# skyepurchase/MeatModeler

Measured on AMD Instinct MI355X. Metric: descriptor-match pairs/sec + BA residuals/sec, 500×1080p frames, 1/2/4/8 GPU, higher is better.
Workload: dtype u8/int32 (match), f64 (BA); 1 GPU; 500 frames 1920x1080, 4000 ORB kpts/frame, BF Hamming 2-NN + ratio, track linking, 2-view DLT, full BA (TRF, Schur, f64 MFMA Cholesky); frames=500, height=1080, width=1920, nfeatures=4000, parallelism=pairs/points x1

## Files before the change

include/meatmodeler.h:

```cpp
#ifndef MEATMODELER_H
#define MEATMODELER_H

#include <stddef.h>
#include <stdint.h>

#ifdef __cplusplus
extern "C" {
#endif

#define MM_OK 0
#define MM_ERR_ARG (-1)
#define MM_ERR_HIP (-2)
#define MM_ERR_WORKSPACE (-3)
#define MM_ERR_NUMERIC (-4)

typedef struct mm_ctx mm_ctx;

int mm_abi_version(void);
int mm_ctx_create(int device, void *hip_stream, mm_ctx **out);
void mm_ctx_destroy(mm_ctx *ctx);
const char *mm_last_error(mm_ctx *ctx);
int mm_ctx_sync(mm_ctx *ctx);
#define MM_CTL_CHOL_FORCE_ABANDON 1
#define MM_CTL_CHOL_LAST_PATH 2
#define MM_CTL_CHOL_RESERVED 3
#define MM_CTL_CU_COUNT 4
#define MM_CTL_CHOL_AVOID_FUSED 5
#define MM_CTL_LINK_LAST_VARIANT 6
#define MM_CTL_BATCH_LAST 7
long long mm_ctx_control(mm_ctx *ctx, int what, long long value);
int mm_timer_create(mm_ctx *ctx, void **timer_out);
int mm_timer_start(mm_ctx *ctx, void *timer);
int mm_timer_stop(mm_ctx *ctx, void *timer);
int mm_timer_elapsed_ms(mm_ctx *ctx, void *timer, float *ms_out);
void mm_timer_destroy(mm_ctx *ctx, void *timer);
int mm_profile_enable(mm_ctx *ctx, int on);
int mm_profile_select(mm_ctx *ctx, const char *name);
int mm_profile_report(mm_ctx *ctx, char *buf, size_t buf_len);

size_t mm_bf_workspace_bytes(int n_pairs, int nq_cap, int nt_cap);
int mm_bf_knn2_batched(mm_ctx *ctx, const uint8_t *q , const int32_t *nq , int nq_cap,
                       size_t q_set_stride, const uint8_t *t , const int32_t *nt , int nt_cap,
                       size_t t_set_stride, int n_pairs, int32_t *idx , int32_t *dist ,
                       void *ws , size_t ws_bytes);
int mm_bf_knn2_hamming(mm_ctx *ctx, const uint8_t *q , int nq, const uint8_t *t , int nt,
                       int32_t *idx , int32_t *dist , void *ws, size_t ws_bytes);
int mm_ratio_filter_batched(mm_ctx *ctx, const int32_t *idx , const int32_t *dist ,
                            const int32_t *nq , int nq_cap, int n_pairs, double threshold,
                            int32_t *pairs , int32_t *m_out );
size_t mm_bf_match_ratio_workspace_bytes(int n_pairs, int nq_cap, int nt_cap);
int mm_bf_match_ratio_batched(mm_ctx *ctx, const uint8_t *q , const int32_t *nq , int nq_cap,
                              size_t q_set_stride, const uint8_t *t , const int32_t *nt , int nt_cap,
                              size_t t_set_stride, int n_pairs, double threshold,
                              int32_t *pairs , int32_t *m_out ,
                              void *ws , size_t ws_bytes);

typedef struct mm_orb_params {
    int32_t nfeatures;
    int32_t nlevels;
    int32_t edge_threshold;
    int32_t fast_threshold;
    float scale_factor;
    int32_t reserved;
} mm_orb_params;
size_t mm_orb_workspace_bytes(int batch, int height, int width, const mm_orb_params *prm);
int mm_orb_detect_compute(mm_ctx *ctx, const uint8_t *imgs , int batch, int height, int width, int stride,
                          const mm_orb_params *prm, const int8_t *pattern , void *ws , size_t ws_bytes,
                          float *kp_xy, int32_t *kp_meta, float *kp_resp, int32_t *kp_mom, uint8_t *desc,
                          int32_t *n_out);
int mm_orb_level_sizes(int height, int width, const mm_orb_params *prm, int32_t *lvl_w ,
                       int32_t *lvl_h , int32_t *lvl_n ,
                       float *lvl_scale );

int64_t mm_link_tracks_clip(int n_frames, int cap, const int32_t *kp_count, const float *kp_xy, int mcap,
                            const int32_t *match_count, const int32_t *matches, int64_t max_tracks,
                            int64_t max_obs, int64_t *track_ptr , int32_t *obs_frame,
                            int32_t *obs_kp, int64_t *n_obs_out);
size_t mm_link_workspace_bytes(int n_frames, int cap);
int mm_link_tracks_device(mm_ctx *ctx, int n_frames, int cap, const int32_t *kp_count, const float *kp_xy,
                          const int32_t *match_count, const int32_t *matches, void *ws, size_t ws_bytes,
                          int32_t *track_ptr, int32_t *obs_frame, int32_t *obs_kp, int64_t *counts );
int mm_flatten_offsets(mm_ctx *ctx, const int32_t *track_ptr, const int32_t *sel, int64_t n_sel, int64_t *out_ptr);
int mm_flatten_tracks(mm_ctx *ctx, const int32_t *track_ptr, const int32_t *obs_frame, const int32_t *obs_kp, const float *kp_xy,
                      int cap, const int32_t *sel , int t_lo, int64_t n_sel, const int64_t *out_ptr , int64_t n_obs,
                      int frame_offset, double *coords, int32_t *frame_indices, int32_t *point_indices);
int64_t mm_ba_build_pairs(int F, int P, int64_t O, const int32_t *fi, const int32_t *pi, const int32_t *pt_ptr,
                          const int32_t *pt_obs, const int32_t *cam_ptr, const int32_t *cam_obs, int span,
                          int64_t *seg_ptr, int32_t *pair_o, int32_t *pair_o2, int64_t max_pairs);
int mm_ba_build_index(int F, int P, int64_t O, const int32_t *fi, const int32_t *pi, int32_t *pt_ptr ,
                      int32_t *pt_obs , int32_t *cam_ptr , int32_t *cam_obs );

#define MM_VERIFY_TOO_FEW 1
#define MM_VERIFY_NO_MODEL 2
#define MM_VERIFY_WEAK 4
#define MM_VERIFY_MALFORMED 8
typedef struct mm_verify_params {
    int32_t n_hyp, min_matches, min_inliers, refit_iters;
    uint32_t seed, pair_base;
    int32_t on_fail, reserved;
    double threshold_px;
} mm_verify_params;
size_t mm_verify_workspace_bytes(int n_pairs, int n_hyp);
int mm_verify_matches(mm_ctx *ctx, const float *kp_xy , const int32_t *pairs ,
                      const int32_t *m , int n_pairs, int cap, const mm_verify_params *prm,
                      int32_t *pairs_out , int32_t *m_out , double *Fm ,
                      double *cost , int32_t *info , void *ws, size_t ws_bytes);

#define MM_POSE_TOO_FEW 1
#define MM_POSE_NO_MODEL 2
#define MM_POSE_AMBIGUOUS 4
#define MM_POSE_MALFORMED 8
typedef struct mm_pose_params {
    int32_t min_matches, reserved;
    double min_front_frac, ambiguous_frac;
} mm_pose_params;
int mm_recover_poses(mm_ctx *ctx, const double *K , const float *kp_xy ,
                     const int32_t *pairs , const int32_t *m , const double *Fm ,
                     int n_pairs, int cap, const mm_pose_params *prm, double *R , double *t ,
                     double *sigma , double *depth , int32_t *info );
#define MM_CHAIN_FEW_COMMON 1
#define MM_CHAIN_BROKEN 2
int mm_chain_poses(mm_ctx *ctx, const int32_t *pairs , const int32_t *m ,
                   const double *depth , const double *R , const double *t ,
                   const int32_t *info , int n_pairs, int cap, const double *E0 , int min_common,
                   double *extrinsics , double *scale , double *rho ,
                   int32_t *chain_info );

#define MM_RESECT_TOO_FEW 1
#define MM_RESECT_NO_MODEL 2
#define MM_RESECT_WEAK 4
#define MM_RESECT_MALFORMED 8
typedef struct mm_resect_params {
    int32_t n_hyp, min_rows, min_inliers, refit_iters, polish_iters, reserved;
    uint32_t seed, cam_base;
    double threshold_px;
} mm_resect_params;
size_t mm_resect_workspace_bytes(int n_cams, int n_hyp, int64_t n_rows);
int mm_resect_cameras(mm_ctx *ctx, const double *K , const double *X , int64_t P, const double *obs ,
                      const int32_t *pi , int64_t O, const int32_t *cam_ptr ,
                      const int32_t *cam_obs , int64_t n_rows, int n_cams, const uint8_t *pt_ok ,
                      const double *prior , const mm_resect_params *prm, double *extrinsics ,
                      double *cost , uint8_t *inlier , int32_t *info , void *ws, size_t ws_bytes);

#define MM_RESECT_PLANAR 16
typedef struct mm_resect_planar_params {
    int32_t n_hyp, min_rows, min_inliers, refit_iters, polish_iters, reserved;
    uint32_t seed, cam_base;
    double threshold_px;
    double planar_tol, collinear_tol;
} mm_resect_planar_params;
size_t mm_resect_planar_workspace_bytes(int n_cams, int n_hyp, int64_t n_rows);
int mm_resect_planar(mm_ctx *ctx, const double *K , const double *X , int64_t P, const double *obs ,
                     const int32_t *pi , int64_t O, const int32_t *cam_ptr ,
                     const int32_t *cam_obs , int64_t n_rows, int n_cams, const uint8_t *pt_ok ,
                     const double *prior , const mm_resect_planar_params *prm,
                     double *extrinsics , double *cost , uint8_t *inlier ,
                     int32_t *info , double *plane , void *ws, size_t ws_bytes);

int mm_triangulate_dlt(mm_ctx *ctx, const double *proj , const int32_t *f0 , const int32_t *f1 ,
                       const double *x0 , const double *x1 , int64_t n,
                       double *X );
#define MM_TRI_BEHIND 1
#define MM_TRI_REPROJ 2
#define MM_TRI_PARALLAX 4
#define MM_TRI_DEGENERATE 8
typedef struct mm_tri_params {
    int32_t refine_iters, reserved;
    double max_reproj_px, max_cos_parallax, min_depth;
} mm_tri_params;
size_t mm_triangulate_tracks_workspace_bytes(int F);
int mm_triangulate_tracks(mm_ctx *ctx, const double *proj , int F, const int32_t *track_ptr , int64_t T,
                          const int32_t *obs_frame , const double *obs_xy , const mm_tri_params *prm,
                          double *X , double *quality , int32_t *flags , void *ws, size_t ws_bytes);

typedef struct mm_ba_problem {
    int32_t F, P;
    int64_t O;
    const double *K;
    const int32_t *fi, *pi;
    const double *obs;
    const int32_t *pt_ptr, *pt_obs;
    const int32_t *cam_ptr, *cam_obs;
    int32_t cam_span;
    int32_t reserved;
    int64_t n_seg;
    const int32_t *seg_ids;
    const int32_t *seg_chunk_ptr;
    int64_t n_chunks;
    const int32_t *chunk_seg;
    const int32_t *chunk_begin, *chunk_end;
    const int32_t *pair_o, *pair_o2;
    const int32_t *pair_p;
} mm_ba_problem;

int mm_ba_residual(mm_ctx *ctx, const mm_ba_problem *pb, const double *cams ,
                   const double *pts , double *res , double *cost2 ,
                   void *ws, size_t ws_bytes);
int mm_ba_jacobian(mm_ctx *ctx, const mm_ba_problem *pb, const double *cams, const double *pts, double *Jc,
                   double *Jp);
int mm_ba_normal_eq(mm_ctx *ctx, const mm_ba_problem *pb, const double *cams, const double *pts, double *B,
                    double *gc, double *C, double *gp);
int mm_ba_jvp(mm_ctx *ctx, const mm_ba_problem *pb, const double *cams, const double *pts, const double *wc,
              const double *wp, double *out);
size_t mm_ba_jvp_dots_workspace_bytes(const mm_ba_problem *pb);
int mm_ba_jvp_dots(mm_ctx *ctx, const mm_ba_problem *pb, const double *cams, const double *pts, const double *wc,
                   const double *wp, double *out, const double *other , double *rows ,
                   void *ws, size_t ws_bytes);
int mm_ba_schur(mm_ctx *ctx, const mm_ba_problem *pb, const double *cams, const double *pts, const double *Bd,
                const double *Cd, const double *gc, const double *gp, double *S, double *v, double *Cinv, void *ws,
                size_t ws_bytes);
size_t mm_ba_schur_workspace_bytes(const mm_ba_problem *pb);
int mm_ba_pairs_count(mm_ctx *ctx, const mm_ba_problem *pb, int32_t *cnt , int32_t *span_out );
int mm_ba_pairs_emit(mm_ctx *ctx, const mm_ba_problem *pb, const int64_t *offsets , int span,
                     int32_t *key , int32_t *pair_o , int32_t *pair_o2 );
typedef struct mm_ba_index {
    int32_t F, P;
    int64_t O;
    const int32_t *fi, *pi;
    int32_t *pt_ptr, *pt_obs, *cam_ptr, *cam_obs;
    int64_t *head;
    int32_t cam_span, chunk;
    int64_t n_pairs;
    int32_t *pair_o, *pair_o2, *pair_p;
    int32_t *seg_ids, *seg_chunk_ptr;
    int32_t *chunk_seg, *chunk_begin, *chunk_end;
} mm_ba_index;
int mm_ba_index_bounds(int F, int cam_span, int64_t n_pairs, int chunk, int64_t *seg_cap, int64_t *chunk_cap);
size_t mm_ba_index_workspace_bytes(mm_ctx *ctx, const mm_ba_index *ix, int stage);
int mm_ba_index_build(mm_ctx *ctx, const mm_ba_index *ix, int stage, void *ws0 , size_t ws0_bytes,
                      void *ws1 , size_t ws1_bytes);
size_t mm_multi_dot_workspace_bytes(void);
int mm_multi_dot(mm_ctx *ctx, int k, const double *const *a, const double *const *b, int64_t n, int64_t split,
                 double *out, void *ws, size_t ws_bytes);
int mm_trf_fused(mm_ctx *ctx, int op, const double *const *in, double *const *outv, const double *const *scalars,
                 double h0, double h1, int64_t n, int64_t split, double *out, void *ws, size_t ws_bytes);
int mm_trf_damping(mm_ctx *ctx, const double *gh2, const double *d11, double Delta, double min_damping, double *out);
size_t mm_ba_backsub_workspace_bytes(const mm_ba_problem *pb);
int mm_ba_backsub(mm_ctx *ctx, const mm_ba_problem *pb, const double *cams, const double *pts, const double *Cinv,
                  const double *gp, const double *dc , double *dp, void *ws , size_t ws_bytes);
int mm_ba_schur_solve(mm_ctx *ctx, const mm_ba_problem *pb, const double *cams, const double *pts, const double *Bd,
                      const double *Cd, const double *gc, const double *gp, double *S, double *v, double *Cinv,
                      int half_bandwidth, int32_t *info, void *ws_schur, size_t ws_schur_bytes, void *ws_chol,
                      size_t ws_chol_bytes, int n_slabs, int cams_per_slab, const int64_t *slab_seg_ptr,
                      const int64_t *slab_chunk_ptr);
int mm_ba_scale_update(mm_ctx *ctx, int F, int P, const double *B, const double *C, double *scale_inv , int first);
int mm_ba_damp(mm_ctx *ctx, int F, int P, const double *B, const double *C, const double *scale_inv, const double *reg ,
               double *Bd, double *Cd);
int mm_trf_step2d(mm_ctx *ctx, const double *r0, const double *d11, const double *r1, const double *r2, const double *r3,
                  const double *bs, const double *reg, const int32_t *info, double Delta, double *board );
typedef struct mm_trf_params {
    double ftol, xtol, gtol;
    double min_damping;
    int64_t max_nfev;
} mm_trf_params;
typedef struct mm_trf_row {
    int32_t iteration, nfev;
    double cost, reduction, step_norm, optimality;
} mm_trf_row;
typedef struct mm_trf_report {
    double cost0, cost, optimality, min_damping ;
    int32_t nfev, njev, status, iterations, log_rows;
    int32_t chol_fallbacks;
    int32_t collectives;
    int32_t reserved;
} mm_trf_report;
size_t mm_ba_trf_workspace_bytes(const mm_ba_problem *pb);
int mm_ba_trf(mm_ctx *ctx, const mm_ba_problem *pb, double *cams , double *pts ,
              const mm_trf_params *prm, mm_trf_report *report , mm_trf_row *log , int log_cap,
              void *ws , size_t ws_bytes);
typedef int (*mm_allreduce_fn)(void *user, double *buf , int64_t count);
typedef struct mm_dist {
    int32_t rank, world;
    int32_t half_bandwidth, band_exchange;
    mm_allreduce_fn allreduce;
    void *user;
} mm_dist;
size_t mm_ba_trf_dist_workspace_bytes(const mm_ba_problem *pb, int half_bandwidth);
int mm_ba_trf_dist(mm_ctx *ctx, const mm_ba_problem *pb, double *cams, double *pts, const mm_trf_params *prm,
                   mm_trf_report *report, mm_trf_row *log, int log_cap, void *ws, size_t ws_bytes, const mm_dist *dist);
size_t mm_ba_trf_batched_workspace_bytes(const mm_ba_problem *pb);
int mm_ba_trf_batched(mm_ctx *ctx, int n_prob, const mm_ba_problem *const *pbs, double *const *cams ,
                      double *const *pts , const mm_trf_params *prm, mm_trf_report *reports ,
                      void *const *ws , const size_t *ws_bytes, int32_t *solved_alone );
typedef struct mm_ba_fixed {
    int32_t F_fixed;
    int32_t reserved;
    const double *cams;
} mm_ba_fixed;
int mm_ba_residual_fixed(mm_ctx *ctx, const mm_ba_problem *pb, const mm_ba_fixed *fx, const double *cams ,
                         const double *pts , double *res , double *cost2 , void *ws,
                         size_t ws_bytes);
int mm_ba_normal_eq_fixed(mm_ctx *ctx, const mm_ba_problem *pb, const mm_ba_fixed *fx, const double *cams, const double *pts,
                          double *B, double *gc, double *C, double *gp);
size_t mm_ba_trf_fixed_workspace_bytes(const mm_ba_problem *pb, const mm_ba_fixed *fx);
int mm_ba_trf_fixed(mm_ctx *ctx, const mm_ba_problem *pb, const mm_ba_fixed *fx, double *cams ,
                    double *pts , const mm_trf_params *prm, mm_trf_report *report ,
                    mm_trf_row *log , int log_cap, void *ws , size_t ws_bytes);
size_t mm_chol_workspace_bytes(int n);
int mm_chol_solve_sym(mm_ctx *ctx, double *A , int n, double *b , int half_bandwidth, int both_triangles,
                      int32_t *info , void *ws, size_t ws_bytes);
int mm_chol_solve(mm_ctx *ctx, double *A , int n, double *b , int nrhs, int half_bandwidth,
                  int32_t *info , void *ws, size_t ws_bytes);

int mm_pyr_down(mm_ctx *ctx, const uint8_t *src , int w, int h, int src_pitch, uint8_t *dst , int dst_pitch);
int mm_lk_track(mm_ctx *ctx, const uint8_t *const *prev_levels, const uint8_t *const *next_levels, const int *w, const int *h,
                const int *pitch, int levels, const float *pts, int n, int win_w, int win_h, int max_count,
                double epsilon_sq, float *next_pts, uint8_t *status, float *err);
int mm_min_eig(mm_ctx *ctx, const uint8_t *img , int w, int h, int pitch, int block_size, double *eig );
int mm_corner_candidates(mm_ctx *ctx, const double *eig, int w, int h, double quality, unsigned long long *max_bits ,
                         long long *val_bits , int32_t *pos , int cap, int32_t *count );
int mm_gftt_select(const int32_t *pos , int64_t n, int w, int h, int max_corners, double min_distance,
                   float *out , int cap);
size_t mm_contrast_workspace_bytes(int batch, int w, int h, int tiles_x, int tiles_y);
int mm_increase_contrast(mm_ctx *ctx, const uint8_t *bgr, int batch, int w, int h, const uint16_t *gamma,
                         const uint16_t *cbrt_tab, const uint8_t *gamma_inv, double clip_limit, int tiles_x, int tiles_y,
                         uint8_t *out, uint8_t *grey , void *ws, size_t ws_bytes);
int mm_bgr_to_grey(mm_ctx *ctx, const uint8_t *bgr , size_t n_pixels, uint8_t *grey );
int mm_write_ply(const char *path, const double *xyz , int64_t n);

#ifdef __cplusplus
}
#endif
#endif
```

meatmodeler_amd/_lib.py:

```python
import ctypes as C
import os

_HERE = os.path.dirname(os.path.abspath(__file__))
LIB_PATH = os.path.join(_HERE, "libmeatmodeler_hip.so")

c_i32p = C.POINTER(C.c_int32)
c_i64p = C.POINTER(C.c_int64)
c_f32p = C.POINTER(C.c_float)
c_f64p = C.POINTER(C.c_double)
c_u8p = C.POINTER(C.c_uint8)
c_i8p = C.POINTER(C.c_int8)
vp = C.c_void_p


class MMError(RuntimeError):
    pass


class OrbParams(C.Structure):
    _fields_ = [("nfeatures", C.c_int32), ("nlevels", C.c_int32), ("edge_threshold", C.c_int32),
                ("fast_threshold", C.c_int32), ("scale_factor", C.c_float), ("reserved", C.c_int32)]


class BAProblem(C.Structure):
    _fields_ = [("F", C.c_int32), ("P", C.c_int32), ("O", C.c_int64), ("K", vp), ("fi", vp), ("pi", vp),
                ("obs", vp), ("pt_ptr", vp), ("pt_obs", vp), ("cam_ptr", vp), ("cam_obs", vp),
                ("cam_span", C.c_int32), ("reserved", C.c_int32), ("n_seg", C.c_int64), ("seg_ids", vp),
                ("seg_chunk_ptr", vp), ("n_chunks", C.c_int64), ("chunk_seg", vp), ("chunk_begin", vp),
                ("chunk_end", vp), ("pair_o", vp), ("pair_o2", vp), ("pair_p", vp)]


class BAIndex(C.Structure):
    _fields_ = [("F", C.c_int32), ("P", C.c_int32), ("O", C.c_int64), ("fi", vp), ("pi", vp),
                ("pt_ptr", vp), ("pt_obs", vp), ("cam_ptr", vp), ("cam_obs", vp), ("head", vp),
                ("cam_span", C.c_int32), ("chunk", C.c_int32), ("n_pairs", C.c_int64),
                ("pair_o", vp), ("pair_o2", vp), ("pair_p", vp), ("seg_ids", vp), ("seg_chunk_ptr", vp),
                ("chunk_seg", vp), ("chunk_begin", vp), ("chunk_end", vp)]


class BAFixed(C.Structure):
    _fields_ = [("F_fixed", C.c_int32), ("reserved", C.c_int32), ("cams", vp)]


class TrfParams(C.Structure):
    _fields_ = [("ftol", C.c_double), ("xtol", C.c_double), ("gtol", C.c_double), ("min_damping", C.c_double),
                ("max_nfev", C.c_int64)]


class TrfRow(C.Structure):
    _fields_ = [("iteration", C.c_int32), ("nfev", C.c_int32), ("cost", C.c_double), ("reduction", C.c_double),
                ("step_norm", C.c_double), ("optimality", C.c_double)]


class TriParams(C.Structure):
    _fields_ = [("refine_iters", C.c_int32), ("reserved", C.c_int32), ("max_reproj_px", C.c_double),
                ("max_cos_parallax", C.c_double), ("min_depth", C.c_double)]


class VerifyParams(C.Structure):
    _fields_ = [("n_hyp", C.c_int32), ("min_matches", C.c_int32), ("min_inliers", C.c_int32), ("refit_iters", C.c_int32),
                ("seed", C.c_uint32), ("pair_base", C.c_uint32), ("on_fail", C.c_int32), ("reserved", C.c_int32),
                ("threshold_px", C.c_double)]


class PoseParams(C.Structure):
    _fields_ = [("min_matches", C.c_int32), ("reserved", C.c_int32), ("min_front_frac", C.c_double),
                ("ambiguous_frac", C.c_double)]


class ResectParams(C.Structure):
    _fields_ = [("n_hyp", C.c_int32), ("min_rows", C.c_int32), ("min_inliers", C.c_int32), ("refit_iters", C.c_int32),
                ("polish_iters", C.c_int32), ("reserved", C.c_int32), ("seed", C.c_uint32), ("cam_base", C.c_uint32),
                ("threshold_px", C.c_double)]


class ResectPlanarParams(C.Structure):
    _fields_ = ResectParams._fields_ + [("planar_tol", C.c_double), ("collinear_tol", C.c_double)]


ALLREDUCE_FN =C.CFUNCTYPE(C.c_int, vp, vp, C.c_int64)


class Dist(C.Structure):
    _fields_ = [("rank", C.c_int32), ("world", C.c_int32), ("half_bandwidth", C.c_int32), ("band_exchange", C.c_int32),
                ("allreduce", ALLREDUCE_FN), ("user", vp)]


class TrfReport(C.Structure):
    _fields_ = [("cost0", C.c_double), ("cost", C.c_double), ("optimality", C.c_double), ("min_damping", C.c_double),
                ("nfev", C.c_int32), ("njev", C.c_int32), ("status", C.c_int32), ("iterations", C.c_int32),
                ("log_rows", C.c_int32), ("chol_fallbacks", C.c_int32), ("collectives", C.c_int32), ("reserved", C.c_int32)]


SIGNATURES = {
    "mm_abi_version": (C.c_int, []),
    "mm_ctx_create": (C.c_int, [C.c_int, vp, C.POINTER(vp)]),
    "mm_ctx_destroy": (None, [vp]),
    "mm_ctx_control": (C.c_longlong, [vp, C.c_int, C.c_longlong]),
    "mm_last_error": (C.c_char_p, [vp]),
    "mm_ctx_sync": (C.c_int, [vp]),
    "mm_timer_create": (C.c_int, [vp, C.POINTER(vp)]),
    "mm_timer_start": (C.c_int, [vp, vp]),
    "mm_timer_stop": (C.c_int, [vp, vp]),
    "mm_timer_elapsed_ms": (C.c_int, [vp, vp, C.POINTER(C.c_float)]),
    "mm_timer_destroy": (None, [vp, vp]),
    "mm_profile_enable": (C.c_int, [vp, C.c_int]),
    "mm_profile_report": (C.c_int, [vp, C.c_char_p, C.c_size_t]),
    "mm_profile_select": (C.c_int, [vp, C.c_char_p]),
    "mm_bf_workspace_bytes": (C.c_size_t, [C.c_int, C.c_int, C.c_int]),
    "mm_bf_knn2_batched": (C.c_int, [vp, vp, vp, C.c_int, C.c_size_t, vp, vp, C.c_int, C.c_size_t, C.c_int, vp, vp,
                                     vp, C.c_size_t]),
    "mm_bf_knn2_hamming": (C.c_int, [vp, vp, C.c_int, vp, C.c_int, vp, vp, vp, C.c_size_t]),
    "mm_ratio_filter_batched": (C.c_int, [vp, vp, vp, vp, C.c_int, C.c_int, C.c_double, vp, vp]),
    "mm_bf_match_ratio_workspace_bytes": (C.c_size_t, [C.c_int, C.c_int, C.c_int]),
    "mm_bf_match_ratio_batched": (C.c_int, [vp, vp, vp, C.c_int, C.c_size_t, vp, vp, C.c_int, C.c_size_t, C.c_int,
                                            C.c_double, vp, vp, vp, C.c_size_t]),
    "mm_orb_workspace_bytes": (C.c_size_t, [C.c_int, C.c_int, C.c_int, C.POINTER(OrbParams)]),
    "mm_orb_detect_compute": (C.c_int, [vp, vp, C.c_int, C.c_int, C.c_int, C.c_int, C.POINTER(OrbParams), vp, vp,
                                        C.c_size_t, vp, vp, vp, vp, vp, vp]),
    "mm_orb_level_sizes": (C.c_int, [C.c_int, C.c_int, C.POINTER(OrbParams), c_i32p, c_i32p, c_i32p, c_f32p]),
    "mm_link_tracks_clip": (C.c_int64, [C.c_int, C.c_int, c_i32p, c_f32p, C.c_int, c_i32p, c_i32p, C.c_int64,
                                        C.c_int64, c_i64p, c_i32p, c_i32p, c_i64p]),
    "mm_link_workspace_bytes": (C.c_size_t, [C.c_int, C.c_int]),
    "mm_link_tracks_device": (C.c_int, [vp, C.c_int, C.c_int, vp, vp, vp, vp, vp, C.c_size_t, vp, vp, vp, vp]),
    "mm_flatten_offsets": (C.c_int, [vp, vp, vp, C.c_int64, vp]),
    "mm_flatten_tracks": (C.c_int, [vp, vp, vp, vp, vp, C.c_int, vp, C.c_int, C.c_int64, vp, C.c_int64, C.c_int, vp, vp, vp]),
    "mm_ba_build_pairs": (C.c_int64, [C.c_int, C.c_int, C.c_int64, c_i32p, c_i32p, c_i32p, c_i32p, c_i32p, c_i32p, C.c_int,
                                      c_i64p, c_i32p, c_i32p, C.c_int64]),
    "mm_ba_build_index": (C.c_int, [C.c_int, C.c_int, C.c_int64, c_i32p, c_i32p, c_i32p, c_i32p, c_i32p, c_i32p]),
    "mm_verify_workspace_bytes": (C.c_size_t, [C.c_int, C.c_int]),
    "mm_verify_matches": (C.c_int, [vp, vp, vp, vp, C.c_int, C.c_int, C.POINTER(VerifyParams), vp, vp, vp, vp, vp, vp, C.c_size_t]),
    "mm_recover_poses": (C.c_int, [vp, c_f64p, vp, vp, vp, vp, C.c_int, C.c_int, C.POINTER(PoseParams), vp, vp, vp, vp, vp]),
    "mm_chain_poses": (C.c_int, [vp, vp, vp, vp, vp, vp, vp, C.c_int, C.c_int, c_f64p, C.c_int, vp, vp, vp, vp]),
    "mm_resect_workspace_bytes": (C.c_size_t, [C.c_int, C.c_int, C.c_int64]),
    "mm_resect_cameras": (C.c_int, [vp, c_f64p, vp, C.c_int64, vp, vp, C.c_int64, vp, vp, C.c_int64, C.c_int, vp, vp,
                                    C.POINTER(ResectParams), vp, vp, vp, vp, vp, C.c_size_t]),
    "mm_resect_planar_workspace_bytes": (C.c_size_t, [C.c_int, C.c_int, C.c_int64]),
    "mm_resect_planar": (C.c_int, [vp, c_f64p, vp, C.c_int64, vp, vp, C.c_int64, vp, vp, C.c_int64, C.c_int, vp, vp,
                                   C.POINTER(ResectPlanarParams), vp, vp, vp, vp, vp, vp, C.c_size_t]),
    "mm_triangulate_dlt": (C.c_int, [vp, vp, vp, vp, vp, vp, C.c_int64, vp]),
    "mm_triangulate_tracks_workspace_bytes": (C.c_size_t, [C.c_int]),
    "mm_triangulate_tracks": (C.c_int, [vp, vp, C.c_int, vp, C.c_int64, vp, vp, C.POINTER(TriParams), vp, vp, vp, vp, C.c_size_t]),
    "mm_ba_residual": (C.c_int, [vp, C.POINTER(BAProblem), vp, vp, vp, vp, vp, C.c_size_t]),
    "mm_ba_jacobian": (C.c_int, [vp, C.POINTER(BAProblem), vp, vp, vp, vp]),
    "mm_ba_normal_eq": (C.c_int, [vp, C.POINTER(BAProblem), vp, vp, vp, vp, vp, vp]),
    "mm_ba_jvp": (C.c_int, [vp, C.POINTER(BAProblem), vp, vp, vp, vp, vp]),
    "mm_ba_schur": (C.c_int, [vp, C.POINTER(BAProblem), vp, vp, vp, vp, vp, vp, vp, vp, vp, vp, C.c_size_t]),
    "mm_ba_schur_workspace_bytes": (C.c_size_t, [C.POINTER(BAProblem)]),
    "mm_ba_pairs_count": (C.c_int, [vp, C.POINTER(BAProblem), vp, vp]),
    "mm_ba_pairs_emit": (C.c_int, [vp, C.POINTER(BAProblem), vp, C.c_int, vp, vp, vp]),
    "mm_ba_index_bounds": (C.c_int, [C.c_int, C.c_int, C.c_int64, C.c_int, c_i64p, c_i64p]),
    "mm_ba_index_workspace_bytes": (C.c_size_t, [vp, C.POINTER(BAIndex), C.c_int]),
    "mm_ba_index_build": (C.c_int, [vp, C.POINTER(BAIndex), C.c_int, vp, C.c_size_t, vp, C.c_size_t]),
    "mm_ba_schur_solve": (C.c_int, [vp, C.POINTER(BAProblem), vp, vp, vp, vp, vp, vp, vp, vp, vp, C.c_int, vp, vp,
                                    C.c_size_t, vp, C.c_size_t, C.c_int, C.c_int, c_i64p, c_i64p]),
    "mm_multi_dot_workspace_bytes": (C.c_size_t, []),
    "mm_multi_dot": (C.c_int, [vp, C.c_int, C.POINTER(vp), C.POINTER(vp), C.c_int64, C.c_int64, vp, vp, C.c_size_t]),
    "mm_trf_fused": (C.c_int, [vp, C.c_int, C.POINTER(vp), C.POINTER(vp), C.POINTER(vp), C.c_double, C.c_double, C.c_int64,
                               C.c_int64, vp, vp, C.c_size_t]),
    "mm_trf_damping": (C.c_int, [vp, vp, vp, C.c_double, C.c_double, vp]),
    "mm_ba_backsub": (C.c_int, [vp, C.POINTER(BAProblem), vp, vp, vp, vp, vp, vp, vp, C.c_size_t]),
    "mm_ba_backsub_workspace_bytes": (C.c_size_t, [C.POINTER(BAProblem)]),
    "mm_chol_workspace_bytes": (C.c_size_t, [C.c_int]),
    "mm_chol_solve": (C.c_int, [vp, vp, C.c_int, vp, C.c_int, C.c_int, vp, vp, C.c_size_t]),
    "mm_ba_jvp_dots_workspace_bytes": (C.c_size_t, [C.POINTER(BAProblem)]),
    "mm_ba_jvp_dots": (C.c_int, [vp, C.POINTER(BAProblem), vp, vp, vp, vp, vp, vp, vp, vp, C.c_size_t]),
    "mm_ba_scale_update": (C.c_int, [vp, C.c_int, C.c_int, vp, vp, vp, C.c_int]),
    "mm_ba_damp": (C.c_int, [vp, C.c_int, C.c_int, vp, vp, vp, vp, vp, vp]),
    "mm_trf_step2d": (C.c_int, [vp, vp, vp, vp, vp, vp, vp, vp, vp, C.c_double, vp]),
    "mm_pyr_down": (C.c_int, [vp, vp, C.c_int, C.c_int, C.c_int, vp, C.c_int]),
    "mm_lk_track": (C.c_int, [vp, vp, vp, vp, vp, vp, C.c_int, vp, C.c_int, C.c_int, C.c_int, C.c_int, C.c_double, vp, vp, vp]),
    "mm_min_eig": (C.c_int, [vp, vp, C.c_int, C.c_int, C.c_int, C.c_int, vp]),
    "mm_corner_candidates": (C.c_int, [vp, vp, C.c_int, C.c_int, C.c_double, vp, vp, vp, C.c_int, vp]),
    "mm_gftt_select": (C.c_int, [vp, C.c_int64, C.c_int, C.c_int, C.c_int, C.c_double, vp, C.c_int]),
    "mm_contrast_workspace_bytes": (C.c_size_t, [C.c_int, C.c_int, C.c_int, C.c_int, C.c_int]),
    "mm_increase_contrast": (C.c_int, [vp, vp, C.c_int, C.c_int, C.c_int, vp, vp, vp, C.c_double, C.c_int, C.c_int, vp, vp, vp,
                                       C.c_size_t]),
    "mm_bgr_to_grey": (C.c_int, [vp, vp, C.c_size_t, vp]),
    "mm_write_ply": (C.c_int, [C.c_char_p, vp, C.c_int64]),
    "mm_chol_solve_sym": (C.c_int, [vp, vp, C.c_int, vp, C.c_int, C.c_int, vp, vp, C.c_size_t]),
    "mm_ba_trf_workspace_bytes": (C.c_size_t, [C.POINTER(BAProblem)]),
    "mm_ba_trf": (C.c_int, [vp, C.POINTER(BAProblem), vp, vp, C.POINTER(TrfParams), C.POINTER(TrfReport),
                            C.POINTER(TrfRow), C.c_int, vp, C.c_size_t]),
    "mm_ba_trf_batched_workspace_bytes": (C.c_size_t, [C.POINTER(BAProblem)]),
    "mm_ba_trf_batched": (C.c_int, [vp, C.c_int, C.POINTER(C.POINTER(BAProblem)), C.POINTER(vp), C.POINTER(vp),
                                    C.POINTER(TrfParams), C.POINTER(TrfReport), C.POINTER(vp), C.POINTER(C.c_size_t), c_i32p]),
    "mm_ba_residual_fixed": (C.c_int, [vp, C.POINTER(BAProblem), C.POINTER(BAFixed), vp, vp, vp, vp, vp, C.c_size_t]),
    "mm_ba_normal_eq_fixed": (C.c_int, [vp, C.POINTER(BAProblem), C.POINTER(BAFixed), vp, vp, vp, vp, vp, vp]),
    "mm_ba_trf_fixed_workspace_bytes": (C.c_size_t, [C.POINTER(BAProblem), C.POINTER(BAFixed)]),
    "mm_ba_trf_fixed": (C.c_int, [vp, C.POINTER(BAProblem), C.POINTER(BAFixed), vp, vp, C.POINTER(TrfParams),
                                  C.POINTER(TrfReport), C.POINTER(TrfRow), C.c_int, vp, C.c_size_t]),
    "mm_ba_trf_dist_workspace_bytes": (C.c_size_t, [C.POINTER(BAProblem), C.c_int]),
    "mm_ba_trf_dist": (C.c_int, [vp, C.POINTER(BAProblem), vp, vp, C.POINTER(TrfParams), C.POINTER(TrfReport),
                                 C.POINTER(TrfRow), C.c_int, vp, C.c_size_t, C.POINTER(Dist)]),
}


def _load():
    if not os.path.exists(LIB_PATH):
        raise ImportError(
            f"{LIB_PATH} is missing: the HIP extension has not been built "
            "(make -C meatmodeler_amd/csrc).  meatmodeler_amd has no CPU fallback.")
    lib = C.CDLL(LIB_PATH)
    for name, (res, args) in SIGNATURES.items():
        fn = getattr(lib, name)
        fn.restype = res
        fn.argtypes = args
    return lib


lib = _load()


def ptr(t):
    if t is None:
        return None
    if hasattr(t, "data_ptr"):
        return t.data_ptr()
    return t.ctypes.data


class Context:

    def __init__(self, device=None, stream=None):
        import torch
        if not torch.cuda.is_available():
            raise MMError("meatmodeler_amd needs an AMD GPU (torch.cuda.is_available() is False); "
                          "there is no CPU path")
        if device is None:
            device = torch.cuda.current_device()
        self.device = torch.device("cuda", device if isinstance(device, int) else device.index or 0)
        self.stream = stream if stream is not None else torch.cuda.current_stream(self.device)
        h = vp()
        rc = lib.mm_ctx_create(self.device.index, vp(self.stream.cuda_stream), C.byref(h))
        if rc != 0:
            raise MMError(f"mm_ctx_create failed ({rc})")
        self.h = h

    def check(self, rc, what=""):
        if rc != 0:
            msg = lib.mm_last_error(self.h)
            raise MMError(f"{what} failed ({rc}): {msg.decode() if msg else ''}")

    def sync(self):
        self.check(lib.mm_ctx_sync(self.h), "mm_ctx_sync")

    CTL_CHOL_FORCE_ABANDON, CTL_CHOL_LAST_PATH, CTL_CHOL_RESERVED, CTL_CU_COUNT, CTL_CHOL_AVOID_FUSED = 1, 2, 3, 4, 5
    CTL_LINK_LAST_VARIANT = 6
    CTL_BATCH_LAST = 7

    def control(self, what, value=0):
        r = int(lib.mm_ctx_control(self.h, int(what), int(value)))
        if r < -1 or (r == -1 and what not in (self.CTL_CHOL_LAST_PATH, self.CTL_LINK_LAST_VARIANT, self.CTL_BATCH_LAST)):
            self.check(r, "mm_ctx_control")
        return r

    def profile(self, level, only=None):
        if only is not None:
            self.check(lib.mm_profile_select(self.h, only.encode()), "mm_profile_select")
        self.check(lib.mm_profile_enable(self.h, int(level)), "mm_profile_enable")

    def profile_report(self):
        buf = C.create_string_buffer(1 << 16)
        n = lib.mm_profile_report(self.h, buf, len(buf))
        if n < 0:
            self.check(n, "mm_profile_report")
        out = {}
        for line in buf.value.decode().splitlines():
            name, cnt, ms = line.split()
            out[name] = (int(cnt), float(ms))
        return out

    def __del__(self):
        try:
            if getattr(self, "h", None):
                lib.mm_ctx_destroy(self.h)
                self.h = None
        except Exception:
            pass


class Timer:

    def __init__(self, ctx):
        self.ctx = ctx
        self.t = vp()
        ctx.check(lib.mm_timer_create(ctx.h, C.byref(self.t)), "mm_timer_create")

    def start(self):
        self.ctx.check(lib.mm_timer_start(self.ctx.h, self.t), "mm_timer_start")

    def stop(self):
        self.ctx.check(lib.mm_timer_stop(self.ctx.h, self.t), "mm_timer_stop")

    def elapsed_ms(self):
        ms = C.c_float()
        self.ctx.check(lib.mm_timer_elapsed_ms(self.ctx.h, self.t, C.byref(ms)), "mm_timer_elapsed_ms")
        return ms.value

    def __del__(self):
        try:
            lib.mm_timer_destroy(self.ctx.h, self.t)
        except Exception:
            pass


_default_ctx = {}


def default_context():
    import torch
    key = (torch.cuda.current_device(), torch.cuda.current_stream().cuda_stream)
    c = _default_ctx.get(key)
    if c is None:
        c = _default_ctx[key] = Context()
    return c
```

meatmodeler_amd/csrc/ba.hip:

```cpp
#include "ba_eval.h"


namespace {

template <bool FIXED>
__device__ __forceinline__ const double *cam_at(const double *__restrict__ cams, const double *__restrict__ fxc, int F, int f) {
    if constexpr (FIXED)
        return f < F ? cams + (size_t)f * 6 : fxc + (size_t)(f - F) * 6;
    else
        return cams + (size_t)f * 6;
}

template <bool FIXED>
__device__ __forceinline__ void ba_residual_body(mm_ba_problem pb, const double *__restrict__ cams, const double *__restrict__ fxc,
                                                          const double *__restrict__ pts, const CamCoef *__restrict__ ctab, double *__restrict__ res,
                                                          double *__restrict__ partial, const unsigned bx, const unsigned gx) {
    __shared__ double sm[4];
    __shared__ double Ks[9];
    if (threadIdx.x < 9) Ks[threadIdx.x] = pb.K[threadIdx.x];
    __syncthreads();
    double acc = 0;
    for (int64_t o = (int64_t)bx * 256 + threadIdx.x; o < pb.O; o += (int64_t)gx * 256) {
        Proj pr;
        const int f = pb.fi[o];
        ba_eval_cc<false, false>(cam_at<FIXED>(cams, fxc, pb.F, f), ctab[f],
                                 pts + (size_t)pb.pi[o] * 3, Ks, pb.obs[2 * o], pb.obs[2 * o + 1], pr);
        if (res) {
            res[2 * o] = pr.r0;
            res[2 * o + 1] = pr.r1;
        }
        acc += pr.r0 * pr.r0 + pr.r1 * pr.r1;
    }
    double t = block_sum<256>(acc, sm);
    if (threadIdx.x == 0) partial[bx] = t;
}
__global__ __launch_bounds__(256) void ba_residual_kernel(mm_ba_problem pb, const double *__restrict__ cams,
                                                          const double *__restrict__ pts, const CamCoef *__restrict__ ctab, double *__restrict__ res,
                                                          double *__restrict__ partial) { ba_residual_body<false>(pb, cams, nullptr, pts, ctab, res, partial, blockIdx.x, gridDim.x); }
__global__ __launch_bounds__(256) void ba_residual_fixed_kernel(mm_ba_problem pb, const double *__restrict__ cams, const double *__restrict__ fxc,
                                                                const double *__restrict__ pts, const CamCoef *__restrict__ ctab, double *__restrict__ res,
                                                                double *__restrict__ partial) { ba_residual_body<true>(pb, cams, fxc, pts, ctab, res, partial, blockIdx.x, gridDim.x); }

__global__ __launch_bounds__(256) void sum_partials_kernel(const double *__restrict__ partial, int n,
                                                           double *__restrict__ out) {
    __shared__ double sm[4];
    double acc = 0;
    for (int i = threadIdx.x; i < n; i += 256) acc += partial[i];
    double t = block_sum<256>(acc, sm);
    if (threadIdx.x == 0) out[0] = t;
}

struct MMHostBoard {
    double v[16];
    unsigned long long seq;
};
__device__ __forceinline__ void sum_partials_publish_body(const double *__restrict__ partial, int n,
                                                                   double *__restrict__ board, int cost_slot, int count,
                                                                   MMHostBoard *hb, unsigned long long seq, const unsigned bx, const unsigned gx) {
    __shared__ double sm[4];
    double acc = 0;
    for (int i = threadIdx.x; i < n; i += 256) acc += partial[i];
    const double t = block_sum<256>(acc, sm);
    if (threadIdx.x == 0) board[cost_slot] = t;
    if (threadIdx.x < 64) {
        const double t0 = __shfl(t, 0, 64);
        if ((int)threadIdx.x < count) hb->v[threadIdx.x] = (int)threadIdx.x == cost_slot ? t0 : board[threadIdx.x];
        __threadfence_system();
        __builtin_amdgcn_wave_barrier();
        if (threadIdx.x == 0) __hip_atomic_store(&hb->seq, seq, __ATOMIC_RELEASE, __HIP_MEMORY_SCOPE_SYSTEM);
    }
}
__global__ __launch_bounds__(256) void sum_partials_publish_kernel(const double *__restrict__ partial, int n,
                                                                   double *__restrict__ board, int cost_slot, int count,
                                                                   MMHostBoard *hb, unsigned long long seq) { sum_partials_publish_body(partial, n, board, cost_slot, count, hb, seq, blockIdx.x, gridDim.x); }

__global__ __launch_bounds__(256) void ba_jacobian_kernel(mm_ba_problem pb, const double *__restrict__ cams,
                                                          const double *__restrict__ pts, const CamCoef *__restrict__ ctab, double *__restrict__ Jc,
                                                          double *__restrict__ Jp) {
    __shared__ double Ks[9];
    if (threadIdx.x < 9) Ks[threadIdx.x] = pb.K[threadIdx.x];
    __syncthreads();
    int64_t o = (int64_t)blockIdx.x * 256 + threadIdx.x;
    if (o >= pb.O) return;
    Proj pr;
    const int f = pb.fi[o];
    ba_eval_cc<true, true>(cams + (size_t)f * 6, ctab[f],
                           pts + (size_t)pb.pi[o] * 3, Ks, pb.obs[2 * o], pb.obs[2 * o + 1], pr);
#pragma unroll
    for (int k = 0; k < 6; ++k) {
        Jc[o * 12 + k] = pr.Jc[0][k];
        Jc[o * 12 + 6 + k] = pr.Jc[1][k];
    }
#pragma unroll
    for (int k = 0; k < 3; ++k) {
        Jp[o * 6 + k] = pr.Jp[0][k];
        Jp[o * 6 + 3 + k] = pr.Jp[1][k];
    }
}

#ifndef MM_PB_LANES
#define MM_PB_LANES 4
#endif
constexpr int PB_LANES = MM_PB_LANES;
template <bool FIXED>
__device__ __forceinline__ void ba_point_blocks_body(mm_ba_problem pb, const double *__restrict__ cams, const double *__restrict__ fxc,
                                                              const double *__restrict__ pts, const CamCoef *__restrict__ ctab, double *__restrict__ C,
                                                              double *__restrict__ gp, const unsigned bx, const unsigned gx) {
    __shared__ double Ks[9];
    if (threadIdx.x < 9) Ks[threadIdx.x] = pb.K[threadIdx.x];
    __syncthreads();
    const int sub = threadIdx.x & (PB_LANES - 1);
    const int p = bx * (256 / PB_LANES) + (threadIdx.x / PB_LANES);
    const bool live = p < pb.P;
    double c[9] = {0, 0, 0, 0, 0, 0, 0, 0, 0};
    if (live) {
        const double *Xp = pts + (size_t)p * 3;
        const int e_end = pb.pt_ptr[p + 1];
        for (int e = pb.pt_ptr[p] + sub; e < e_end; e += PB_LANES) {
            const int o = pb.pt_obs[e];
            Proj pr;
            const int f = pb.fi[o];
            ba_eval_cc<false, true>(cam_at<FIXED>(cams, fxc, pb.F, f), ctab[f], Xp, Ks, pb.obs[2 * (size_t)o], pb.obs[2 * (size_t)o + 1], pr);
#pragma unroll
            for (int m = 0; m < 2; ++m) {
                const double j0 = pr.Jp[m][0], j1 = pr.Jp[m][1], j2 = pr.Jp[m][2];
                const double r = m == 0 ? pr.r0 : pr.r1;
                c[0] += j0 * j0; c[1] += j0 * j1; c[2] += j0 * j2;
                c[3] += j1 * j1; c[4] += j1 * j2; c[5] += j2 * j2;
                c[6] += j0 * r; c[7] += j1 * r; c[8] += j2 * r;
            }
        }
    }
#pragma unroll
    for (int off = 1; off < PB_LANES; off <<= 1) {
        double t[9];
#pragma unroll
        for (int q = 0; q < 9; ++q) t[q] = __shfl_xor(c[q], off, 64);
#pragma unroll
        for (int q = 0; q < 9; ++q) c[q] += t[q];
    }
    if (live && sub == 0) {
        double *Cp = C + (size_t)p * 6;
#pragma unroll
        for (int q = 0; q < 6; ++q) Cp[q] = c[q];
        gp[(size_t)p * 3] = c[6]; gp[(size_t)p * 3 + 1] = c[7]; gp[(size_t)p * 3 + 2] = c[8];
    }
}
__global__ __launch_bounds__(256) void ba_point_blocks_kernel(mm_ba_problem pb, const double *__restrict__ cams,
                                                              const double *__restrict__ pts, const CamCoef *__restrict__ ctab, double *__restrict__ C,
                                                              double *__restrict__ gp) { ba_point_blocks_body<false>(pb, cams, nullptr, pts, ctab, C, gp, blockIdx.x, gridDim.x); }
__global__ __launch_bounds__(256) void ba_point_blocks_fixed_kernel(mm_ba_problem pb, const double *__restrict__ cams, const double *__restrict__ fxc,
                                                                    const double *__restrict__ pts, const CamCoef *__restrict__ ctab, double *__restrict__ C,
                                                                    double *__restrict__ gp) { ba_point_blocks_body<true>(pb, cams, fxc, pts, ctab, C, gp, blockIdx.x, gridDim.x); }

__device__ __forceinline__ void ba_camera_blocks_body(mm_ba_problem pb, const double *__restrict__ cams,
                                                               const double *__restrict__ pts, double *__restrict__ B,
                                                               double *__restrict__ gc, const unsigned bx, const unsigned gx) {
    __shared__ double smn[4 * 27];
    __shared__ double Ks[9];
    __shared__ double cs[6];
    const int f = bx;
    if (threadIdx.x < 9) Ks[threadIdx.x] = pb.K[threadIdx.x];
    if (threadIdx.x < 6) cs[threadIdx.x] = cams[(size_t)f * 6 + threadIdx.x];
    __syncthreads();
    const CamCoef ccf = cam_coef_of(cs);
    double acc[27];
#pragma unroll
    for (int i = 0; i < 27; ++i) acc[i] = 0;
    for (int e = pb.cam_ptr[f] + threadIdx.x; e < pb.cam_ptr[f + 1]; e += 256) {
        int o = pb.cam_obs[e];
        Proj pr;
        ba_eval_cc<true, false>(cs, ccf, pts + (size_t)pb.pi[o] * 3, Ks, pb.obs[2 * (size_t)o], pb.obs[2 * (size_t)o + 1],
                                pr);
        int t = 0;
#pragma unroll
        for (int i = 0; i < 6; ++i) {
#pragma unroll
            for (int j = i; j < 6; ++j) {
                acc[t] += pr.Jc[0][i] * pr.Jc[0][j] + pr.Jc[1][i] * pr.Jc[1][j];
                ++t;
            }
            acc[21 + i] += pr.Jc[0][i] * pr.r0 + pr.Jc[1][i] * pr.r1;
        }
    }
    block_sum_n<27, 256>(acc, smn);
    if (threadIdx.x == 0) {
        int t = 0;
#pragma unroll
        for (int i = 0; i < 6; ++i) {
#pragma unroll
            for (int j = i; j < 6; ++j) {
                B[(size_t)f * 36 + i * 6 + j] = acc[t];
                B[(size_t)f * 36 + j * 6 + i] = acc[t];
                ++t;
            }
            gc[(size_t)f * 6 + i] = acc[21 + i];
        }
    }
}
__global__ __launch_bounds__(256) void ba_camera_blocks_kernel(mm_ba_problem pb, const double *__restrict__ cams,
                                                               const double *__restrict__ pts, double *__restrict__ B,
                                                               double *__restrict__ gc) { ba_camera_blocks_body(pb, cams, pts, B, gc, blockIdx.x, gridDim.x); }

__global__ __launch_bounds__(256) void ba_normal_eq_kernel(mm_ba_problem pb, const double *__restrict__ cams, const double *__restrict__ pts,
                                                           const CamCoef *__restrict__ ctab, double *__restrict__ B, double *__restrict__ gc,
                                                           double *__restrict__ C, double *__restrict__ gp) {
    if ((int)blockIdx.x < pb.F) ba_camera_blocks_body(pb, cams, pts, B, gc, blockIdx.x, (unsigned)pb.F);
    else ba_point_blocks_body<false>(pb, cams, nullptr, pts, ctab, C, gp, blockIdx.x - (unsigned)pb.F, gridDim.x - (unsigned)pb.F);
}
__global__ __launch_bounds__(256) void ba_normal_eq_fixed_kernel(mm_ba_problem pb, const double *__restrict__ cams, const double *__restrict__ fxc,
                                                                 const double *__restrict__ pts, const CamCoef *__restrict__ ctab, double *__restrict__ B,
                                                                 double *__restrict__ gc, double *__restrict__ C, double *__restrict__ gp) {
    if ((int)blockIdx.x < pb.F) ba_camera_blocks_body(pb, cams, pts, B, gc, blockIdx.x, (unsigned)pb.F);
    else ba_point_blocks_body<true>(pb, cams, fxc, pts, ctab, C, gp, blockIdx.x - (unsigned)pb.F, gridDim.x - (unsigned)pb.F);
}

__global__ __launch_bounds__(256) void ba_jvp_kernel(mm_ba_problem pb, const double *__restrict__ cams,
                                                     const double *__restrict__ pts, const CamCoef *__restrict__ ctab, const double *__restrict__ wc,
                                                     const double *__restrict__ wp, double *__restrict__ out) {
    __shared__ double Ks[9];
    if (threadIdx.x < 9) Ks[threadIdx.x] = pb.K[threadIdx.x];
    __syncthreads();
    int64_t o = (int64_t)blockIdx.x * 256 + threadIdx.x;
    if (o >= pb.O) return;
    const int f = pb.fi[o], p = pb.pi[o];
    Proj pr;
    ba_eval_cc<true, true>(cams + (size_t)f * 6, ctab[f],
                           pts + (size_t)p * 3, Ks, pb.obs[2 * o], pb.obs[2 * o + 1], pr);
    double y0 = 0, y1 = 0;
    if (wc) {
#pragma unroll
        for (int k = 0; k < 6; ++k) {
            double w = wc[(size_t)f * 6 + k];
            y0 += pr.Jc[0][k] * w;
            y1 += pr.Jc[1][k] * w;
        }
    }
    if (wp) {
#pragma unroll
        for (int k = 0; k < 3; ++k) {
            double w = wp[(size_t)p * 3 + k];
            y0 += pr.Jp[0][k] * w;
            y1 += pr.Jp[1][k] * w;
        }
    }
    out[2 * o] = y0;
    out[2 * o + 1] = y1;
}

template <bool FIXED>
__device__ __forceinline__ void ba_jvp_dots_body(mm_ba_problem pb, const double *__restrict__ cams, const double *__restrict__ fxc,
                                                          const double *__restrict__ pts, const CamCoef *__restrict__ ctab, const double *__restrict__ wc,
                                                          const double *__restrict__ wp, double *__restrict__ out,
                                                          const double *__restrict__ other, double *__restrict__ partial, const unsigned bx, const unsigned gx) {
    __shared__ double Ks[9];
    __shared__ double sm[(256 / 64) * 2];
    if (threadIdx.x < 9) Ks[threadIdx.x] = pb.K[threadIdx.x];
    __syncthreads();
    double acc[2] = {0.0, 0.0};
    for (int64_t o = (int64_t)bx * 256 + threadIdx.x; o < pb.O; o += (int64_t)gx * 256) {
        const int f = pb.fi[o], p = pb.pi[o];
        Proj pr;
        ba_eval_cc<true, true>(cam_at<FIXED>(cams, fxc, pb.F, f), ctab[f],
                               pts + (size_t)p * 3, Ks, pb.obs[2 * o], pb.obs[2 * o + 1], pr);
        double y0 = 0, y1 = 0;
        if (wc && (!FIXED || f < pb.F)) {
#pragma unroll
            for (int k = 0; k < 6; ++k) {
                const double w = wc[(size_t)f * 6 + k];
                y0 += pr.Jc[0][k] * w;
                y1 += pr.Jc[1][k] * w;
            }
        }
        if (wp) {
#pragma unroll
            for (int k = 0; k < 3; ++k) {
                const double w = wp[(size_t)p * 3 + k];
                y0 += pr.Jp[0][k] * w;
                y1 += pr.Jp[1][k] * w;
            }
        }
        out[2 * o] = y0;
        out[2 * o + 1] = y1;
        const double sq = y0 * y0 + y1 * y1;
        acc[1] += sq;
        acc[0] += other ? y0 * other[2 * o] + y1 * other[2 * o + 1] : sq;
    }
    block_sum_n<2, 256>(acc, sm);
    if (threadIdx.x == 0) {
        partial[2 * (size_t)bx] = acc[0];
        partial[2 * (size_t)bx + 1] = acc[1];
    }
}
__global__ __launch_bounds__(256) void ba_jvp_dots_kernel(mm_ba_problem pb, const double *__restrict__ cams,
                                                          const double *__restrict__ pts, const CamCoef *__restrict__ ctab, const double *__restrict__ wc,
                                                          const double *__restrict__ wp, double *__restrict__ out,
                                                          const double *__restrict__ other, double *__restrict__ partial) { ba_jvp_dots_body<false>(pb, cams, nullptr, pts, ctab, wc, wp, out, other, partial, blockIdx.x, gridDim.x); }
__global__ __launch_bounds__(256) void ba_jvp_dots_fixed_kernel(mm_ba_problem pb, const double *__restrict__ cams, const double *__restrict__ fxc,
                                                                const double *__restrict__ pts, const CamCoef *__restrict__ ctab, const double *__restrict__ wc,
                                                                const double *__restrict__ wp, double *__restrict__ out,
                                                                const double *__restrict__ other, double *__restrict__ partial) { ba_jvp_dots_body<true>(pb, cams, fxc, pts, ctab, wc, wp, out, other, partial, blockIdx.x, gridDim.x); }

__global__ __launch_bounds__(256) void jvp_rows_kernel(const double *__restrict__ partial, unsigned n_wg, double *__restrict__ rows) { (void)jvp_rows_body(partial, n_wg, rows, blockIdx.x, gridDim.x); }

__global__ __launch_bounds__(256) void ba_backsub_kernel(mm_ba_problem pb, const double *__restrict__ cams,
                                                         const double *__restrict__ pts, const CamCoef *__restrict__ ctab,
                                                         const double *__restrict__ Cinv, const double *__restrict__ gp,
                                                         const double *__restrict__ dc, double *__restrict__ dp) {
    __shared__ double Ks[9];
    if (threadIdx.x < 9) Ks[threadIdx.x] = pb.K[threadIdx.x];
    __syncthreads();
    int p = blockIdx.x * 256 + threadIdx.x;
    if (p >= pb.P) return;
    const double *Xp = pts + (size_t)p * 3;
    double t0 = gp[(size_t)p * 3], t1 = gp[(size_t)p * 3 + 1], t2 = gp[(size_t)p * 3 + 2];
    for (int e = pb.pt_ptr[p]; e < pb.pt_ptr[p + 1]; ++e) {
        int o = pb.pt_obs[e];
        int f = pb.fi[o];
        Proj pr;
        ba_eval_cc<true, true>(cams + (size_t)f * 6, ctab[f], Xp, Ks,
                               pb.obs[2 * (size_t)o], pb.obs[2 * (size_t)o + 1], pr);
        double s0 = 0, s1 = 0;
#pragma unroll
        for (int k = 0; k < 6; ++k) {
            double d = dc[(size_t)f * 6 + k];
            s0 += pr.Jc[0][k] * d;
            s1 += pr.Jc[1][k] * d;
        }
        t0 -= pr.Jp[0][0] * s0 + pr.Jp[1][0] * s1;
        t1 -= pr.Jp[0][1] * s0 + pr.Jp[1][1] * s1;
        t2 -= pr.Jp[0][2] * s0 + pr.Jp[1][2] * s1;
    }
    const double *c = Cinv + (size_t)p * 6;
    dp[(size_t)p * 3] = c[0] * t0 + c[1] * t1 + c[2] * t2;
    dp[(size_t)p * 3 + 1] = c[1] * t0 + c[3] * t1 + c[4] * t2;
    dp[(size_t)p * 3 + 2] = c[2] * t0 + c[4] * t1 + c[5] * t2;
}

template <bool FIXED>
__device__ __forceinline__ void ba_backsub_obs_body(mm_ba_problem pb, const double *__restrict__ cams, const double *__restrict__ fxc,
                                                             const double *__restrict__ pts, const CamCoef *__restrict__ ctab,
                                                             const double *__restrict__ dc, double *__restrict__ T, const unsigned bx, const unsigned gx) {
    __shared__ double Ks[9];
    if (threadIdx.x < 9) Ks[threadIdx.x] = pb.K[threadIdx.x];
    __syncthreads();
    const int64_t e = (int64_t)bx * 256 + threadIdx.x;
    if (e >= pb.O) return;
    const int o = pb.pt_obs[e];
    const int f = pb.fi[o], p = pb.pi[o];
    Proj pr;
    ba_eval_cc<true, true>(cam_at<FIXED>(cams, fxc, pb.F, f), ctab[f], pts + (size_t)p * 3, Ks, pb.obs[2 * (size_t)o],
                           pb.obs[2 * (size_t)o + 1], pr);
    double s0 = 0, s1 = 0;
    if (!FIXED || f < pb.F) {
#pragma unroll
        for (int k = 0; k < 6; ++k) {
            const double d = dc[(size_t)f * 6 + k];
            s0 += pr.Jc[0][k] * d;
            s1 += pr.Jc[1][k] * d;
        }
    }
    T[3 * e] = pr.Jp[0][0] * s0 + pr.Jp[1][0] * s1;
    T[3 * e + 1] = pr.Jp[0][1] * s0 + pr.Jp[1][1] * s1;
    T[3 * e + 2] = pr.Jp[0][2] * s0 + pr.Jp[1][2] * s1;
}
__global__ __launch_bounds__(256) void ba_backsub_obs_kernel(mm_ba_problem pb, const double *__restrict__ cams,
                                                             const double *__restrict__ pts, const CamCoef *__restrict__ ctab,
                                                             const double *__restrict__ dc, double *__restrict__ T) { ba_backsub_obs_body<false>(pb, cams, nullptr, pts, ctab, dc, T, blockIdx.x, gridDim.x); }
__global__ __launch_bounds__(256) void ba_backsub_obs_fixed_kernel(mm_ba_problem pb, const double *__restrict__ cams, const double *__restrict__ fxc,
                                                                   const double *__restrict__ pts, const CamCoef *__restrict__ ctab,
                                                                   const double *__restrict__ dc, double *__restrict__ T) { ba_backsub_obs_body<true>(pb, cams, fxc, pts, ctab, dc, T, blockIdx.x, gridDim.x); }

__device__ __forceinline__ void ba_backsub_points_body(mm_ba_problem pb, const double *__restrict__ T,
                                                                const double *__restrict__ Cinv, const double *__restrict__ gp,
                                                                double *__restrict__ dp, const unsigned bx, const unsigned gx) {
    const int sub = threadIdx.x & (PB_LANES - 1);
    const int p = bx * (256 / PB_LANES) + (threadIdx.x / PB_LANES);
    const bool live = p < pb.P;
    double t[3] = {0.0, 0.0, 0.0};
    if (live) {
        const int e_end = pb.pt_ptr[p + 1];
        for (int e = pb.pt_ptr[p] + sub; e < e_end; e += PB_LANES) {
            t[0] += T[3 * (size_t)e];
            t[1] += T[3 * (size_t)e + 1];
            t[2] += T[3 * (size_t)e + 2];
        }
    }
#pragma unroll
    for (int off = 1; off < PB_LANES; off <<= 1) {
        double u[3];
#pragma unroll
        for (int q = 0; q < 3; ++q) u[q] = __shfl_xor(t[q], off, 64);
#pragma unroll
        for (int q = 0; q < 3; ++q) t[q] += u[q];
    }
    if (live && sub == 0) {
        const double t0 = gp[(size_t)p * 3] - t[0], t1 = gp[(size_t)p * 3 + 1] - t[1], t2 = gp[(size_t)p * 3 + 2] - t[2];
        const double *c = Cinv + (size_t)p * 6;
        dp[(size_t)p * 3] = c[0] * t0 + c[1] * t1 + c[2] * t2;
        dp[(size_t)p * 3 + 1] = c[1] * t0 + c[3] * t1 + c[4] * t2;
        dp[(size_t)p * 3 + 2] = c[2] * t0 + c[4] * t1 + c[5] * t2;
    }
}
__global__ __launch_bounds__(256) void ba_backsub_points_kernel(mm_ba_problem pb, const double *__restrict__ T,
                                                                const double *__restrict__ Cinv, const double *__restrict__ gp,
                                                                double *__restrict__ dp) { ba_backsub_points_body(pb, T, Cinv, gp, dp, blockIdx.x, gridDim.x); }

__device__ __forceinline__ void cam_coef_body(const double *__restrict__ cams, int F, CamCoef *__restrict__ tab, const unsigned bx, const unsigned gx) {
    const int f = bx * 256 + threadIdx.x;
    if (f < F) tab[f] = cam_coef_of(cams + (size_t)f * 6);
}
__global__ __launch_bounds__(256) void cam_coef_kernel(const double *__restrict__ cams, int F, CamCoef *__restrict__ tab) { cam_coef_body(cams, F, tab, blockIdx.x, gridDim.x); }

int check_pb(mm_ctx *ctx, const mm_ba_problem *pb, const char *who) {
    if (!ctx) return MM_ERR_ARG;
    if (!pb || pb->F < 0 || pb->P < 0 || pb->O < 0 || !pb->K) return mm_fail(ctx, MM_ERR_ARG, "%s: bad problem", who);
    if (pb->O > 0 && (!pb->fi || !pb->pi || !pb->obs)) return mm_fail(ctx, MM_ERR_ARG, "%s: null observation arrays", who);
    return MM_OK;
}

constexpr int RES_BLOCKS = 2048;
constexpr int JVP_MAX_WG = 2048;
inline int res_wg_cap() {
    static const int cap = [] {
        const char *e = getenv("MM_RES_WG");
        const int v = e ? atoi(e) : RES_BLOCKS;
        return v < 1 ? 1 : (v > RES_BLOCKS ? RES_BLOCKS : v);
    }();
    return cap;
}
inline int jvp_wg_cap() {
    static const int cap = [] {
        const char *e = getenv("MM_JVP_WG");
        const int v = e ? atoi(e) : 1024;
        return v < 1 ? 1 : (v > JVP_MAX_WG ? JVP_MAX_WG : v);
    }();
    return cap;
}

__device__ __forceinline__ void trf_damping_body(const double *__restrict__ gh2, const double *__restrict__ d11, double Delta,
                                                 double min_damping, double *__restrict__ out) {
    if (threadIdx.x != 0) return;
    const double reg = trf_damping_value(gh2[0], d11[0], Delta);
    out[0] = reg;
    out[1] = fmax(reg, min_damping);
}
__global__ void trf_damping_kernel(const double *__restrict__ gh2, const double *__restrict__ d11, double Delta,
                                   double min_damping, double *__restrict__ out) {
    if (blockIdx.x != 0) return;
    trf_damping_body(gh2, d11, Delta, min_damping, out);
}

#define MM_BATCH_PROB(gfield)                                   \
    const int pid = list[blockIdx.y];                           \
    const mm_batch_prob &bp = tab[pid];                         \
    if (blockIdx.x >= bp.gfield) return
__global__ __launch_bounds__(256) void cam_coef_batch_kernel(const mm_batch_prob *__restrict__ tab, const int32_t *__restrict__ list, int which) {
    MM_BATCH_PROB(g_coef);
    cam_coef_body(which ? bp.x_new : bp.x, bp.pb.F, (CamCoef *)(which ? bp.ctab_new : bp.ctab_x), blockIdx.x, bp.g_coef);
}
__global__ __launch_bounds__(256) void ba_residual_batch_kernel(const mm_batch_prob *__restrict__ tab, const int32_t *__restrict__ list) {
    MM_BATCH_PROB(g_res);
    ba_residual_body<false>(bp.pb, bp.x_new, nullptr, bp.x_new + bp.nc, (const CamCoef *)bp.ctab_new, nullptr, bp.res_partial, blockIdx.x, bp.g_res);
}
__global__ __launch_bounds__(256) void sum_partials_publish_batch_kernel(const mm_batch_prob *__restrict__ tab, const int32_t *__restrict__ list,
                                                                         const mm_batch_dyn *__restrict__ dyn) {
    const int pid = list[blockIdx.x];
    const mm_batch_prob &bp = tab[pid];
    sum_partials_publish_body(bp.res_partial, (int)bp.g_res, bp.board, 14, 16, (MMHostBoard *)bp.mailbox, dyn[pid].seq, 0, 1);
}
__global__ __launch_bounds__(64) void publish_r0_batch_kernel(const mm_batch_prob *__restrict__ tab, const int32_t *__restrict__ list,
                                                              const mm_batch_dyn *__restrict__ dyn) {
    const int pid = list[blockIdx.x];
    const mm_batch_prob &bp = tab[pid];
    MMHostBoard *hb = (MMHostBoard *)bp.mailbox;
    if (threadIdx.x < 6) hb->v[threadIdx.x] = bp.r0[threadIdx.x];
    __threadfence_system();
    __builtin_amdgcn_wave_barrier();
    if (threadIdx.x == 0) __hip_atomic_store(&hb->seq, dyn[pid].seq, __ATOMIC_RELEASE, __HIP_MEMORY_SCOPE_SYSTEM);
}
__global__ __launch_bounds__(256) void ba_jvp_dots_batch_kernel(const mm_batch_prob *__restrict__ tab, const int32_t *__restrict__ list, int second) {
    MM_BATCH_PROB(g_jvp);
    const double *w = second ? bp.s2 : bp.ghs;
    ba_jvp_dots_body<false>(bp.pb, bp.x, nullptr, bp.x + bp.nc, (const CamCoef *)bp.ctab_x, w, w + bp.nc, second ? bp.Jq2 : bp.u1,
                     second ? bp.u1 : nullptr, bp.jvp_partial, blockIdx.x, bp.g_jvp);
}
__global__ __launch_bounds__(256) void jvp_rows_batch_kernel(const mm_batch_prob *__restrict__ tab, const int32_t *__restrict__ list, int second) {
    const mm_batch_prob &bp = tab[list[blockIdx.x]];
    jvp_rows_body(bp.jvp_partial, bp.g_jvp, second ? bp.bs : bp.d11, 0, 1);
}
__global__ void trf_damping_batch_kernel(const mm_batch_prob *__restrict__ tab, const int32_t *__restrict__ list,
                                         const mm_batch_dyn *__restrict__ dyn) {
    const int pid = list[blockIdx.x];
    const mm_batch_prob &bp = tab[pid];
    trf_damping_body(bp.r0 + 2, bp.d11 + 2, dyn[pid].Delta, dyn[pid].min_damping, bp.damp);
}
__global__ void set_reg_batch_kernel(const mm_batch_prob *__restrict__ tab, const int32_t *__restrict__ list,
                                     const mm_batch_dyn *__restrict__ dyn) {
    const int pid = list[blockIdx.x];
    if (threadIdx.x == 0) tab[pid].damp[1] = dyn[pid].reg;
}
__global__ __launch_bounds__(256) void ba_backsub_obs_batch_kernel(const mm_batch_prob *__restrict__ tab, const int32_t *__restrict__ list) {
    MM_BATCH_PROB(g_obs);
    ba_backsub_obs_body<false>(bp.pb, bp.x, nullptr, bp.x + bp.nc, (const CamCoef *)bp.ctab_x, bp.v, bp.backsub_T, blockIdx.x, bp.g_obs);
}
__global__ __launch_bounds__(256) void ba_backsub_points_batch_kernel(const mm_batch_prob *__restrict__ tab, const int32_t *__restrict__ list) {
    MM_BATCH_PROB(g_pts);
    ba_backsub_points_body(bp.pb, bp.backsub_T, bp.Cinv, bp.g + bp.nc, bp.dp, blockIdx.x, bp.g_pts);
}
__global__ __launch_bounds__(256) void ba_normal_eq_batch_kernel(const mm_batch_prob *__restrict__ tab, const int32_t *__restrict__ list) {
    const mm_batch_prob &bp = tab[list[blockIdx.y]];
    const unsigned F = (unsigned)bp.pb.F;
    if (blockIdx.x < F) ba_camera_blocks_body(bp.pb, bp.x, bp.x + bp.nc, bp.B, bp.g, blockIdx.x, F);
    else if (blockIdx.x - F < bp.g_pblk)
        ba_point_blocks_body<false>(bp.pb, bp.x, nullptr, bp.x + bp.nc, (const CamCoef *)bp.ctab_x, bp.C, bp.g + bp.nc, blockIdx.x - F, bp.g_pblk);
}

}

int mm_cam_coef_table(mm_ctx *ctx, const double *cams, int F, const void **tab_out) {
    const int rows = F + ctx->fx_F;
    if (rows > ctx->cam_tab_cap) {
        if (ctx->cam_tab) (void)hipFree(ctx->cam_tab);
        ctx->cam_tab = nullptr;
        ctx->cam_tab_cap = 0;
        const int cap = rows < 1024 ? 1024 : rows + rows / 2;
        MM_HIP(ctx, hipMalloc(&ctx->cam_tab, (size_t)cap * sizeof(CamCoef)));
        ctx->cam_tab_cap = cap;
        ctx->cam_tab_for = nullptr;
        ctx->fx_tab_ok = false;
    }
    if (!(ctx->cam_tab_hold && ctx->cam_tab_for == cams && ctx->cam_tab_F == F)) {
        if (F > 0)
            MM_LAUNCH(ctx, "cam_coef_kernel", cam_coef_kernel, dim3((F + 255) / 256), dim3(256), 0, cams, F, (CamCoef *)ctx->cam_tab);
        ctx->cam_tab_for = cams;
        ctx->cam_tab_F = F;
    }
    if (ctx->fx_F > 0 && !ctx->fx_tab_ok) {
        MM_LAUNCH(ctx, "cam_coef_kernel", cam_coef_kernel, dim3((ctx->fx_F + 255) / 256), dim3(256), 0, ctx->fx_cams, ctx->fx_F,
                  (CamCoef *)ctx->cam_tab + F);
        ctx->fx_tab_ok = true;
    }
    *tab_out = ctx->cam_tab;
    return MM_OK;
}
int mm_cam_table_adopt(mm_ctx *ctx, const double *cams, int F, void **tab_out) {
    const int rows = F + ctx->fx_F;
    if (rows > ctx->cam_tab_cap) {
        if (ctx->cam_tab) (void)hipFree(ctx->cam_tab);
        ctx->cam_tab = nullptr;
        ctx->cam_tab_cap = 0;
        const int cap = rows < 1024 ? 1024 : rows + rows / 2;
        MM_HIP(ctx, hipMalloc(&ctx->cam_tab, (size_t)cap * sizeof(CamCoef)));
        ctx->cam_tab_cap = cap;
        ctx->fx_tab_ok = false;
    }
    ctx->cam_tab_for = cams;
    ctx->cam_tab_F = F;
    *tab_out = ctx->cam_tab;
    return MM_OK;
}
void mm_cam_table_hold(mm_ctx *ctx, bool on) {
    ctx->cam_tab_hold = on;
    ctx->cam_tab_for = nullptr;
}
void mm_cam_table_invalidate(mm_ctx *ctx) { ctx->cam_tab_for = nullptr; }

int mm_ba_residual_publish(mm_ctx *ctx, const mm_ba_problem *pb, const double *cams, const double *pts, void *ws,
                           size_t ws_bytes, double *board, int cost_slot, int count, void *host_board, unsigned long long seq);

#define MM_CAM_TABLE(ctx, pb, cams)                                               \
    const CamCoef *ctab = nullptr;                                                \
    do {                                                                          \
        const void *t_ = nullptr;                                                 \
        int rc_ = mm_cam_coef_table(ctx, cams, (pb)->F, &t_);                     \
        if (rc_) return rc_;                                                      \
        ctab = (const CamCoef *)t_;                                               \
    } while (0)

extern "C" {

int mm_ba_residual(mm_ctx *ctx, const mm_ba_problem *pb, const double *cams, const double *pts, double *res,
                   double *cost2, void *ws, size_t ws_bytes) {
    int rc = check_pb(ctx, pb, "mm_ba_residual");
    if (rc) return rc;
    if (!cams || !pts || !cost2) return mm_fail(ctx, MM_ERR_ARG, "mm_ba_residual: null pointer");
    if (!ws || ws_bytes < RES_BLOCKS * sizeof(double)) return mm_fail(ctx, MM_ERR_WORKSPACE, "mm_ba_residual: workspace < 16 KiB");
    int64_t nb = (pb->O + 255) / 256;
    int blocks = (int)(nb < 1 ? 1 : (nb > res_wg_cap() ? res_wg_cap() : nb));
    MM_CAM_TABLE(ctx, pb, cams);
    if (ctx->fx_F > 0)
        MM_LAUNCH(ctx, "ba_residual_fixed_kernel", ba_residual_fixed_kernel, dim3(blocks), dim3(256), 0, *pb, cams, ctx->fx_cams, pts, ctab, res,
                  (double *)ws);
    else
        MM_LAUNCH(ctx, "ba_residual_kernel", ba_residual_kernel, dim3(blocks), dim3(256), 0, *pb, cams, pts, ctab, res, (double *)ws);
    MM_LAUNCH(ctx, "sum_partials_kernel", sum_partials_kernel, dim3(1), dim3(256), 0, (const double *)ws, blocks, cost2);
    return MM_OK;
}

int mm_ba_jacobian(mm_ctx *ctx, const mm_ba_problem *pb, const double *cams, const double *pts, double *Jc, double *Jp) {
    int rc = check_pb(ctx, pb, "mm_ba_jacobian");
    if (rc) return rc;
    if (!cams || !pts || !Jc || !Jp) return mm_fail(ctx, MM_ERR_ARG, "mm_ba_jacobian: null pointer");
    if (ctx->fx_F > 0) return mm_fail(ctx, MM_ERR_ARG, "mm_ba_jacobian: no fixed-camera form");
    if (pb->O == 0) return MM_OK;
    MM_CAM_TABLE(ctx, pb, cams);
    MM_LAUNCH(ctx, "ba_jacobian_kernel", ba_jacobian_kernel, dim3((unsigned)((pb->O + 255) / 256)), dim3(256), 0, *pb, cams, pts, ctab, Jc, Jp);
    return MM_OK;
}

int mm_ba_normal_eq(mm_ctx *ctx, const mm_ba_problem *pb, const double *cams, const double *pts, double *B, double *gc,
                    double *C, double *gp) {
    int rc = check_pb(ctx, pb, "mm_ba_normal_eq");
    if (rc) return rc;
    if (!cams || !pts) return mm_fail(ctx, MM_ERR_ARG, "mm_ba_normal_eq: null pointer");
    if ((B == nullptr) != (gc == nullptr) || (C == nullptr) != (gp == nullptr))
        return mm_fail(ctx, MM_ERR_ARG, "mm_ba_normal_eq: B/gc and C/gp come in pairs");
    if (B && C && pb->P > 0 && pb->F > 0) {
        if (!pb->pt_ptr || !pb->pt_obs || !pb->cam_ptr || !pb->cam_obs) return mm_fail(ctx, MM_ERR_ARG, "mm_ba_normal_eq: CSR missing");
        MM_CAM_TABLE(ctx, pb, cams);
        const unsigned g_pblk = (unsigned)((pb->P + 256 / PB_LANES - 1) / (256 / PB_LANES));
        if (ctx->fx_F > 0)
            MM_LAUNCH(ctx, "ba_normal_eq_fixed_kernel", ba_normal_eq_fixed_kernel, dim3((unsigned)pb->F + g_pblk), dim3(256), 0, *pb, cams,
                      ctx->fx_cams, pts, ctab, B, gc, C, gp);
        else
            MM_LAUNCH(ctx, "ba_normal_eq_kernel", ba_normal_eq_kernel, dim3((unsigned)pb->F + g_pblk), dim3(256), 0, *pb, cams, pts, ctab, B, gc, C, gp);
        return MM_OK;
    }
    if (C) {
        if (!pb->pt_ptr || !pb->pt_obs) return mm_fail(ctx, MM_ERR_ARG, "mm_ba_normal_eq: point CSR missing");
        if (pb->P > 0) {
            MM_CAM_TABLE(ctx, pb, cams);
            if (ctx->fx_F > 0)
                MM_LAUNCH(ctx, "ba_point_blocks_fixed_kernel", ba_point_blocks_fixed_kernel, dim3((pb->P + 256 / PB_LANES - 1) / (256 / PB_LANES)),
                          dim3(256), 0, *pb, cams, ctx->fx_cams, pts, ctab, C, gp);
            else
                MM_LAUNCH(ctx, "ba_point_blocks_kernel", ba_point_blocks_kernel, dim3((pb->P + 256 / PB_LANES - 1) / (256 / PB_LANES)), dim3(256), 0,
                          *pb, cams, pts, ctab, C, gp);
        }
    }
    if (B) {
        if (!pb->cam_ptr || !pb->cam_obs) return mm_fail(ctx, MM_ERR_ARG, "mm_ba_normal_eq: camera CSR missing");
        if (pb->F > 0) {
            MM_LAUNCH(ctx, "ba_camera_blocks_kernel", ba_camera_blocks_kernel, dim3(pb->F), dim3(256), 0, *pb, cams, pts, B, gc);
        }
    }
    return MM_OK;
}

int mm_ba_jvp(mm_ctx *ctx, const mm_ba_problem *pb, const double *cams, const double *pts, const double *wc,
              const double *wp, double *out) {
    int rc = check_pb(ctx, pb, "mm_ba_jvp");
    if (rc) return rc;
    if (!cams || !pts || !out) return mm_fail(ctx, MM_ERR_ARG, "mm_ba_jvp: null pointer");
    if (ctx->fx_F > 0) return mm_fail(ctx, MM_ERR_ARG, "mm_ba_jvp: no fixed-camera form");
    if (pb->O == 0) return MM_OK;
    MM_CAM_TABLE(ctx, pb, cams);
    MM_LAUNCH(ctx, "ba_jvp_kernel", ba_jvp_kernel, dim3((unsigned)((pb->O + 255) / 256)), dim3(256), 0, *pb, cams, pts, ctab, wc, wp, out);
    return MM_OK;
}

size_t mm_ba_jvp_dots_workspace_bytes(const mm_ba_problem *pb) {
    if (!pb || pb->O <= 0) return 256;
    return 256 + mm_align_up((size_t)((pb->O + 255) / 256) * 2 * sizeof(double), 256);
}

int mm_ba_jvp_dots(mm_ctx *ctx, const mm_ba_problem *pb, const double *cams, const double *pts, const double *wc,
                   const double *wp, double *out, const double *other, double *rows, void *ws, size_t ws_bytes) {
    int rc = check_pb(ctx, pb, "mm_ba_jvp_dots");
    if (rc) return rc;
    if (!cams || !pts || !out || !rows) return mm_fail(ctx, MM_ERR_ARG, "mm_ba_jvp_dots: null pointer");
    if (!ws || ws_bytes < mm_ba_jvp_dots_workspace_bytes(pb) || ((uintptr_t)ws & 255))
        return mm_fail(ctx, MM_ERR_WORKSPACE, "mm_ba_jvp_dots: workspace too small or misaligned");
    if (pb->O == 0) {
        MM_HIP(ctx, hipMemsetAsync(rows, 0, 6 * sizeof(double), ctx->stream));
        return MM_OK;
    }
    const int64_t n_all = (pb->O + 255) / 256;
    const unsigned n_wg = (unsigned)(n_all < jvp_wg_cap() ? n_all : jvp_wg_cap());
    MM_CAM_TABLE(ctx, pb, cams);
    if (ctx->fx_F > 0)
        MM_LAUNCH(ctx, "ba_jvp_fixed_kernel", ba_jvp_dots_fixed_kernel, dim3(n_wg), dim3(256), 0, *pb, cams, ctx->fx_cams, pts, ctab, wc, wp,
                  out, other, (double *)((char *)ws + 256));
    else
        MM_LAUNCH(ctx, "ba_jvp_kernel", ba_jvp_dots_kernel, dim3(n_wg), dim3(256), 0, *pb, cams, pts, ctab, wc, wp, out, other,
                  (double *)((char *)ws + 256));
    if (ctx->jvp_rows_deferred) {
        ctx->jvp_partial = (const double *)((char *)ws + 256);
        ctx->jvp_n_wg = n_wg;
        return MM_OK;
    }
    MM_LAUNCH(ctx, "jvp_rows_kernel", jvp_rows_kernel, dim3(1), dim3(256), 0, (const double *)((char *)ws + 256), n_wg, rows);
    return MM_OK;
}

size_t mm_ba_backsub_workspace_bytes(const mm_ba_problem *pb) {
    if (!pb || pb->O <= 0) return 256;
    return mm_align_up((size_t)pb->O * 3 * sizeof(double), 256);
}

int mm_ba_backsub(mm_ctx *ctx, const mm_ba_problem *pb, const double *cams, const double *pts, const double *Cinv,
                  const double *gp, const double *dc, double *dp, void *ws, size_t ws_bytes) {
    int rc = check_pb(ctx, pb, "mm_ba_backsub");
    if (rc) return rc;
    if (!cams || !pts || !Cinv || !gp || !dc || !dp || !pb->pt_ptr || !pb->pt_obs)
        return mm_fail(ctx, MM_ERR_ARG, "mm_ba_backsub: null pointer");
    if (ws && ws_bytes < mm_ba_backsub_workspace_bytes(pb)) return mm_fail(ctx, MM_ERR_WORKSPACE, "mm_ba_backsub: workspace too small");
    if (pb->P == 0) return MM_OK;
    if (ctx->fx_F > 0 && !ws) return mm_fail(ctx, MM_ERR_WORKSPACE, "mm_ba_backsub: fixed cameras need the workspace");
    MM_CAM_TABLE(ctx, pb, cams);
    if (ws && pb->O > 0) {
        if (ctx->fx_F > 0)
            MM_LAUNCH(ctx, "ba_backsub_fixed_kernel", ba_backsub_obs_fixed_kernel, dim3((unsigned)((pb->O + 255) / 256)), dim3(256), 0, *pb,
                      cams, ctx->fx_cams, pts, ctab, dc, (double *)ws);
        else
            MM_LAUNCH(ctx, "ba_backsub_kernel", ba_backsub_obs_kernel, dim3((unsigned)((pb->O + 255) / 256)), dim3(256), 0, *pb, cams, pts,
                      ctab, dc, (double *)ws);
        MM_LAUNCH(ctx, "ba_backsub_points_kernel", ba_backsub_points_kernel, dim3((pb->P + 256 / PB_LANES - 1) / (256 / PB_LANES)), dim3(256), 0,
                  *pb, (const double *)ws, Cinv, gp, dp);
        return MM_OK;
    }
    MM_LAUNCH(ctx, "ba_backsub_kernel", ba_backsub_kernel, dim3((pb->P + 255) / 256), dim3(256), 0, *pb, cams, pts, ctab, Cinv, gp, dc, dp);
    return MM_OK;
}

static int mm_ba_fixed_check(mm_ctx *ctx, const mm_ba_fixed *fx, const char *who) {
    if (fx->F_fixed < 0 || (fx->F_fixed > 0 && !fx->cams)) return mm_fail(ctx, MM_ERR_ARG, "%s: bad fixed-camera descriptor", who);
    return MM_OK;
}

int mm_ba_residual_fixed(mm_ctx *ctx, const mm_ba_problem *pb, const mm_ba_fixed *fx, const double *cams, const double *pts,
                         double *res, double *cost2, void *ws, size_t ws_bytes) {
    if (!ctx) return MM_ERR_ARG;
    if (!fx || fx->F_fixed == 0) return mm_ba_residual(ctx, pb, cams, pts, res, cost2, ws, ws_bytes);
    int rc = mm_ba_fixed_check(ctx, fx, "mm_ba_residual_fixed");
    if (rc) return rc;
    mm_fixed_scope scope(ctx, fx);
    return mm_ba_residual(ctx, pb, cams, pts, res, cost2, ws, ws_bytes);
}

int mm_ba_normal_eq_fixed(mm_ctx *ctx, const mm_ba_problem *pb, const mm_ba_fixed *fx, const double *cams, const double *pts,
                          double *B, double *gc, double *C, double *gp) {
    if (!ctx) return MM_ERR_ARG;
    if (!fx || fx->F_fixed == 0) return mm_ba_normal_eq(ctx, pb, cams, pts, B, gc, C, gp);
    int rc = mm_ba_fixed_check(ctx, fx, "mm_ba_normal_eq_fixed");
    if (rc) return rc;
    mm_fixed_scope scope(ctx, fx);
    return mm_ba_normal_eq(ctx, pb, cams, pts, B, gc, C, gp);
}

int mm_trf_damping(mm_ctx *ctx, const double *gh2, const double *d11, double Delta, double min_damping, double *out) {
    if (!ctx) return MM_ERR_ARG;
    if (!gh2 || !d11 || !out || !(Delta > 0.0)) return mm_fail(ctx, MM_ERR_ARG, "mm_trf_damping: bad argument");
    MM_LAUNCH(ctx, "trf_damping_kernel", trf_damping_kernel, dim3(1), dim3(64), 0, gh2, d11, Delta, min_damping, out);
    return MM_OK;
}

}

int mm_ba_residual_publish(mm_ctx *ctx, const mm_ba_problem *pb, const double *cams, const double *pts, void *ws,
                           size_t ws_bytes, double *board, int cost_slot, int count, void *host_board, unsigned long long seq) {
    int rc = check_pb(ctx, pb, "mm_ba_residual");
    if (rc) return rc;
    if (!cams || !pts || !board || !host_board || count > 16 || cost_slot >= count) return mm_fail(ctx, MM_ERR_ARG, "mm_ba_residual_publish: bad argument");
    if (!ws || ws_bytes < RES_BLOCKS * sizeof(double)) return mm_fail(ctx, MM_ERR_WORKSPACE, "mm_ba_residual: workspace < 16 KiB");
    int64_t nb = (pb->O + 255) / 256;
    int blocks = (int)(nb < 1 ? 1 : (nb > res_wg_cap() ? res_wg_cap() : nb));
    MM_CAM_TABLE(ctx, pb, cams);
    if (ctx->fx_F > 0)
        MM_LAUNCH(ctx, "ba_residual_fixed_kernel", ba_residual_fixed_kernel, dim3(blocks), dim3(256), 0, *pb, cams, ctx->fx_cams, pts, ctab,
                  (double *)nullptr, (double *)ws);
    else
        MM_LAUNCH(ctx, "ba_residual_kernel", ba_residual_kernel, dim3(blocks), dim3(256), 0, *pb, cams, pts, ctab, (double *)nullptr, (double *)ws);
    MM_LAUNCH(ctx, "sum_partials_kernel", sum_partials_publish_kernel, dim3(1), dim3(256), 0, (const double *)ws, blocks, board,
              cost_slot, count, (MMHostBoard *)host_board, seq);
    return MM_OK;
}


void mm_batch_ba_setup(mm_batch_prob *bp) {
    const mm_ba_problem &pb = bp->pb;
    const int64_t nb = (pb.O + 255) / 256;
    bp->g_res = (uint32_t)(nb < 1 ? 1 : (nb > res_wg_cap() ? res_wg_cap() : nb));
    bp->g_jvp = (uint32_t)(nb < jvp_wg_cap() ? (nb < 1 ? 1 : nb) : jvp_wg_cap());
    bp->g_pblk = (uint32_t)((pb.P + 256 / PB_LANES - 1) / (256 / PB_LANES));
    bp->g_obs = (uint32_t)(nb < 1 ? 1 : nb);
    bp->g_pts = (uint32_t)((pb.P + 256 / PB_LANES - 1) / (256 / PB_LANES));
    bp->g_coef = (uint32_t)((pb.F + 255) / 256);
}
int mm_batch_cam_coef(mm_ctx *ctx, const mm_batch_prob *tab, const int32_t *list, int n_list, unsigned max_g, int which) {
    if (n_list <= 0) return MM_OK;
    MM_LAUNCH(ctx, "cam_coef_kernel", cam_coef_batch_kernel, dim3(max_g, (unsigned)n_list), dim3(256), 0, tab, list, which);
    return MM_OK;
}
int mm_batch_jvp_dots(mm_ctx *ctx, const mm_batch_prob *tab, const int32_t *list, int n_list, unsigned max_g, int second) {
    if (n_list <= 0) return MM_OK;
    MM_LAUNCH(ctx, "ba_jvp_kernel", ba_jvp_dots_batch_kernel, dim3(max_g, (unsigned)n_list), dim3(256), 0, tab, list, second);
    MM_LAUNCH(ctx, "jvp_rows_kernel", jvp_rows_batch_kernel, dim3((unsigned)n_list), dim3(256), 0, tab, list, second);
    return MM_OK;
}
int mm_batch_damping(mm_ctx *ctx, const mm_batch_prob *tab, const int32_t *list, int n_list, const mm_batch_dyn *dyn) {
    if (n_list <= 0) return MM_OK;
    MM_LAUNCH(ctx, "trf_damping_kernel", trf_damping_batch_kernel, dim3((unsigned)n_list), dim3(64), 0, tab, list, dyn);
    return MM_OK;
}
int mm_batch_set_reg(mm_ctx *ctx, const mm_batch_prob *tab, const int32_t *list, int n_list, const mm_batch_dyn *dyn) {
    if (n_list <= 0) return MM_OK;
    MM_LAUNCH(ctx, "set_reg_kernel", set_reg_batch_kernel, dim3((unsigned)n_list), dim3(64), 0, tab, list, dyn);
    return MM_OK;
}
int mm_batch_backsub(mm_ctx *ctx, const mm_batch_prob *tab, const int32_t *list, int n_list, unsigned max_g_obs, unsigned max_g_pts) {
    if (n_list <= 0) return MM_OK;
    MM_LAUNCH(ctx, "ba_backsub_kernel", ba_backsub_obs_batch_kernel, dim3(max_g_obs, (unsigned)n_list), dim3(256), 0, tab, list);
    MM_LAUNCH(ctx, "ba_backsub_points_kernel", ba_backsub_points_batch_kernel, dim3(max_g_pts, (unsigned)n_list), dim3(256), 0, tab, list);
    return MM_OK;
}
int mm_batch_residual_publish(mm_ctx *ctx, const mm_batch_prob *tab, const int32_t *list, int n_list, unsigned max_g,
                              const mm_batch_dyn *dyn) {
    if (n_list <= 0) return MM_OK;
    MM_LAUNCH(ctx, "ba_residual_kernel", ba_residual_batch_kernel, dim3(max_g, (unsigned)n_list), dim3(256), 0, tab, list);
    MM_LAUNCH(ctx, "sum_partials_kernel", sum_partials_publish_batch_kernel, dim3((unsigned)n_list), dim3(256), 0, tab, list, dyn);
    return MM_OK;
}
int mm_batch_normal_eq(mm_ctx *ctx, const mm_batch_prob *tab, const int32_t *list, int n_list, unsigned max_g_pblk, unsigned max_F) {
    if (n_list <= 0) return MM_OK;
    MM_LAUNCH(ctx, "ba_normal_eq_kernel", ba_normal_eq_batch_kernel, dim3(max_F + max_g_pblk, (unsigned)n_list), dim3(256), 0, tab, list);
    return MM_OK;
}
int mm_batch_publish_rows(mm_ctx *ctx, const mm_batch_prob *tab, const int32_t *list, int n_list, const mm_batch_dyn *dyn) {
    if (n_list <= 0) return MM_OK;
    MM_LAUNCH(ctx, "board_publish_kernel", publish_r0_batch_kernel, dim3((unsigned)n_list), dim3(64), 0, tab, list, dyn);
    return MM_OK;
}
```

meatmodeler_amd/csrc/ba_index.hip:

```cpp
#include <cstring>
#include "mm_common.h"
#include <rocprim/rocprim.hpp>

namespace {

constexpr int HEAD_SPAN = 0, HEAD_PAIRS = 1, HEAD_BAD_RANGE = 2, HEAD_NOT_POINT_MAJOR = 3, HEAD_SEG = 4, HEAD_CHUNKS = 5;

__device__ __forceinline__ bool idx_ok(const int64_t *head) { return head[HEAD_BAD_RANGE] == 0 && head[HEAD_NOT_POINT_MAJOR] == 0; }

__global__ __launch_bounds__(256) void idx_validate_kernel(const int32_t *__restrict__ fi, const int32_t *__restrict__ pi,
                                                           int64_t O, int F, int P, int64_t *__restrict__ head) {
    const int64_t o = (int64_t)blockIdx.x * 256 + threadIdx.x;
    bool bad = false, unsorted = false;
    if (o < O) {
        const int f = fi[o], p = pi[o];
        bad = f < 0 || f >= F || p < 0 || p >= P;
        unsorted = o > 0 && pi[o - 1] > p;
    }
    if (__ballot(bad) != 0 && (threadIdx.x & 63) == 0) head[HEAD_BAD_RANGE] = 1;
    if (__ballot(unsorted) != 0 && (threadIdx.x & 63) == 0) head[HEAD_NOT_POINT_MAJOR] = 1;
}

__global__ __launch_bounds__(256) void idx_ptr_kernel(const int32_t *__restrict__ keys, int64_t n, int nbins,
                                                      int32_t *__restrict__ ptr, int32_t *__restrict__ identity,
                                                      const int64_t *__restrict__ head) {
    if (!idx_ok(head)) return;
    const int64_t i = (int64_t)blockIdx.x * 256 + threadIdx.x;
    if (i >= n) return;
    const int k = keys[i];
    const int lo = i == 0 ? 0 : keys[i - 1] + 1;
    for (int b = lo; b <= k; ++b) ptr[b] = (int32_t)i;
    if (i == n - 1)
        for (int b = k + 1; b <= nbins; ++b) ptr[b] = (int32_t)n;
    if (identity) identity[i] = (int32_t)i;
}

__global__ __launch_bounds__(256) void idx_count_kernel(const int32_t *__restrict__ fi, const int32_t *__restrict__ pi,
                                                        const int32_t *__restrict__ pt_ptr, int64_t O,
                                                        int32_t *__restrict__ cnt, int32_t *__restrict__ span_out,
                                                        const int64_t *__restrict__ head) {
    if (!idx_ok(head)) return;
    const int64_t o = (int64_t)blockIdx.x * 256 + threadIdx.x;
    int dmax = 0;
    if (o < O) {
        const int f = fi[o], p = pi[o];
        int c = 0;
        for (int e = pt_ptr[p]; e < pt_ptr[p + 1]; ++e) {
            const int d = f - fi[e];
            c += d >= 0;
            dmax = max(dmax, d);
        }
        cnt[o] = c;
    }
    for (int off = 32; off > 0; off >>= 1) dmax = max(dmax, __shfl_down(dmax, off, 64));
    if ((threadIdx.x & 63) == 0 && dmax > __hip_atomic_load(span_out, __ATOMIC_RELAXED, __HIP_MEMORY_SCOPE_AGENT)) atomicMax(span_out, dmax);
}

__global__ void idx_head0_kernel(const int32_t *__restrict__ cnt, const int64_t *__restrict__ offs, int64_t O,
                                 const int32_t *__restrict__ span, int64_t *__restrict__ head) {
    if (!idx_ok(head)) return;
    head[HEAD_SPAN] = *span;
    head[HEAD_PAIRS] = offs[O - 1] + cnt[O - 1];
}

__global__ __launch_bounds__(256) void idx_emit_kernel(const int32_t *__restrict__ fi, const int32_t *__restrict__ pi,
                                                       const int32_t *__restrict__ pt_ptr, int64_t O,
                                                       const int64_t *__restrict__ offs, int span, int64_t n_pairs,
                                                       int32_t *__restrict__ key, uint64_t *__restrict__ val,
                                                       const int64_t *__restrict__ head) {
    if (!idx_ok(head)) return;
    const int64_t o = (int64_t)blockIdx.x * 256 + threadIdx.x;
    if (o >= O) return;
    const int f = fi[o], p = pi[o];
    int64_t w = offs[o];
    for (int e = pt_ptr[p]; e < pt_ptr[p + 1]; ++e) {
        const int d = f - fi[e];
        if (d < 0) continue;
        if (w >= n_pairs) return;
        key[w] = f * (span + 1) + min(d, span);
        val[w] = ((uint64_t)(uint32_t)e << 32) | (uint32_t)o;
        ++w;
    }
}

__global__ __launch_bounds__(256) void idx_unpack_kernel(const uint64_t *__restrict__ val, const int32_t *__restrict__ pi,
                                                         int64_t n_pairs, int64_t O, int32_t *__restrict__ pair_o,
                                                         int32_t *__restrict__ pair_o2, int32_t *__restrict__ pair_p) {
    const int64_t i = (int64_t)blockIdx.x * 256 + threadIdx.x;
    if (i >= n_pairs) return;
    const uint64_t v = val[i];
    const uint32_t o = (uint32_t)v, o2 = (uint32_t)(v >> 32);
    pair_o[i] = (int32_t)o;
    pair_o2[i] = (int32_t)o2;
    pair_p[i] = pi[min((int64_t)o, O - 1)];
}

__global__ __launch_bounds__(256) void idx_segcount_kernel(const int32_t *__restrict__ counts, const int32_t *__restrict__ n_seg,
                                                           int64_t seg_cap, int chunk, int32_t *__restrict__ pairs_of,
                                                           int32_t *__restrict__ chunks_of) {
    const int64_t s = (int64_t)blockIdx.x * 256 + threadIdx.x;
    if (s > seg_cap) return;
    const int c = s < *n_seg ? counts[s] : 0;
    pairs_of[s] = c;
    chunks_of[s] = (c + chunk - 1) / chunk;
}

__global__ __launch_bounds__(256) void idx_chunks_kernel(const int32_t *__restrict__ n_seg_dev, const int32_t *__restrict__ seg_lo,
                                                         const int32_t *__restrict__ pairs_of,
                                                         const int32_t *__restrict__ seg_chunk_ptr, int chunk, int64_t chunk_cap,
                                                         int32_t *__restrict__ chunk_seg, int32_t *__restrict__ chunk_begin,
                                                         int32_t *__restrict__ chunk_end, int64_t *__restrict__ head) {
    const int64_t s = ((int64_t)blockIdx.x * 256 + threadIdx.x) >> 6;
    const int lane = threadIdx.x & 63;
    const int n_seg = *n_seg_dev;
    if (s == 0 && lane == 0) {
        head[HEAD_SEG] = n_seg;
        head[HEAD_CHUNKS] = seg_chunk_ptr[n_seg];
    }
    if (s >= n_seg) return;
    const int lo = seg_lo[s], hi = lo + pairs_of[s];
    const int64_t c0 = seg_chunk_ptr[s], c1 = seg_chunk_ptr[s + 1];
    for (int64_t c = c0 + lane; c < c1 && c < chunk_cap; c += 64) {
        const int b = lo + chunk * (int)(c - c0);
        chunk_seg[c] = (int32_t)s;
        chunk_begin[c] = b;
        chunk_end[c] = min(b + chunk, hi);
    }
}

int bits_for(int64_t n_values) {
    int b = 1;
    while (b < 63 && ((int64_t)1 << b) < n_values) ++b;
    return b;
}

struct Carve {
    size_t at = 0;
    size_t take(size_t bytes) {
        const size_t o = at;
        at += mm_align_up(bytes ? bytes : 1, 256);
        return o;
    }
};
struct Ws0 {
    size_t keys, cnt, offs, span, tmp, tmp_bytes, total;
};
struct Ws1 {
    size_t key, val, key_s, val_s, counts, n_seg, pairs_of, chunks_of, seg_lo, tmp, tmp_bytes, total;
};

hipError_t ws0_layout(int F, int64_t O, hipStream_t st, Ws0 &w) {
    size_t t_sort = 0, t_scan = 0;
    hipError_t e = rocprim::radix_sort_pairs(nullptr, t_sort, (const int32_t *)nullptr, (int32_t *)nullptr, (const int32_t *)nullptr,
                                             (int32_t *)nullptr, (size_t)O, 0u, (unsigned)bits_for(F), st);
    if (e != hipSuccess) return e;
    e = rocprim::exclusive_scan(nullptr, t_scan, (const int32_t *)nullptr, (int64_t *)nullptr, (int64_t)0, (size_t)O,
                                rocprim::plus<int64_t>(), st);
    if (e != hipSuccess) return e;
    Carve c;
    w.keys = c.take((size_t)O * 4);
    w.cnt = c.take((size_t)O * 4);
    w.offs = c.take((size_t)O * 8);
    w.span = c.take(4);
    w.tmp_bytes = t_sort > t_scan ? t_sort : t_scan;
    w.tmp = c.take(w.tmp_bytes);
    w.total = c.at;
    return hipSuccess;
}

hipError_t ws1_layout(int64_t n_pairs, int64_t seg_cap, int key_bits, hipStream_t st, Ws1 &w) {
    size_t t_sort = 0, t_rle = 0, t_scan = 0;
    hipError_t e = rocprim::radix_sort_pairs(nullptr, t_sort, (const int32_t *)nullptr, (int32_t *)nullptr, (const uint64_t *)nullptr,
                                             (uint64_t *)nullptr, (size_t)n_pairs, 0u, (unsigned)key_bits, st);
    if (e != hipSuccess) return e;
    e = rocprim::run_length_encode(nullptr, t_rle, (const int32_t *)nullptr, (size_t)n_pairs, (int32_t *)nullptr, (int32_t *)nullptr,
                                   (int32_t *)nullptr, st);
    if (e != hipSuccess) return e;
    e = rocprim::exclusive_scan(nullptr, t_scan, (const int32_t *)nullptr, (int32_t *)nullptr, (int32_t)0, (size_t)seg_cap + 1,
                                rocprim::plus<int32_t>(), st);
    if (e != hipSuccess) return e;
    Carve c;
    w.key = c.take((size_t)n_pairs * 4);
    w.val = c.take((size_t)n_pairs * 8);
    w.key_s = c.take((size_t)n_pairs * 4);
    w.val_s = c.take((size_t)n_pairs * 8);
    w.counts = c.take((size_t)seg_cap * 4);
    w.n_seg = c.take(4);
    w.pairs_of = c.take((size_t)(seg_cap + 1) * 4);
    w.chunks_of = c.take((size_t)(seg_cap + 1) * 4);
    w.seg_lo = c.take((size_t)(seg_cap + 1) * 4);
    w.tmp_bytes = t_sort > t_rle ? t_sort : t_rle;
    if (t_scan > w.tmp_bytes) w.tmp_bytes = t_scan;
    w.tmp = c.take(w.tmp_bytes);
    w.total = c.at;
    return hipSuccess;
}

bool index_args_ok(const mm_ba_index *ix) {
    return ix && ix->F > 0 && ix->P > 0 && ix->O > 0 && ix->O < 0x7fffffffLL && ix->fi && ix->pi && ix->head;
}
bool band_ok(const mm_ba_index *ix) {
    return ix->cam_span >= 0 && ix->cam_span < ix->F && (int64_t)ix->F * (ix->cam_span + 1) < 0x80000000LL && ix->n_pairs > 0 &&
           ix->n_pairs < 0x7fffffffLL && ix->chunk >= 64 && ix->chunk % 64 == 0;
}

}

extern "C" {

int mm_ba_index_bounds(int F, int cam_span, int64_t n_pairs, int chunk, int64_t *seg_cap, int64_t *chunk_cap) {
    if (F <= 0 || cam_span < 0 || n_pairs < 0 || chunk <= 0 || !seg_cap || !chunk_cap) return MM_ERR_ARG;
    const int64_t keys = (int64_t)F * ((int64_t)cam_span + 1);
    *seg_cap = n_pairs < keys ? n_pairs : keys;
    *chunk_cap = *seg_cap + n_pairs / chunk;
    return MM_OK;
}

size_t mm_ba_index_workspace_bytes(mm_ctx *ctx, const mm_ba_index *ix, int stage) {
    if (!ctx || !index_args_ok(ix)) return 0;
    if (stage == 0) {
        Ws0 w;
        return ws0_layout(ix->F, ix->O, ctx->stream, w) == hipSuccess ? w.total : 0;
    }
    if (stage != 1 || !band_ok(ix)) return 0;
    int64_t seg_cap, chunk_cap;
    mm_ba_index_bounds(ix->F, ix->cam_span, ix->n_pairs, ix->chunk, &seg_cap, &chunk_cap);
    Ws1 w;
    return ws1_layout(ix->n_pairs, seg_cap, bits_for((int64_t)ix->F * (ix->cam_span + 1)), ctx->stream, w) == hipSuccess ? w.total : 0;
}

int mm_ba_index_build(mm_ctx *ctx, const mm_ba_index *ix, int stage, void *ws0, size_t ws0_bytes, void *ws1, size_t ws1_bytes) {
    if (!ctx) return MM_ERR_ARG;
    if (!index_args_ok(ix) || !ix->pt_ptr || !ix->pt_obs || !ix->cam_ptr || !ix->cam_obs || !ws0 || ((uintptr_t)ws0 & 15))
        return mm_fail(ctx, MM_ERR_ARG, "mm_ba_index_build: bad argument");
    const int64_t O = ix->O;
    const unsigned gO = (unsigned)((O + 255) / 256);
    hipStream_t st = ctx->stream;
    Ws0 w0;
    MM_HIP(ctx, ws0_layout(ix->F, O, st, w0));
    if (ws0_bytes < w0.total) return mm_fail(ctx, MM_ERR_WORKSPACE, "mm_ba_index_build: stage 0 workspace too small");
    uint8_t *b0 = (uint8_t *)ws0;
    int32_t *keys = (int32_t *)(b0 + w0.keys), *cnt = (int32_t *)(b0 + w0.cnt), *span = (int32_t *)(b0 + w0.span);
    int64_t *offs = (int64_t *)(b0 + w0.offs);
    if (stage == 0) {
        MM_HIP(ctx, hipMemsetAsync(ix->head, 0, 8 * sizeof(int64_t), st));
        MM_HIP(ctx, hipMemsetAsync(span, 0, sizeof(int32_t), st));
        MM_LAUNCH(ctx, "idx_validate_kernel", idx_validate_kernel, dim3(gO), dim3(256), 0, ix->fi, ix->pi, O, ix->F, ix->P, ix->head);
        MM_LAUNCH(ctx, "idx_ptr_kernel", idx_ptr_kernel, dim3(gO), dim3(256), 0, ix->pi, O, ix->P, ix->pt_ptr, ix->pt_obs,
                  (const int64_t *)ix->head);
        size_t tb = w0.tmp_bytes;
        MM_HIP(ctx, rocprim::radix_sort_pairs((void *)(b0 + w0.tmp), tb, ix->fi, keys, (const int32_t *)ix->pt_obs, ix->cam_obs,
                                              (size_t)O, 0u, (unsigned)bits_for(ix->F), st));
        MM_LAUNCH(ctx, "idx_ptr_kernel", idx_ptr_kernel, dim3(gO), dim3(256), 0, (const int32_t *)keys, O, ix->F, ix->cam_ptr,
                  (int32_t *)nullptr, (const int64_t *)ix->head);
        MM_LAUNCH(ctx, "idx_count_kernel", idx_count_kernel, dim3(gO), dim3(256), 0, ix->fi, ix->pi, (const int32_t *)ix->pt_ptr, O,
                  cnt, span, (const int64_t *)ix->head);
        tb = w0.tmp_bytes;
        MM_HIP(ctx, rocprim::exclusive_scan((void *)(b0 + w0.tmp), tb, (const int32_t *)cnt, offs, (int64_t)0, (size_t)O,
                                            rocprim::plus<int64_t>(), st));
        MM_LAUNCH(ctx, "idx_head0_kernel", idx_head0_kernel, dim3(1), dim3(1), 0, (const int32_t *)cnt, (const int64_t *)offs, O,
                  (const int32_t *)span, ix->head);
        return MM_OK;
    }
    if (stage != 1) return mm_fail(ctx, MM_ERR_ARG, "mm_ba_index_build: stage must be 0 or 1");
    if (!band_ok(ix) || !ix->pair_o || !ix->pair_o2 || !ix->pair_p || !ix->seg_ids || !ix->seg_chunk_ptr || !ix->chunk_seg ||
        !ix->chunk_begin || !ix->chunk_end || !ws1 || ((uintptr_t)ws1 & 15))
        return mm_fail(ctx, MM_ERR_ARG, "mm_ba_index_build: bad stage 1 argument");
    int64_t seg_cap, chunk_cap;
    mm_ba_index_bounds(ix->F, ix->cam_span, ix->n_pairs, ix->chunk, &seg_cap, &chunk_cap);
    const int key_bits = bits_for((int64_t)ix->F * (ix->cam_span + 1));
    Ws1 w1;
    MM_HIP(ctx, ws1_layout(ix->n_pairs, seg_cap, key_bits, st, w1));
    if (ws1_bytes < w1.total) return mm_fail(ctx, MM_ERR_WORKSPACE, "mm_ba_index_build: stage 1 workspace too small");
    uint8_t *b1 = (uint8_t *)ws1;
    int32_t *key = (int32_t *)(b1 + w1.key), *key_s = (int32_t *)(b1 + w1.key_s), *counts = (int32_t *)(b1 + w1.counts);
    int32_t *n_seg = (int32_t *)(b1 + w1.n_seg), *pairs_of = (int32_t *)(b1 + w1.pairs_of), *chunks_of = (int32_t *)(b1 + w1.chunks_of);
    int32_t *seg_lo = (int32_t *)(b1 + w1.seg_lo);
    uint64_t *val = (uint64_t *)(b1 + w1.val), *val_s = (uint64_t *)(b1 + w1.val_s);
    const int64_t n = ix->n_pairs;
    const unsigned gN = (unsigned)((n + 255) / 256);
    MM_HIP(ctx, hipMemsetAsync(key, 0, (size_t)n * 4, st));
    MM_HIP(ctx, hipMemsetAsync(val, 0, (size_t)n * 8, st));
    MM_LAUNCH(ctx, "idx_emit_kernel", idx_emit_kernel, dim3(gO), dim3(256), 0, ix->fi, ix->pi, (const int32_t *)ix->pt_ptr, O,
              (const int64_t *)offs, ix->cam_span, n, key, val, (const int64_t *)ix->head);
    size_t tb = w1.tmp_bytes;
    MM_HIP(ctx, rocprim::radix_sort_pairs((void *)(b1 + w1.tmp), tb, (const int32_t *)key, key_s, (const uint64_t *)val, val_s, (size_t)n,
                                          0u, (unsigned)key_bits, st));
    MM_LAUNCH(ctx, "idx_unpack_kernel", idx_unpack_kernel, dim3(gN), dim3(256), 0, (const uint64_t *)val_s, ix->pi, n, O, ix->pair_o,
              ix->pair_o2, ix->pair_p);
    tb = w1.tmp_bytes;
    MM_HIP(ctx, rocprim::run_length_encode((void *)(b1 + w1.tmp), tb, (const int32_t *)key_s, (size_t)n, ix->seg_ids, counts, n_seg, st));
    MM_LAUNCH(ctx, "idx_segcount_kernel", idx_segcount_kernel, dim3((unsigned)((seg_cap + 1 + 255) / 256)), dim3(256), 0,
              (const int32_t *)counts, (const int32_t *)n_seg, seg_cap, ix->chunk, pairs_of, chunks_of);
    tb = w1.tmp_bytes;
    MM_HIP(ctx, rocprim::exclusive_scan((void *)(b1 + w1.tmp), tb, (const int32_t *)pairs_of, seg_lo, (int32_t)0, (size_t)seg_cap + 1,
                                        rocprim::plus<int32_t>(), st));
    tb = w1.tmp_bytes;
    MM_HIP(ctx, rocprim::exclusive_scan((void *)(b1 + w1.tmp), tb, (const int32_t *)chunks_of, ix->seg_chunk_ptr, (int32_t)0,
                                        (size_t)seg_cap + 1, rocprim::plus<int32_t>(), st));
    MM_LAUNCH(ctx, "idx_chunks_kernel", idx_chunks_kernel, dim3((unsigned)((seg_cap * 64 + 255) / 256)), dim3(256), 0,
              (const int32_t *)n_seg, (const int32_t *)seg_lo, (const int32_t *)pairs_of, (const int32_t *)ix->seg_chunk_ptr, ix->chunk,
              chunk_cap, ix->chunk_seg, ix->chunk_begin, ix->chunk_end, ix->head);
    return MM_OK;
}

}
```

meatmodeler_amd/csrc/mm_common.h:

```cpp
#pragma once
#include <hip/hip_runtime.h>
#include <cstdarg>
#include <cstdio>
#include <cstring>
#include <vector>
#include "../../include/meatmodeler.h"

struct mm_prof_rec {
    const char *name;
    hipEvent_t a, b;
};

struct mm_ctx {
    int device;
    hipStream_t stream;
    char err[512];
    int prof = 0;
    char prof_only[64] = {0};
    std::vector<mm_prof_rec> recs;
    std::vector<hipEvent_t> pool;
    hipStream_t aux = nullptr;
    hipEvent_t ev_fork = nullptr, ev_join = nullptr;
    bool attr_chol_fused = false, attr_chol_bwd = false, attr_chol_batch = false;
    int cu_count = 0, fused_wgs = 0, chol_last_path = -1, debug_abandon = 0;
    bool chol_avoid_fused = false;
    bool chol_strict_budget = false;
    hipEvent_t fused_ev = nullptr;
    bool fused_ev_pending = false;
    bool fused_no_event = false;
    int link_last_variant = -1;
    void *cam_tab = nullptr;
    int cam_tab_cap = 0, cam_tab_F = 0;
    const double *cam_tab_for = nullptr;
    bool cam_tab_hold = false;
    const double *fx_cams = nullptr;
    int fx_F = 0;
    bool fx_tab_ok = false;
    void *host_board = nullptr;
    unsigned long long host_board_seq = 0;
    void *batch_dev = nullptr, *batch_host = nullptr;
    size_t batch_dev_cap = 0, batch_host_cap = 0;
    bool jvp_rows_deferred = false;
    const double *jvp_partial = nullptr;
    unsigned jvp_n_wg = 0;
    const void *chol_init_done = nullptr;
    int chol_init_sides = 0;
    int batch_last = -1;
};

struct mm_stream_swap {
    mm_ctx *c;
    hipStream_t saved;
    mm_stream_swap(mm_ctx *ctx, hipStream_t s) : c(ctx), saved(ctx->stream) { ctx->stream = s; }
    ~mm_stream_swap() { c->stream = saved; }
};

struct mm_fixed_scope {
    mm_ctx *c;
    mm_fixed_scope(mm_ctx *ctx, const mm_ba_fixed *fx) : c(ctx) {
        ctx->fx_cams = fx->cams;
        ctx->fx_F = fx->F_fixed;
        ctx->fx_tab_ok = false;
    }
    ~mm_fixed_scope() {
        c->fx_cams = nullptr;
        c->fx_F = 0;
        c->fx_tab_ok = false;
    }
};

int mm_cam_coef_table(mm_ctx *ctx, const double *cams, int F, const void **tab_out);
void mm_cam_table_hold(mm_ctx *ctx, bool on);
void mm_cam_table_invalidate(mm_ctx *ctx);

int mm_ba_residual_publish(mm_ctx *ctx, const mm_ba_problem *pb, const double *cams, const double *pts, void *ws,
                           size_t ws_bytes, double *board, int cost_slot, int count, void *host_board, unsigned long long seq);

int mm_trf_fused0_scaled(mm_ctx *ctx, const double *g, double *si, const double *B, const double *C, double *gh, double *ghs, int64_t n,
                         int64_t split, double *out, void *ws, size_t ws_bytes);
int mm_trf_fused5_coef(mm_ctx *ctx, const double *x, const double *s1, const double *s2, double *x_new, const double *h01, int64_t n,
                       int64_t split, void *ctab, int F);
int mm_trf_rows_step2d(mm_ctx *ctx, const double *partial, unsigned n_wg, double *rows, const double *r0, const double *d11,
                       const double *r1, const double *r2, const double *r3, const double *reg, const int32_t *info, double Delta,
                       double *board);
int mm_cam_table_adopt(mm_ctx *ctx, const double *cams, int F, void **tab_out);
int mm_ba_damp_damping(mm_ctx *ctx, int F, int P, const double *B, const double *C, const double *scale_inv, const double *gh2,
                       const double *d11, double Delta, double min_damping, double *damp_out, double *Bd, double *Cd);
void mm_chol_release_budget(mm_ctx *ctx);
bool mm_chol_fused_eligible(int n, int half_bandwidth);
struct mm_chol_geom {
    int n, nblk, bwb;
    int a, m, b;
    int pad;
};
struct mm_chol_layout {
    double *Linv, *ytmp, *contrib, *contrib_bwd, *lpub, *spub;
    int32_t *flags;
    mm_chol_geom g;
    uint64_t nflags, nsent, nlpub;
};
struct mm_chol_plan {
    mm_chol_layout lay;
    bool fused;
    int sides;
    unsigned grid_fused, grid_bwd;
};
struct mm_chol_init_args {
    int32_t *info, *flags;
    size_t nflags;
    unsigned long long *sentinel_buf;
    size_t nsent;
    unsigned long long *lpub;
    size_t nlpub;
    unsigned long long *Linv;
    size_t nblk;
};
bool mm_chol_init_plan(mm_ctx *ctx, int n, int half_bandwidth, int32_t *info, void *ws, size_t ws_bytes, mm_chol_init_args *out, int *sides, int *bwb);
void mm_chol_init_done(mm_ctx *ctx, const void *ws, int sides);
struct mm_damp_spec {
    const double *B, *C, *si;
    const double *gh2, *d11;
    double Delta, min_damping;
    double *damp_out;
    const double *reg;
};
int mm_ba_schur_solve_damped(mm_ctx *ctx, const mm_ba_problem *pb, const double *cams, const double *pts, const mm_damp_spec *dmp,
                             double *Bd, double *Cd, const double *gc, const double *gp, double *S, double *v, double *Cinv,
                             int half_bandwidth, int32_t *info, void *ws_schur, size_t ws_schur_bytes, void *ws_chol,
                             size_t ws_chol_bytes);
int mm_chol_solve_gated(mm_ctx *ctx, double *A, int n, double *b, int nrhs, int half_bandwidth, int32_t *info, void *ws,
                        size_t ws_bytes, const int32_t *slab_ready, int cams_per_slab, int n_cams, int sym_mode);

struct mm_batch_prob {
    mm_ba_problem pb;
    int64_t n, nc;
    double *x, *x_new, *g, *si, *gh, *ghs, *gn, *q1, *w, *q2, *s1, *s2;
    double *B, *Bd, *C, *Cd, *Cinv, *u1, *Jq2, *dp, *v, *S;
    double *r0, *r1, *r2, *r3, *d11, *bs, *damp, *board;
    int32_t *info;
    void *ctab_x, *ctab_new;
    double *res_partial;
    unsigned *md_counter;
    double *md_partial;
    double *jvp_partial;
    double *backsub_T;
    double *schur_partial, *schur_camtab;
    int32_t *schur_seg_done, *schur_desc;
    mm_chol_layout chol;
    int32_t half_bw, chol_sym_mirror;
    uint32_t g_vec, g_res, g_jvp, g_pblk, g_obs, g_pts, g_scale, g_damp, g_prep, g_pairs, g_chol, g_bwd, g_coef, g_zero;
    void *mailbox;
};
struct mm_batch_dyn {
    double Delta;
    unsigned long long seq;
    double min_damping;
    double reg;
};

int mm_batch_fused(mm_ctx *ctx, int op, const mm_batch_prob *tab, const int32_t *list, int n_list, unsigned max_g);
unsigned mm_batch_fused_grid(int64_t n);
int mm_batch_scale_update(mm_ctx *ctx, const mm_batch_prob *tab, const int32_t *list, int n_list, unsigned max_g);
int mm_batch_damp(mm_ctx *ctx, const mm_batch_prob *tab, const int32_t *list, int n_list, unsigned max_g);
int mm_batch_accept(mm_ctx *ctx, const mm_batch_prob *tab, const int32_t *list, int n_list, unsigned max_g);
int mm_batch_step2d(mm_ctx *ctx, const mm_batch_prob *tab, const int32_t *list, int n_list, const mm_batch_dyn *dyn);
void mm_batch_ba_setup(mm_batch_prob *bp);
int mm_batch_cam_coef(mm_ctx *ctx, const mm_batch_prob *tab, const int32_t *list, int n_list, unsigned max_g, int which );
int mm_batch_jvp_dots(mm_ctx *ctx, const mm_batch_prob *tab, const int32_t *list, int n_list, unsigned max_g, int second);
int mm_batch_damping(mm_ctx *ctx, const mm_batch_prob *tab, const int32_t *list, int n_list, const mm_batch_dyn *dyn);
int mm_batch_set_reg(mm_ctx *ctx, const mm_batch_prob *tab, const int32_t *list, int n_list, const mm_batch_dyn *dyn);
int mm_batch_backsub(mm_ctx *ctx, const mm_batch_prob *tab, const int32_t *list, int n_list, unsigned max_g_obs, unsigned max_g_pts);
int mm_batch_residual_publish(mm_ctx *ctx, const mm_batch_prob *tab, const int32_t *list, int n_list, unsigned max_g,
                              const mm_batch_dyn *dyn);
int mm_batch_normal_eq(mm_ctx *ctx, const mm_batch_prob *tab, const int32_t *list, int n_list, unsigned max_g_pblk, unsigned max_F);
int mm_batch_publish_rows(mm_ctx *ctx, const mm_batch_prob *tab, const int32_t *list, int n_list, const mm_batch_dyn *dyn);
int mm_batch_schur_setup(mm_ctx *ctx, mm_batch_prob *bp, void *ws_schur, size_t ws_schur_bytes);
int mm_batch_schur(mm_ctx *ctx, const mm_batch_prob *tab, const int32_t *list, int n_list, unsigned max_g_zero, unsigned max_g_prep,
                   unsigned max_g_pairs);
int mm_batch_chol_setup(mm_ctx *ctx, mm_batch_prob *bp, void *ws_chol, size_t ws_chol_bytes);
int mm_batch_chol(mm_ctx *ctx, const mm_batch_prob *tab, const int32_t *list, int n_list, unsigned max_g_chol, unsigned max_g_bwd);

static inline hipEvent_t mm_prof_event(mm_ctx *c) {
    hipEvent_t e = nullptr;
    if (!c->pool.empty()) {
        e = c->pool.back();
        c->pool.pop_back();
    } else {
        (void)hipEventCreate(&e);
    }
    return e;
}

#define MM_LAUNCH(ctx, name, kernel, grid, block, shmem, ...)                                          \
    do {                                                                                               \
        hipEvent_t ea_ = nullptr, eb_ = nullptr;                                                       \
        const dim3 g_ = (grid);                                                                        \
        const bool p_ = (ctx)->prof == 1 || ((ctx)->prof == 2 && (size_t)g_.x * g_.y * g_.z >= 64) || \
                        ((ctx)->prof == 3 && strcmp(name, (ctx)->prof_only) == 0);                      \
        if (p_) {                                                                                      \
            ea_ = mm_prof_event(ctx);                                                                  \
            eb_ = mm_prof_event(ctx);                                                                  \
            (void)hipEventRecord(ea_, (ctx)->stream);                                                  \
        }                                                                                              \
        hipLaunchKernelGGL(kernel, g_, block, shmem, (ctx)->stream, __VA_ARGS__);                      \
        if (p_) {                                                                                      \
            (void)hipEventRecord(eb_, (ctx)->stream);                                                  \
            (ctx)->recs.push_back(mm_prof_rec{name, ea_, eb_});                                        \
        }                                                                                              \
        MM_LAUNCH_CHECK(ctx, name);                                                                    \
    } while (0)

static inline int mm_fail(mm_ctx *ctx, int code, const char *fmt, ...) {
    if (ctx) {
        va_list ap;
        va_start(ap, fmt);
        vsnprintf(ctx->err, sizeof(ctx->err), fmt, ap);
        va_end(ap);
    }
    return code;
}

#define MM_HIP(ctx, call)                                                                              \
    do {                                                                                               \
        hipError_t e_ = (call);                                                                        \
        if (e_ != hipSuccess)                                                                          \
            return mm_fail(ctx, MM_ERR_HIP, "%s failed: %s (%s:%d)", #call, hipGetErrorString(e_),    \
                           __FILE__, __LINE__);                                                        \
    } while (0)

#define MM_LAUNCH_CHECK(ctx, name)                                                                     \
    do {                                                                                               \
        hipError_t e_ = hipGetLastError();                                                             \
        if (e_ != hipSuccess)                                                                          \
            return mm_fail(ctx, MM_ERR_HIP, "launch of %s failed: %s", name, hipGetErrorString(e_));   \
    } while (0)

static inline size_t mm_align_up(size_t x, size_t a) { return (x + a - 1) / a * a; }
```

meatmodeler_amd/csrc/trf.hip:

```cpp
#include "mm_common.h"
#include "trf_decide.h"
#include <chrono>
#include <vector>
#include <algorithm>
#include <initializer_list>
#include <utility>
#include <cmath>
#include <cstdlib>

namespace {

__global__ __launch_bounds__(256) void vec_mul_kernel(const double *__restrict__ a, const double *__restrict__ b,
                                                      double *__restrict__ out, int64_t n) {
    const int64_t i = (int64_t)blockIdx.x * 256 + threadIdx.x;
    if (i < n) out[i] = a[i] * b[i];
}

struct HostBoard {
    double v[16];
    unsigned long long seq;
    unsigned long long pad[7];
};

__global__ __launch_bounds__(64) void board_publish_kernel(const double *__restrict__ dev, int count, HostBoard *hb,
                                                          unsigned long long seq) {
    if ((int)threadIdx.x < count) hb->v[threadIdx.x] = dev[threadIdx.x];
    __threadfence_system();
    __builtin_amdgcn_wave_barrier();
    if (threadIdx.x == 0) __hip_atomic_store(&hb->seq, seq, __ATOMIC_RELEASE, __HIP_MEMORY_SCOPE_SYSTEM);
}

constexpr int EX_MAX_ITEMS = 12, EX_SCALARS = 64, EX_MAX_WORLD = 16;
struct ExItems {
    double *p[EX_MAX_ITEMS];
    int kind[EX_MAX_ITEMS];
    int n, rank, world;
    const int32_t *info;
};
__global__ __launch_bounds__(64) void ex_pack_kernel(ExItems it, double *__restrict__ ex) {
    const int t = threadIdx.x;
    double v = 0.0;
    if (t < it.n) {
        const double *r = it.p[t];
        const int k = it.kind[t];
        if (k == 0) v = it.rank == 0 ? r[0] + r[1] : r[1];
        else if (k == 1) v = r[2];
        else if (k == 3) v = r[0];
    }
    ex[t] = v;
    __syncthreads();
    if (t == 0) {
        int slot = 16;
        for (int i = 0; i < it.n; ++i) {
            if (it.kind[i] == 2) { ex[slot + it.rank] = it.p[i][1]; slot += EX_MAX_WORLD; }
            if (it.kind[i] == 4) { ex[slot + it.rank] = it.info[0] < 0 ? 1.0 : 0.0; slot += EX_MAX_WORLD; }
        }
    }
}
__global__ __launch_bounds__(64) void ex_unpack_kernel(ExItems it, const double *__restrict__ ex) {
    const int t = threadIdx.x;
    if (t < it.n) {
        double *r = it.p[t];
        const int k = it.kind[t];
        if (k == 0 || k == 1) r[2] = ex[t];
        else if (k == 3) r[0] = ex[t];
    }
    if (t == 0) {
        int slot = 16;
        for (int i = 0; i < it.n; ++i) {
            if (it.kind[i] == 2) {
                double m = it.p[i][0];
                for (int q = 0; q < it.world; ++q) m = fmax(m, ex[slot + q]);
                it.p[i][2] = m;
                slot += EX_MAX_WORLD;
            }
            if (it.kind[i] == 4) {
                double sum = 0.0;
                for (int q = 0; q < it.world; ++q) sum += ex[slot + q];
                it.p[i][0] = sum;
                slot += EX_MAX_WORLD;
            }
        }
    }
}
__global__ __launch_bounds__(256) void band_pack_kernel(const double *__restrict__ S, int64_t n, int hb, double *__restrict__ band) {
    const int64_t i = (int64_t)blockIdx.x * 256 + threadIdx.x, total = n * (hb + 1);
    if (i >= total) return;
    const int64_t j = i / (hb + 1), k = i % (hb + 1);
    band[i] = j + k < n ? S[(j + k) * n + j] : 0.0;
}
__global__ __launch_bounds__(256) void band_unpack_kernel(double *__restrict__ S, int64_t n, int hb, const double *__restrict__ band,
                                                          const double *__restrict__ Bd, double dup) {
    const int64_t i = (int64_t)blockIdx.x * 256 + threadIdx.x, total = n * (hb + 1);
    if (i >= total) return;
    const int64_t j = i / (hb + 1), k = i % (hb + 1), row = j + k;
    if (row >= n) return;
    double v = band[i];
    if (row / 6 == j / 6) v -= dup * Bd[(j / 6) * 36 + (row % 6) * 6 + j % 6];
    S[row * n + j] = v;
}
__global__ __launch_bounds__(256) void dedup_dense_kernel(double *__restrict__ S, int64_t n, const double *__restrict__ Bd, double dup) {
    const int64_t i = (int64_t)blockIdx.x * 256 + threadIdx.x;
    if (i >= n * 6) return;
    const int64_t f = i / 36, a = (i % 36) / 6, b = i % 6;
    S[(6 * f + a) * n + 6 * f + b] -= dup * Bd[i];
}
__global__ __launch_bounds__(256) void axpy_kernel(double *__restrict__ y, const double *__restrict__ x, double a, int64_t n) {
    const int64_t i = (int64_t)blockIdx.x * 256 + threadIdx.x;
    if (i < n) y[i] += a * x[i];
}

struct Carve {
    char *p;
    size_t used = 0;
    explicit Carve(void *base) : p((char *)base) {}
    template <class T>
    T *take(size_t count) {
        T *r = p ? (T *)(p + used) : nullptr;
        used += mm_align_up(count * sizeof(T), 256);
        return r;
    }
};

struct TrfWs {
    double *x, *x_new, *g, *si, *gh, *ghs, *gn, *q1, *w, *q2, *s1, *s2;
    double *B, *Bd, *C, *Cd, *Cinv, *u1, *Jq2, *dp, *v, *S;
    double *r0, *r1, *r2, *r3, *d11, *bs, *damp, *board, *cost2, *rowsx;
    int32_t *info;
    void *ws_res, *ws_md, *ws_jvp, *ws_schur, *ws_chol, *ws_back;
    size_t ws_res_b, ws_md_b, ws_jvp_b, ws_schur_b, ws_chol_b, ws_back_b;
    double *exs, *ex;
    size_t ex_count;
    size_t total;
};

TrfWs carve_trf(const mm_ba_problem *pb, void *base, int64_t ex_half_bw = -1) {
    TrfWs t;
    Carve c(base);
    const size_t F = pb->F, P = pb->P, O = (size_t)pb->O, n = 6 * F + 3 * P, nc = 6 * F;
    double **vecs[12] = {&t.x, &t.x_new, &t.g, &t.si, &t.gh, &t.ghs, &t.gn, &t.q1, &t.w, &t.q2, &t.s1, &t.s2};
    for (auto v : vecs) *v = c.take<double>(n + 2);
    t.B = c.take<double>(F * 36);
    t.Bd = c.take<double>(F * 36);
    t.C = c.take<double>(P * 6 + 2);
    t.Cd = c.take<double>(P * 6 + 2);
    t.Cinv = c.take<double>(P * 6 + 2);
    t.u1 = c.take<double>(O * 2 + 2);
    t.Jq2 = c.take<double>(O * 2 + 2);
    t.dp = c.take<double>(P * 3 + 2);
    t.v = c.take<double>(nc + 2);
    t.S = c.take<double>(2 * nc * nc + 2);
    t.r0 = c.take<double>(6);
    t.r1 = c.take<double>(9);
    t.r2 = c.take<double>(6);
    t.r3 = c.take<double>(18);
    t.d11 = c.take<double>(6);
    t.bs = c.take<double>(6);
    t.damp = c.take<double>(2);
    t.board = c.take<double>(16);
    t.cost2 = c.take<double>(1);
    t.rowsx = c.take<double>(3);
    t.info = c.take<int32_t>(1);
    t.ws_res_b = 2048 * 8;
    t.ws_res = c.take<char>(t.ws_res_b);
    t.ws_md_b = mm_multi_dot_workspace_bytes();
    t.ws_md = c.take<char>(t.ws_md_b);
    t.ws_jvp_b = mm_ba_jvp_dots_workspace_bytes(pb);
    t.ws_jvp = c.take<char>(t.ws_jvp_b);
    t.ws_schur_b = mm_ba_schur_workspace_bytes(pb);
    if (t.ws_schur_b < 256) t.ws_schur_b = 256;
    t.ws_schur = c.take<char>(t.ws_schur_b);
    t.ws_chol_b = mm_chol_workspace_bytes((int)nc);
    t.ws_chol = c.take<char>(t.ws_chol_b);
    t.ws_back_b = mm_ba_backsub_workspace_bytes(pb);
    t.ws_back = c.take<char>(t.ws_back_b);
    t.exs = nullptr;
    t.ex = nullptr;
    t.ex_count = 0;
    if (ex_half_bw >= 0) {
        const size_t hb = (size_t)(ex_half_bw < (int64_t)nc - 1 ? ex_half_bw : (nc ? nc - 1 : 0));
        t.ex_count = nc * (hb + 1) + nc;
        if (t.ex_count < F * 42) t.ex_count = F * 42;
        t.exs = c.take<double>(EX_SCALARS);
        t.ex = c.take<double>(t.ex_count + 2);
    }
    t.total = c.used;
    return t;
}

int wait_seq(mm_ctx *ctx, const unsigned long long *word, unsigned long long seq, const char *what, int problem = -1) {
    const auto t0 = std::chrono::steady_clock::now();
    unsigned long spins = 0;
    while (__atomic_load_n(word, __ATOMIC_ACQUIRE) != seq) {
        __builtin_ia32_pause();
        if ((++spins & 0xFFFFF) == 0 && std::chrono::steady_clock::now() - t0 > std::chrono::seconds(20)) {
            MM_HIP(ctx, hipStreamSynchronize(ctx->stream));
            if (__atomic_load_n(word, __ATOMIC_ACQUIRE) == seq) break;
            if (problem < 0) return mm_fail(ctx, MM_ERR_HIP, "%s never arrived", what);
            return mm_fail(ctx, MM_ERR_HIP, "%s %d never arrived", what, problem);
        }
    }
    return MM_OK;
}

using namespace mm_trf;

}

extern "C" size_t mm_ba_trf_workspace_bytes(const mm_ba_problem *pb) {
    if (!pb || pb->F < 0 || pb->P < 0 || pb->O < 0) return 0;
    return carve_trf(pb, nullptr).total;
}

#define TRF_CALL(expr)        \
    do {                      \
        int rc_ = (expr);     \
        if (rc_) return rc_;  \
    } while (0)

extern "C" size_t mm_ba_trf_dist_workspace_bytes(const mm_ba_problem *pb, int half_bandwidth) {
    if (!pb || pb->F < 0 || pb->P < 0 || pb->O < 0 || half_bandwidth < 0) return 0;
    return carve_trf(pb, nullptr, half_bandwidth).total;
}

static int trf_run(mm_ctx *ctx, const mm_ba_problem *pb, double *cams, double *pts, const mm_trf_params *prm, mm_trf_report *rep,
                   mm_trf_row *log, int log_cap, void *ws, size_t ws_bytes, const mm_dist *dist) {
    const auto t_enter = std::chrono::steady_clock::now();
    if (!ctx) return MM_ERR_ARG;
    if (!pb || !cams || !pts || !prm || !rep || pb->F <= 0 || pb->P < 0 || pb->O < 0 || !pb->K || log_cap < 0 || (log_cap > 0 && !log))
        return mm_fail(ctx, MM_ERR_ARG, "mm_ba_trf: bad argument");
    if (dist && (dist->world < 1 || dist->world > EX_MAX_WORLD || dist->rank < 0 || dist->rank >= dist->world || !dist->allreduce ||
                 dist->half_bandwidth < 0))
        return mm_fail(ctx, MM_ERR_ARG, "mm_ba_trf_dist: bad communicator description (1 <= world <= %d)", EX_MAX_WORLD);
    const size_t need = dist ? mm_ba_trf_dist_workspace_bytes(pb, dist->half_bandwidth) : mm_ba_trf_workspace_bytes(pb);
    if (!ws || ws_bytes < need || ((uintptr_t)ws & 255))
        return mm_fail(ctx, MM_ERR_WORKSPACE, "mm_ba_trf: workspace too small or misaligned");
    const TrfWs t = carve_trf(pb, ws, dist ? dist->half_bandwidth : -1);
    struct TableHold {
        mm_ctx *c;
        explicit TableHold(mm_ctx *ctx) : c(ctx) { mm_cam_table_hold(c, true); }
        ~TableHold() { mm_cam_table_hold(c, false); }
    } table_hold(ctx);
    struct FusedGuard {
        mm_ctx *c;
        bool saved, saved_strict, saved_no_event;
        FusedGuard(mm_ctx *ctx, bool sharded)
            : c(ctx), saved(ctx->chol_avoid_fused), saved_strict(ctx->chol_strict_budget), saved_no_event(ctx->fused_no_event) {
            c->fused_no_event = true;
            if (sharded) c->chol_strict_budget = true;
        }
        ~FusedGuard() {
            c->chol_avoid_fused = saved;
            c->chol_strict_budget = saved_strict;
            c->fused_no_event = saved_no_event;
            mm_chol_release_budget(c);
        }
    } fused_guard(ctx, dist != nullptr);
    const int F = pb->F, P = pb->P;
    const int64_t nc = 6 * (int64_t)F, n = nc + 3 * (int64_t)P;
    hipStream_t st = ctx->stream;
    auto pts_of = [&](double *v) { return v + nc; };
    MM_HIP(ctx, hipMemsetAsync(t.ws_md, 0, t.ws_md_b, st));
    MM_HIP(ctx, hipMemsetAsync(t.ws_jvp, 0, t.ws_jvp_b, st));
    MM_HIP(ctx, hipMemsetAsync(t.S, 0, (size_t)(2 * nc * nc) * sizeof(double), st));
    double *x = t.x, *x_new = t.x_new;
    MM_HIP(ctx, hipMemcpyAsync(x, cams, (size_t)nc * sizeof(double), hipMemcpyDeviceToDevice, st));
    if (P) MM_HIP(ctx, hipMemcpyAsync(x + nc, pts, (size_t)3 * P * sizeof(double), hipMemcpyDeviceToDevice, st));
    double host[16];
    rep->chol_fallbacks = 0;
    rep->collectives = 0;
    auto ar = [&](double *buf, int64_t count) -> int {
        ++rep->collectives;
        const int rc = dist->allreduce(dist->user, buf, count);
        return rc ? mm_fail(ctx, MM_ERR_HIP, "mm_ba_trf_dist: the all-reduce callback failed (%d)", rc) : MM_OK;
    };
    auto exchange = [&](std::initializer_list<std::pair<double *, int>> items) -> int {
        if (!dist) return MM_OK;
        ExItems it = {};
        it.rank = dist->rank;
        it.world = dist->world;
        it.info = t.info;
        for (auto &pr : items) {
            it.p[it.n] = pr.first;
            it.kind[it.n] = pr.second;
            ++it.n;
        }
        hipLaunchKernelGGL(ex_pack_kernel, dim3(1), dim3(64), 0, st, it, t.exs);
        TRF_CALL(ar(t.exs, EX_SCALARS));
        hipLaunchKernelGGL(ex_unpack_kernel, dim3(1), dim3(64), 0, st, it, (const double *)t.exs);
        MM_LAUNCH_CHECK(ctx, "ex_unpack_kernel");
        return MM_OK;
    };
    auto normal_eq = [&](double *v) -> int {
        TRF_CALL(mm_ba_normal_eq(ctx, pb, v, pts_of(v), t.B, t.g, t.C, pts_of(t.g)));
        if (!dist) return MM_OK;
        MM_HIP(ctx, hipMemcpyAsync(t.ex, t.B, (size_t)F * 36 * sizeof(double), hipMemcpyDeviceToDevice, st));
        MM_HIP(ctx, hipMemcpyAsync(t.ex + (size_t)F * 36, t.g, (size_t)nc * sizeof(double), hipMemcpyDeviceToDevice, st));
        TRF_CALL(ar(t.ex, (int64_t)F * 42));
        MM_HIP(ctx, hipMemcpyAsync(t.B, t.ex, (size_t)F * 36 * sizeof(double), hipMemcpyDeviceToDevice, st));
        MM_HIP(ctx, hipMemcpyAsync(t.g, t.ex + (size_t)F * 36, (size_t)nc * sizeof(double), hipMemcpyDeviceToDevice, st));
        return MM_OK;
    };
    if (!ctx->host_board) {
        MM_HIP(ctx, hipHostMalloc(&ctx->host_board, sizeof(HostBoard), hipHostMallocDefault));
        memset(ctx->host_board, 0, sizeof(HostBoard));
        ctx->host_board_seq = 0;
    }
    HostBoard *hb = (HostBoard *)ctx->host_board;
    auto take_board = [&](unsigned long long seq, int count) -> int {
        TRF_CALL(wait_seq(ctx, &hb->seq, seq, "mm_ba_trf: the trial-step scalars"));
        for (int i = 0; i < count; ++i) host[i] = ((volatile double *)hb->v)[i];
        mm_chol_release_budget(ctx);
        return MM_OK;
    };
    auto read_board = [&](const double *dev, int count) -> int {
        const unsigned long long seq = ++ctx->host_board_seq;
        hipLaunchKernelGGL(board_publish_kernel, dim3(1), dim3(64), 0, st, dev, count, hb, seq);
        MM_LAUNCH_CHECK(ctx, "board_publish_kernel");
        return take_board(seq, count);
    };
    TRF_CALL(mm_ba_residual(ctx, pb, x, pts_of(x), nullptr, t.cost2, t.ws_res, t.ws_res_b));
    if (dist) {
        const double av = ctx->chol_avoid_fused ? 1.0 : 0.0;
        MM_HIP(ctx, hipMemcpyAsync(t.board + 15, &av, sizeof(double), hipMemcpyHostToDevice, st));
        MM_HIP(ctx, hipStreamSynchronize(st));
        TRF_CALL(exchange({{t.cost2, 3}, {t.board + 15, 3}}));
        TRF_CALL(read_board(t.board + 15, 1));
        if (host[0] > 0) ctx->chol_avoid_fused = true;
    }
    TRF_CALL(read_board(t.cost2, 1));
    const double cost0 = 0.5 * host[0];
    rep->cost0 = cost0;
    if (!std::isfinite(cost0)) {
        rep->status = -2;
        return mm_fail(ctx, MM_ERR_NUMERIC, "mm_ba_trf: residuals are not finite in the initial point");
    }
    const int half_bw = dist ? dist->half_bandwidth : 6 * pb->cam_span + 5;
    TRF_CALL(normal_eq(x));
    TRF_CALL(mm_ba_scale_update(ctx, F, P, t.B, t.C, t.si, 1));
    {
        hipLaunchKernelGGL(vec_mul_kernel, dim3((unsigned)((n + 255) / 256)), dim3(256), 0, st, (const double *)x, (const double *)t.si, t.w, n);
        const double *pa[1] = {t.w}, *pbv[1] = {t.w};
        TRF_CALL(mm_multi_dot(ctx, 1, pa, pbv, n, nc, t.rowsx, t.ws_md, t.ws_md_b));
        TRF_CALL(exchange({{t.rowsx, 0}}));
        TRF_CALL(read_board(t.rowsx, 3));
    }
    TrfDecide d(cost0, host[2], n, *prm, log, log_cap);
    Outcome next = d.begin();
    static const bool timing = getenv("MM_TRF_TIMING") && atoi(getenv("MM_TRF_TIMING")) > 0;
    const auto t_loop = std::chrono::steady_clock::now();
    auto t_iter = t_loop;
    if (timing) fprintf(stderr, "mm_ba_trf timing: prologue %.1f us\n", std::chrono::duration<double, std::micro>(t_loop - t_enter).count());
    for (;;) {
        if (timing && d.iteration > 0) {
            const auto now = std::chrono::steady_clock::now();
            fprintf(stderr, "mm_ba_trf timing: iteration %d %.1f us (nfev %d)\n", d.iteration - 1,
                    std::chrono::duration<double, std::micro>(now - t_iter).count(), d.nfev);
            t_iter = now;
        }
        if (!dist && d.iteration > 0) {
            TRF_CALL(mm_trf_fused0_scaled(ctx, t.g, t.si, t.B, t.C, t.gh, t.ghs, n, nc, t.r0, t.ws_md, t.ws_md_b));
        } else {
            const double *in[2] = {t.g, t.si};
            double *outv[2] = {t.gh, t.ghs};
            TRF_CALL(mm_trf_fused(ctx, 0, in, outv, nullptr, 0, 0, n, nc, t.r0, t.ws_md, t.ws_md_b));
        }
        TRF_CALL(mm_ba_jvp_dots(ctx, pb, x, pts_of(x), t.ghs, pts_of(t.ghs), t.u1, nullptr, t.d11, t.ws_jvp, t.ws_jvp_b));
        TRF_CALL(exchange({{t.r0, 0}, {t.r0 + 3, 2}, {t.d11, 1}, {t.d11 + 3, 1}}));
        if (next == FINAL) {
            TRF_CALL(read_board(t.r0, 6));
            d.on_final(host[5]);
            break;
        }
        double *reg_eff = t.damp + 1;
        bool rows_pending = false;
        auto trial = [&](double Delta_) -> int {
            if (rows_pending) {
                rows_pending = false;
                TRF_CALL(mm_trf_rows_step2d(ctx, ctx->jvp_partial, ctx->jvp_n_wg, t.bs, t.r0, t.d11, t.r1, t.r2, t.r3, reg_eff, t.info, Delta_,
                                            t.board));
            } else {
                TRF_CALL(mm_trf_step2d(ctx, t.r0, t.d11, t.r1, t.r2, t.r3, t.bs, reg_eff, t.info, Delta_, t.board));
            }
            if (F > 0 && !dist) {
                void *ctab = nullptr;
                TRF_CALL(mm_cam_table_adopt(ctx, x_new, (int)F, &ctab));
                TRF_CALL(mm_trf_fused5_coef(ctx, x, t.s1, t.s2, x_new, t.board, n, nc, ctab, (int)F));
            } else {
                const double *in[3] = {x, t.s1, t.s2};
                double *outv[1] = {x_new};
                const double *sc[1] = {t.board};
                TRF_CALL(mm_trf_fused(ctx, 5, in, outv, sc, 0, 0, n, nc, nullptr, t.ws_md, t.ws_md_b));
                mm_cam_table_invalidate(ctx);
            }
            if (!dist) {
                const unsigned long long seq = ++ctx->host_board_seq;
                TRF_CALL(mm_ba_residual_publish(ctx, pb, x_new, pts_of(x_new), t.ws_res, t.ws_res_b, t.board, 14, 16,
                                                ctx->host_board, seq));
                return take_board(seq, 16);
            }
            TRF_CALL(mm_ba_residual(ctx, pb, x_new, pts_of(x_new), nullptr, t.board + 14, t.ws_res, t.ws_res_b));
            TRF_CALL(exchange({{t.board + 14, 3}, {t.board + 15, 4}}));
            return read_board(t.board, 16);
        };
        bool damping_known = false;
        Outcome solve;
        do {
            if (!dist) {
                mm_damp_spec dmp = {t.B, t.C, t.si, nullptr, nullptr, d.Delta, d.min_damping, t.damp, reg_eff};
                if (!damping_known) {
                    dmp.gh2 = t.r0 + 2;
                    dmp.d11 = t.d11 + 2;
                    damping_known = true;
                }
                TRF_CALL(mm_ba_schur_solve_damped(ctx, pb, x, pts_of(x), &dmp, t.Bd, t.Cd, t.g, pts_of(t.g), t.S, t.v, t.Cinv,
                                                  half_bw, t.info, t.ws_schur, t.ws_schur_b, t.ws_chol, t.ws_chol_b));
            } else {
                if (!damping_known) {
                    TRF_CALL(mm_ba_damp_damping(ctx, F, P, t.B, t.C, t.si, t.r0 + 2, t.d11 + 2, d.Delta, d.min_damping, t.damp, t.Bd, t.Cd));
                    damping_known = true;
                } else {
                    TRF_CALL(mm_ba_damp(ctx, F, P, t.B, t.C, t.si, reg_eff, t.Bd, t.Cd));
                }
                TRF_CALL(mm_ba_schur(ctx, pb, x, pts_of(x), t.Bd, t.Cd, t.g, pts_of(t.g), t.S, t.v, t.Cinv, t.ws_schur,
                                     t.ws_schur_b));
                const double dup = (double)(dist->world - 1);
                if (dist->band_exchange) {
                    const int hb = (int)(half_bw < nc - 1 ? half_bw : nc - 1);
                    const int64_t cnt = nc * (hb + 1);
                    hipLaunchKernelGGL(band_pack_kernel, dim3((unsigned)((cnt + 255) / 256)), dim3(256), 0, st, (const double *)t.S, nc, hb, t.ex);
                    MM_HIP(ctx, hipMemcpyAsync(t.ex + cnt, t.v, (size_t)nc * sizeof(double), hipMemcpyDeviceToDevice, st));
                    TRF_CALL(ar(t.ex, cnt + nc));
                    hipLaunchKernelGGL(band_unpack_kernel, dim3((unsigned)((cnt + 255) / 256)), dim3(256), 0, st, t.S, nc, hb,
                                       (const double *)t.ex, (const double *)t.Bd, dup);
                    MM_HIP(ctx, hipMemcpyAsync(t.v, t.ex + cnt, (size_t)nc * sizeof(double), hipMemcpyDeviceToDevice, st));
                } else {
                    MM_HIP(ctx, hipMemcpyAsync(t.S + nc * nc, t.v, (size_t)nc * sizeof(double), hipMemcpyDeviceToDevice, st));
                    TRF_CALL(ar(t.S, nc * nc + nc));
                    MM_HIP(ctx, hipMemcpyAsync(t.v, t.S + nc * nc, (size_t)nc * sizeof(double), hipMemcpyDeviceToDevice, st));
                    hipLaunchKernelGGL(dedup_dense_kernel, dim3((unsigned)((nc * 6 + 255) / 256)), dim3(256), 0, st, t.S, nc,
                                       (const double *)t.Bd, dup);
                }
                hipLaunchKernelGGL(axpy_kernel, dim3((unsigned)((nc + 255) / 256)), dim3(256), 0, st, t.v, (const double *)t.g, -dup, nc);
                MM_LAUNCH_CHECK(ctx, "axpy_kernel");
                TRF_CALL(mm_chol_solve_sym(ctx, t.S, (int)nc, t.v, half_bw, dist->band_exchange ? 0 : 1, t.info, t.ws_chol, t.ws_chol_b));
            }
            TRF_CALL(mm_ba_backsub(ctx, pb, x, pts_of(x), t.Cinv, pts_of(t.g), t.v, t.dp, t.ws_back, t.ws_back_b));
            {
                const double *in[4] = {t.v, t.dp, t.si, t.gh};
                double *outv[2] = {t.gn, t.q1};
                const double *sc[1] = {t.r0 + 2};
                TRF_CALL(mm_trf_fused(ctx, 1, in, outv, sc, 0, 0, n, nc, t.r1, t.ws_md, t.ws_md_b));
                TRF_CALL(exchange({{t.r1, 0}, {t.r1 + 3, 0}}));
            }
            {
                const double *in[2] = {t.gn, t.q1};
                double *outv[1] = {t.w};
                const double *sc[1] = {t.r1 + 2};
                TRF_CALL(mm_trf_fused(ctx, 2, in, outv, sc, 0, 0, n, nc, t.r2, t.ws_md, t.ws_md_b));
                TRF_CALL(exchange({{t.r2, 0}}));
            }
            {
                const double *in[5] = {t.w, t.q1, t.si, t.gh, x};
                double *outv[3] = {t.q2, t.s1, t.s2};
                const double *sc[1] = {t.r2 + 2};
                TRF_CALL(mm_trf_fused(ctx, 3, in, outv, sc, 0, 0, n, nc, t.r3, t.ws_md, t.ws_md_b));
            }
            ctx->jvp_rows_deferred = !dist && P > 0 && pb->O > 0;
            {
                const int rc_ = mm_ba_jvp_dots(ctx, pb, x, pts_of(x), t.s2, pts_of(t.s2), t.Jq2, t.u1, t.bs, t.ws_jvp, t.ws_jvp_b);
                rows_pending = ctx->jvp_rows_deferred;
                ctx->jvp_rows_deferred = false;
                if (rc_) return rc_;
            }
            TRF_CALL(exchange({{t.r3, 0}, {t.r3 + 3, 0}, {t.r3 + 6, 0}, {t.r3 + 9, 0}, {t.r3 + 12, 0}, {t.bs, 1}, {t.bs + 3, 1}}));
            TRF_CALL(trial(d.Delta));
            solve = d.on_solve(dist && host[15] > 0 ? -1 : (int)host[6], host[13], host[10], host[9]);
            if (solve == ABANDONED) {
                if (ctx->chol_avoid_fused) return mm_fail(ctx, MM_ERR_HIP, "mm_ba_trf: the banded factorisation reported info = -1");
                ctx->chol_avoid_fused = true;
                ++rep->chol_fallbacks;
            } else if (solve == RETRY) {
                MM_HIP(ctx, hipMemcpyAsync(t.damp + 1, &d.reg, sizeof(double), hipMemcpyHostToDevice, st));
                MM_HIP(ctx, hipStreamSynchronize(st));
            }
        } while (solve == ABANDONED || solve == RETRY);
        if (solve == INDEFINITE)
            return mm_fail(ctx, MM_ERR_NUMERIC, "mm_ba_trf: reduced camera system is not positive definite (pivot %d)", (int)host[6]);
        if (solve == DONE) break;
        while ((next = d.on_trial(host[2], host[3], host[4], host[14])) == TRIAL) TRF_CALL(trial(d.Delta));
        if (d.accepted) {
            std::swap(x, x_new);
            TRF_CALL(normal_eq(x));
            if (dist) TRF_CALL(mm_ba_scale_update(ctx, F, P, t.B, t.C, t.si, 0));
        }
    }
    MM_HIP(ctx, hipMemcpyAsync(cams, x, (size_t)nc * sizeof(double), hipMemcpyDeviceToDevice, st));
    if (P) MM_HIP(ctx, hipMemcpyAsync(pts, x + nc, (size_t)3 * P * sizeof(double), hipMemcpyDeviceToDevice, st));
    MM_HIP(ctx, hipStreamSynchronize(st));
    if (timing) fprintf(stderr, "mm_ba_trf timing: total %.1f us, %d iterations\n",
                        std::chrono::duration<double, std::micro>(std::chrono::steady_clock::now() - t_enter).count(), d.iteration);
    d.fill(*rep);
    return MM_OK;
}

extern "C" int mm_ba_trf(mm_ctx *ctx, const mm_ba_problem *pb, double *cams, double *pts, const mm_trf_params *prm,
                         mm_trf_report *rep, mm_trf_row *log, int log_cap, void *ws, size_t ws_bytes) {
    return trf_run(ctx, pb, cams, pts, prm, rep, log, log_cap, ws, ws_bytes, nullptr);
}

extern "C" int mm_ba_trf_dist(mm_ctx *ctx, const mm_ba_problem *pb, double *cams, double *pts, const mm_trf_params *prm,
                              mm_trf_report *rep, mm_trf_row *log, int log_cap, void *ws, size_t ws_bytes, const mm_dist *dist) {
    if (!dist) return mm_fail(ctx, MM_ERR_ARG, "mm_ba_trf_dist: null communicator description");
    return trf_run(ctx, pb, cams, pts, prm, rep, log, log_cap, ws, ws_bytes, dist);
}

extern "C" size_t mm_ba_trf_fixed_workspace_bytes(const mm_ba_problem *pb, const mm_ba_fixed *fx) {
    (void)fx;
    return mm_ba_trf_workspace_bytes(pb);
}

extern "C" int mm_ba_trf_fixed(mm_ctx *ctx, const mm_ba_problem *pb, const mm_ba_fixed *fx, double *cams, double *pts,
                               const mm_trf_params *prm, mm_trf_report *rep, mm_trf_row *log, int log_cap, void *ws, size_t ws_bytes) {
    if (!ctx) return MM_ERR_ARG;
    if (!fx || fx->F_fixed == 0) return trf_run(ctx, pb, cams, pts, prm, rep, log, log_cap, ws, ws_bytes, nullptr);
    if (fx->F_fixed < 0 || !fx->cams) return mm_fail(ctx, MM_ERR_ARG, "mm_ba_trf_fixed: bad fixed-camera descriptor");
    if (pb && pb->O > 0 && pb->n_chunks <= 0) return mm_fail(ctx, MM_ERR_ARG, "mm_ba_trf_fixed: the problem needs its co-observation pair list");
    mm_fixed_scope scope(ctx, fx);
    return trf_run(ctx, pb, cams, pts, prm, rep, log, log_cap, ws, ws_bytes, nullptr);
}

namespace {
size_t batch_tables_bytes(const mm_ba_problem *pb) { return 2 * mm_align_up((size_t)pb->F * 5 * sizeof(double), 256); }
}

extern "C" size_t mm_ba_trf_batched_workspace_bytes(const mm_ba_problem *pb) {
    if (!pb || pb->F < 0 || pb->P < 0 || pb->O < 0) return 0;
    return carve_trf(pb, nullptr).total + batch_tables_bytes(pb);
}

extern "C" int mm_ba_trf_batched(mm_ctx *ctx, int n_prob, const mm_ba_problem *const *pbs, double *const *cams, double *const *pts,
                                 const mm_trf_params *prm, mm_trf_report *reports, void *const *ws, const size_t *ws_bytes,
                                 int32_t *solved_alone) {
    if (!ctx) return MM_ERR_ARG;
    if (n_prob < 0 || (n_prob > 0 && (!pbs || !cams || !pts || !prm || !reports || !ws || !ws_bytes)))
        return mm_fail(ctx, MM_ERR_ARG, "mm_ba_trf_batched: bad argument");
    if (n_prob == 0) return MM_OK;
    hipStream_t st = ctx->stream;
    for (int p = 0; p < n_prob; ++p) {
        const mm_ba_problem *pb = pbs[p];
        if (!pb || !cams[p] || !pts[p] || pb->F <= 0 || pb->P < 0 || pb->O < 0 || !pb->K)
            return mm_fail(ctx, MM_ERR_ARG, "mm_ba_trf_batched: bad problem %d", p);
        if (!ws[p] || ws_bytes[p] < mm_ba_trf_batched_workspace_bytes(pb) || ((uintptr_t)ws[p] & 255))
            return mm_fail(ctx, MM_ERR_WORKSPACE, "mm_ba_trf_batched: workspace of problem %d too small or misaligned", p);
        if (solved_alone) solved_alone[p] = 0;
    }
    auto solve_alone = [&](int p) -> int {
        if (solved_alone) solved_alone[p] = 1;
        return trf_run(ctx, pbs[p], cams[p], pts[p], prm, &reports[p], nullptr, 0, ws[p], ws_bytes[p], nullptr);
    };
    std::vector<mm_batch_prob> tab((size_t)n_prob);
    std::vector<TrfWs> tws((size_t)n_prob);
    bool batchable = n_prob > 1;
    for (int p = 0; p < n_prob && batchable; ++p) {
        const mm_ba_problem *pb = pbs[p];
        const TrfWs t = carve_trf(pb, ws[p]);
        tws[p] = t;
        mm_batch_prob &b = tab[p];
        memset(&b, 0, sizeof(b));
        b.pb = *pb;
        b.nc = 6 * (int64_t)pb->F;
        b.n = b.nc + 3 * (int64_t)pb->P;
        b.x = t.x; b.x_new = t.x_new; b.g = t.g; b.si = t.si; b.gh = t.gh; b.ghs = t.ghs; b.gn = t.gn; b.q1 = t.q1; b.w = t.w;
        b.q2 = t.q2; b.s1 = t.s1; b.s2 = t.s2;
        b.B = t.B; b.Bd = t.Bd; b.C = t.C; b.Cd = t.Cd; b.Cinv = t.Cinv; b.u1 = t.u1; b.Jq2 = t.Jq2; b.dp = t.dp; b.v = t.v; b.S = t.S;
        b.r0 = t.r0; b.r1 = t.r1; b.r2 = t.r2; b.r3 = t.r3; b.d11 = t.d11; b.bs = t.bs; b.damp = t.damp; b.board = t.board;
        b.info = t.info;
        char *extra = (char *)ws[p] + t.total;
        b.ctab_x = extra;
        b.ctab_new = extra + mm_align_up((size_t)pb->F * 5 * sizeof(double), 256);
        b.res_partial = (double *)t.ws_res;
        b.md_counter = (unsigned *)t.ws_md;
        b.md_partial = (double *)((char *)t.ws_md + 256);
        b.jvp_partial = (double *)((char *)t.ws_jvp + 256);
        b.backsub_T = (double *)t.ws_back;
        b.half_bw = 6 * pb->cam_span + 5;
        b.g_vec = mm_batch_fused_grid(b.n);
        b.g_scale = (uint32_t)((b.n + 255) / 256);
        b.g_damp = (uint32_t)(((int64_t)pb->F * 36 + (int64_t)pb->P * 6 + 255) / 256);
        mm_batch_ba_setup(&b);
        if (pb->O <= 0 || pb->P <= 0 || mm_batch_schur_setup(ctx, &b, t.ws_schur, t.ws_schur_b) != MM_OK ||
            mm_batch_chol_setup(ctx, &b, t.ws_chol, t.ws_chol_b) != MM_OK)
            batchable = false;
    }
    ctx->batch_last = batchable ? n_prob : 0;
    if (!batchable) {
        if (getenv("MM_BATCH_DEBUG")) fprintf(stderr, "mm_ba_trf_batched: %d problems one by one (%s)\n", n_prob, n_prob > 1 ? ctx->err : "a single problem");
        for (int p = 0; p < n_prob; ++p) TRF_CALL(solve_alone(p));
        return MM_OK;
    }
    const size_t tab_b = mm_align_up((size_t)n_prob * sizeof(mm_batch_prob), 256), dyn_b = mm_align_up((size_t)n_prob * sizeof(mm_batch_dyn), 256);
    const size_t list_b = mm_align_up((size_t)n_prob * sizeof(int32_t), 256);
    constexpr int N_LISTS = 7;
    const size_t dev_need = tab_b + dyn_b + N_LISTS * list_b;
    const size_t host_need = dyn_b + N_LISTS * list_b + (size_t)n_prob * sizeof(HostBoard) + (size_t)n_prob * 4 * sizeof(double);
    if (ctx->batch_dev_cap < dev_need) {
        if (ctx->batch_dev) (void)hipFree(ctx->batch_dev);
        ctx->batch_dev = nullptr;
        ctx->batch_dev_cap = 0;
        MM_HIP(ctx, hipMalloc(&ctx->batch_dev, dev_need));
        ctx->batch_dev_cap = dev_need;
    }
    if (ctx->batch_host_cap < host_need) {
        if (ctx->batch_host) (void)hipHostFree(ctx->batch_host);
        ctx->batch_host = nullptr;
        ctx->batch_host_cap = 0;
        MM_HIP(ctx, hipHostMalloc(&ctx->batch_host, host_need, hipHostMallocDefault));
        ctx->batch_host_cap = host_need;
    }
    char *dbase = (char *)ctx->batch_dev, *hbase = (char *)ctx->batch_host;
    mm_batch_prob *d_tab = (mm_batch_prob *)dbase;
    mm_batch_dyn *d_dyn = (mm_batch_dyn *)(dbase + tab_b);
    int32_t *d_list[N_LISTS];
    for (int q = 0; q < N_LISTS; ++q) d_list[q] = (int32_t *)(dbase + tab_b + dyn_b + q * list_b);
    mm_batch_dyn *h_dyn = (mm_batch_dyn *)hbase;
    int32_t *h_list[N_LISTS];
    for (int q = 0; q < N_LISTS; ++q) h_list[q] = (int32_t *)(hbase + dyn_b + q * list_b);
    HostBoard *mail = (HostBoard *)(hbase + dyn_b + N_LISTS * list_b);
    double *h_init = (double *)(mail + n_prob);
    memset(mail, 0, (size_t)n_prob * sizeof(HostBoard));
    for (int p = 0; p < n_prob; ++p) tab[p].mailbox = &mail[p];
    MM_HIP(ctx, hipMemcpyAsync(d_tab, tab.data(), (size_t)n_prob * sizeof(mm_batch_prob), hipMemcpyHostToDevice, st));
    for (int p = 0; p < n_prob; ++p) {
        const mm_ba_problem *pb = pbs[p];
        const TrfWs &t = tws[p];
        const int64_t nc = tab[p].nc, n = tab[p].n;
        MM_HIP(ctx, hipMemsetAsync(t.ws_md, 0, t.ws_md_b, st));
        MM_HIP(ctx, hipMemsetAsync(t.ws_jvp, 0, t.ws_jvp_b, st));
        MM_HIP(ctx, hipMemcpyAsync(t.x, cams[p], (size_t)nc * sizeof(double), hipMemcpyDeviceToDevice, st));
        MM_HIP(ctx, hipMemcpyAsync(t.x + nc, pts[p], (size_t)3 * pb->P * sizeof(double), hipMemcpyDeviceToDevice, st));
        TRF_CALL(mm_ba_residual(ctx, pb, t.x, t.x + nc, nullptr, t.cost2, t.ws_res, t.ws_res_b));
        TRF_CALL(mm_ba_normal_eq(ctx, pb, t.x, t.x + nc, t.B, t.g, t.C, t.g + nc));
        TRF_CALL(mm_ba_scale_update(ctx, pb->F, pb->P, t.B, t.C, t.si, 1));
        hipLaunchKernelGGL(vec_mul_kernel, dim3((unsigned)((n + 255) / 256)), dim3(256), 0, st, (const double *)t.x, (const double *)t.si, t.w, n);
        const double *pa[1] = {t.w}, *pbv[1] = {t.w};
        TRF_CALL(mm_multi_dot(ctx, 1, pa, pbv, n, nc, t.rowsx, t.ws_md, t.ws_md_b));
        MM_HIP(ctx, hipMemcpyAsync(h_init + 4 * p, t.cost2, sizeof(double), hipMemcpyDeviceToHost, st));
        MM_HIP(ctx, hipMemcpyAsync(h_init + 4 * p + 1, t.rowsx, 3 * sizeof(double), hipMemcpyDeviceToHost, st));
    }
    MM_HIP(ctx, hipStreamSynchronize(st));
    std::vector<TrfDecide> D;
    std::vector<Outcome> next((size_t)n_prob);
    D.reserve((size_t)n_prob);
    for (int p = 0; p < n_prob; ++p) {
        const double cost0 = 0.5 * h_init[4 * p];
        if (!std::isfinite(cost0)) {
            reports[p].status = -2;
            return mm_fail(ctx, MM_ERR_NUMERIC, "mm_ba_trf_batched: residuals of problem %d are not finite in the initial point", p);
        }
        D.emplace_back(cost0, h_init[4 * p + 3], tab[p].n, *prm);
        next[p] = D[p].begin();
    }
    auto upload_lists = [&]() -> int {
        MM_HIP(ctx, hipMemcpyAsync(d_dyn, h_dyn, (size_t)n_prob * sizeof(mm_batch_dyn), hipMemcpyHostToDevice, st));
        MM_HIP(ctx, hipMemcpyAsync(d_list[0], h_list[0], (N_LISTS - 1) * list_b, hipMemcpyHostToDevice, st));
        return MM_OK;
    };
    auto max_of = [&](const int32_t *list, int cnt, uint32_t mm_batch_prob::*field) {
        uint32_t m = 1;
        for (int q = 0; q < cnt; ++q) m = std::max(m, tab[list[q]].*field);
        return m;
    };
    {
        for (int p = 0; p < n_prob; ++p) h_list[2][p] = p;
        TRF_CALL(upload_lists());
        TRF_CALL(mm_batch_cam_coef(ctx, d_tab, d_list[2], n_prob, max_of(h_list[2], n_prob, &mm_batch_prob::g_coef), 0));
    }
    for (unsigned long long round = 1;; ++round) {
        int n_f0 = 0, n_final = 0, n_body = 0, n_trial = 0, n_all = 0, n_retry = 0;
        for (int p = 0; p < n_prob; ++p) {
            const Outcome w = next[p];
            if (w == DONE || w == ABANDONED || w == INDEFINITE) continue;
            h_dyn[p].Delta = D[p].Delta;
            h_dyn[p].seq = round;
            h_dyn[p].min_damping = D[p].min_damping;
            h_dyn[p].reg = D[p].reg;
            if (w == BODY || w == FINAL) h_list[0][n_f0++] = p;
            if (w == FINAL) h_list[1][n_final++] = p;
            if (w == BODY) h_list[2][n_body++] = p;
            if (w != FINAL) h_list[3][n_trial++] = p;
            if (w == BODY || w == RETRY) h_list[4][n_all++] = p;
            if (w == RETRY) h_list[5][n_retry++] = p;
        }
        if (n_f0 + n_trial == 0) break;
        TRF_CALL(upload_lists());
        TRF_CALL(mm_batch_fused(ctx, 0, d_tab, d_list[0], n_f0, max_of(h_list[0], n_f0, &mm_batch_prob::g_vec)));
        TRF_CALL(mm_batch_publish_rows(ctx, d_tab, d_list[1], n_final, d_dyn));
        if (n_body) {
            TRF_CALL(mm_batch_jvp_dots(ctx, d_tab, d_list[2], n_body, max_of(h_list[2], n_body, &mm_batch_prob::g_jvp), 0));
            TRF_CALL(mm_batch_damping(ctx, d_tab, d_list[2], n_body, d_dyn));
        }
        TRF_CALL(mm_batch_set_reg(ctx, d_tab, d_list[5], n_retry, d_dyn));
        if (n_all) {
            const int32_t *L = d_list[4];
            const int32_t *H = h_list[4];
            const uint32_t gv = max_of(H, n_all, &mm_batch_prob::g_vec);
            TRF_CALL(mm_batch_damp(ctx, d_tab, L, n_all, max_of(H, n_all, &mm_batch_prob::g_damp)));
            TRF_CALL(mm_batch_schur(ctx, d_tab, L, n_all, max_of(H, n_all, &mm_batch_prob::g_zero), max_of(H, n_all, &mm_batch_prob::g_prep),
                                    max_of(H, n_all, &mm_batch_prob::g_pairs)));
            TRF_CALL(mm_batch_chol(ctx, d_tab, L, n_all, max_of(H, n_all, &mm_batch_prob::g_chol), max_of(H, n_all, &mm_batch_prob::g_bwd)));
            TRF_CALL(mm_batch_backsub(ctx, d_tab, L, n_all, max_of(H, n_all, &mm_batch_prob::g_obs), max_of(H, n_all, &mm_batch_prob::g_pts)));
            TRF_CALL(mm_batch_fused(ctx, 1, d_tab, L, n_all, gv));
            TRF_CALL(mm_batch_fused(ctx, 2, d_tab, L, n_all, gv));
            TRF_CALL(mm_batch_fused(ctx, 3, d_tab, L, n_all, gv));
            TRF_CALL(mm_batch_jvp_dots(ctx, d_tab, L, n_all, max_of(H, n_all, &mm_batch_prob::g_jvp), 1));
        }
        if (n_trial) {
            const int32_t *L = d_list[3];
            TRF_CALL(mm_batch_step2d(ctx, d_tab, L, n_trial, d_dyn));
            TRF_CALL(mm_batch_fused(ctx, 5, d_tab, L, n_trial, max_of(h_list[3], n_trial, &mm_batch_prob::g_vec)));
            TRF_CALL(mm_batch_cam_coef(ctx, d_tab, L, n_trial, max_of(h_list[3], n_trial, &mm_batch_prob::g_coef), 1));
            TRF_CALL(mm_batch_residual_publish(ctx, d_tab, L, n_trial, max_of(h_list[3], n_trial, &mm_batch_prob::g_res), d_dyn));
        }
        int n_accept = 0;
        for (int q = 0; q < n_final; ++q) {
            const int p = h_list[1][q];
            TRF_CALL(wait_seq(ctx, &mail[p].seq, round, "mm_ba_trf_batched: the scalars of problem", p));
            next[p] = D[p].on_final(((volatile double *)mail[p].v)[5]);
        }
        for (int q = 0; q < n_trial; ++q) {
            const int p = h_list[3][q];
            TrfDecide &d = D[p];
            TRF_CALL(wait_seq(ctx, &mail[p].seq, round, "mm_ba_trf_batched: the scalars of problem", p));
            double host[16];
            for (int i = 0; i < 16; ++i) host[i] = ((volatile double *)mail[p].v)[i];
            if (next[p] != TRIAL) {
                next[p] = d.on_solve((int)host[6], host[13], host[10], host[9]);
                if (next[p] != USABLE) continue;
            }
            next[p] = d.on_trial(host[2], host[3], host[4], host[14]);
            if (next[p] != TRIAL && d.accepted) h_list[6][n_accept++] = p;
        }
        if (n_accept) {
            MM_HIP(ctx, hipMemcpyAsync(d_list[6], h_list[6], (size_t)n_accept * sizeof(int32_t), hipMemcpyHostToDevice, st));
            const int32_t *L = d_list[6];
            TRF_CALL(mm_batch_accept(ctx, d_tab, L, n_accept, max_of(h_list[6], n_accept, &mm_batch_prob::g_vec)));
            TRF_CALL(mm_batch_normal_eq(ctx, d_tab, L, n_accept, max_of(h_list[6], n_accept, &mm_batch_prob::g_pblk),
                                        [&] { int m = 1; for (int q = 0; q < n_accept; ++q) m = std::max(m, tab[h_list[6][q]].pb.F); return (unsigned)m; }()));
            TRF_CALL(mm_batch_scale_update(ctx, d_tab, L, n_accept, max_of(h_list[6], n_accept, &mm_batch_prob::g_scale)));
        }
    }
    for (int p = 0; p < n_prob; ++p) {
        if (next[p] != DONE) continue;
        const int64_t nc = tab[p].nc;
        MM_HIP(ctx, hipMemcpyAsync(cams[p], tws[p].x, (size_t)nc * sizeof(double), hipMemcpyDeviceToDevice, st));
        MM_HIP(ctx, hipMemcpyAsync(pts[p], tws[p].x + nc, (size_t)3 * pbs[p]->P * sizeof(double), hipMemcpyDeviceToDevice, st));
        mm_trf_report &r = reports[p];
        D[p].fill(r);
        r.log_rows = 0;
        r.chol_fallbacks = 0;
        r.collectives = 0;
    }
    MM_HIP(ctx, hipStreamSynchronize(st));
    for (int p = 0; p < n_prob; ++p)
        if (next[p] != DONE) {
            --ctx->batch_last;
            TRF_CALL(solve_alone(p));
        }
    return MM_OK;
}
```

Measured before the change: 9053 billion descriptor pairs/s (match stage).

## Speculate normal equations on trial step and reorder points for locality

```diff
diff --git a/include/meatmodeler.h b/include/meatmodeler.h
--- a/include/meatmodeler.h
+++ b/include/meatmodeler.h
@@ -292,6 +292,16 @@
                          size_t ws_bytes);
 int mm_ba_normal_eq_fixed(mm_ctx *ctx, const mm_ba_problem *pb, const mm_ba_fixed *fx, const double *cams, const double *pts,
                           double *B, double *gc, double *C, double *gp);
+int mm_ba_backsub_fixed(mm_ctx *ctx, const mm_ba_problem *pb, const mm_ba_fixed *fx, const double *cams, const double *pts,
+                        const double *Cinv, const double *gp, const double *dc , double *dp, void *ws ,
+                        size_t ws_bytes);
+int mm_ba_normal_eq_gated(mm_ctx *ctx, const mm_ba_problem *pb, const mm_ba_fixed *fx , const double *cams,
+                          const double *pts, double *B, double *gc, double *C, double *gp, const int32_t *go );
+int mm_trf_trial_flag(mm_ctx *ctx, const double *partial , int n, double cost, const int32_t *info ,
+                      double *board , int32_t *go );
+size_t mm_ba_point_order_workspace_bytes(mm_ctx *ctx, const mm_ba_problem *pb);
+int mm_ba_point_order(mm_ctx *ctx, const mm_ba_problem *pb, int32_t *order , void *ws , size_t ws_bytes);
+int mm_ba_point_order_set(mm_ctx *ctx, const int32_t *order , int P);
 size_t mm_ba_trf_fixed_workspace_bytes(const mm_ba_problem *pb, const mm_ba_fixed *fx);
 int mm_ba_trf_fixed(mm_ctx *ctx, const mm_ba_problem *pb, const mm_ba_fixed *fx, double *cams ,
                     double *pts , const mm_trf_params *prm, mm_trf_report *report ,
diff --git a/meatmodeler_amd/_lib.py b/meatmodeler_amd/_lib.py
--- a/meatmodeler_amd/_lib.py
+++ b/meatmodeler_amd/_lib.py
@@ -187,6 +187,12 @@
                                     C.POINTER(TrfParams), C.POINTER(TrfReport), C.POINTER(vp), C.POINTER(C.c_size_t), c_i32p]),
     "mm_ba_residual_fixed": (C.c_int, [vp, C.POINTER(BAProblem), C.POINTER(BAFixed), vp, vp, vp, vp, vp, C.c_size_t]),
     "mm_ba_normal_eq_fixed": (C.c_int, [vp, C.POINTER(BAProblem), C.POINTER(BAFixed), vp, vp, vp, vp, vp, vp]),
+    "mm_ba_backsub_fixed": (C.c_int, [vp, C.POINTER(BAProblem), C.POINTER(BAFixed), vp, vp, vp, vp, vp, vp, vp, C.c_size_t]),
+    "mm_ba_normal_eq_gated": (C.c_int, [vp, C.POINTER(BAProblem), C.POINTER(BAFixed), vp, vp, vp, vp, vp, vp, vp]),
+    "mm_trf_trial_flag": (C.c_int, [vp, vp, C.c_int, C.c_double, vp, vp, vp]),
+    "mm_ba_point_order_workspace_bytes": (C.c_size_t, [vp, C.POINTER(BAProblem)]),
+    "mm_ba_point_order": (C.c_int, [vp, C.POINTER(BAProblem), vp, vp, C.c_size_t]),
+    "mm_ba_point_order_set": (C.c_int, [vp, vp, C.c_int]),
     "mm_ba_trf_fixed_workspace_bytes": (C.c_size_t, [C.POINTER(BAProblem), C.POINTER(BAFixed)]),
     "mm_ba_trf_fixed": (C.c_int, [vp, C.POINTER(BAProblem), C.POINTER(BAFixed), vp, vp, C.POINTER(TrfParams),
                                   C.POINTER(TrfReport), C.POINTER(TrfRow), C.c_int, vp, C.c_size_t]),
diff --git a/meatmodeler_amd/csrc/ba.hip b/meatmodeler_amd/csrc/ba.hip
--- a/meatmodeler_amd/csrc/ba.hip
+++ b/meatmodeler_amd/csrc/ba.hip
@@ -54,9 +54,12 @@
     double v[16];
     unsigned long long seq;
 };
+constexpr int GO_SLOT = 15;
 __device__ __forceinline__ void sum_partials_publish_body(const double *__restrict__ partial, int n,
                                                                    double *__restrict__ board, int cost_slot, int count,
-                                                                   MMHostBoard *hb, unsigned long long seq, const unsigned bx, const unsigned gx) {
+                                                                   MMHostBoard *hb, unsigned long long seq, double cost,
+                                                                   const int32_t *__restrict__ info, int32_t *__restrict__ go,
+                                                                   const unsigned bx, const unsigned gx) {
     __shared__ double sm[4];
     double acc = 0;
     for (int i = threadIdx.x; i < n; i += 256) acc += partial[i];
@@ -64,7 +67,18 @@
     if (threadIdx.x == 0) board[cost_slot] = t;
     if (threadIdx.x < 64) {
         const double t0 = __shfl(t, 0, 64);
-        if ((int)threadIdx.x < count) hb->v[threadIdx.x] = (int)threadIdx.x == cost_slot ? t0 : board[threadIdx.x];
+        double flag = 0.0;
+        if (go) {
+            const double cost_new = 0.5 * t0;
+            const bool g = info[0] == 0 && isfinite(cost_new) && cost - cost_new > 0;
+            flag = g ? 1.0 : 0.0;
+            if (threadIdx.x == 0) {
+                go[0] = g ? 1 : 0;
+                board[GO_SLOT] = flag;
+            }
+        }
+        if ((int)threadIdx.x < count)
+            hb->v[threadIdx.x] = (int)threadIdx.x == cost_slot ? t0 : (go && (int)threadIdx.x == GO_SLOT ? flag : board[threadIdx.x]);
         __threadfence_system();
         __builtin_amdgcn_wave_barrier();
         if (threadIdx.x == 0) __hip_atomic_store(&hb->seq, seq, __ATOMIC_RELEASE, __HIP_MEMORY_SCOPE_SYSTEM);
@@ -72,7 +86,10 @@
 }
 __global__ __launch_bounds__(256) void sum_partials_publish_kernel(const double *__restrict__ partial, int n,
                                                                    double *__restrict__ board, int cost_slot, int count,
-                                                                   MMHostBoard *hb, unsigned long long seq) { sum_partials_publish_body(partial, n, board, cost_slot, count, hb, seq, blockIdx.x, gridDim.x); }
+                                                                   MMHostBoard *hb, unsigned long long seq, double cost,
+                                                                   const int32_t *__restrict__ info, int32_t *__restrict__ go) {
+    sum_partials_publish_body(partial, n, board, cost_slot, count, hb, seq, cost, info, go, blockIdx.x, gridDim.x);
+}
 
 __global__ __launch_bounds__(256) void ba_jacobian_kernel(mm_ba_problem pb, const double *__restrict__ cams,
                                                           const double *__restrict__ pts, const CamCoef *__restrict__ ctab, double *__restrict__ Jc,
@@ -105,13 +122,15 @@
 template <bool FIXED>
 __device__ __forceinline__ void ba_point_blocks_body(mm_ba_problem pb, const double *__restrict__ cams, const double *__restrict__ fxc,
                                                               const double *__restrict__ pts, const CamCoef *__restrict__ ctab, double *__restrict__ C,
-                                                              double *__restrict__ gp, const unsigned bx, const unsigned gx) {
+                                                              double *__restrict__ gp, const int32_t *__restrict__ order, const unsigned bx,
+                                                              const unsigned gx) {
     __shared__ double Ks[9];
     if (threadIdx.x < 9) Ks[threadIdx.x] = pb.K[threadIdx.x];
     __syncthreads();
     const int sub = threadIdx.x & (PB_LANES - 1);
-    const int p = bx * (256 / PB_LANES) + (threadIdx.x / PB_LANES);
-    const bool live = p < pb.P;
+    const int slot = bx * (256 / PB_LANES) + (threadIdx.x / PB_LANES);
+    const bool live = slot < pb.P;
+    const int p = live && order ? order[slot] : slot;
     double c[9] = {0, 0, 0, 0, 0, 0, 0, 0, 0};
     if (live) {
         const double *Xp = pts + (size_t)p * 3;
@@ -148,10 +167,10 @@
 }
 __global__ __launch_bounds__(256) void ba_point_blocks_kernel(mm_ba_problem pb, const double *__restrict__ cams,
                                                               const double *__restrict__ pts, const CamCoef *__restrict__ ctab, double *__restrict__ C,
-                                                              double *__restrict__ gp) { ba_point_blocks_body<false>(pb, cams, nullptr, pts, ctab, C, gp, blockIdx.x, gridDim.x); }
+                                                              double *__restrict__ gp, const int32_t *__restrict__ order) { ba_point_blocks_body<false>(pb, cams, nullptr, pts, ctab, C, gp, order, blockIdx.x, gridDim.x); }
 __global__ __launch_bounds__(256) void ba_point_blocks_fixed_kernel(mm_ba_problem pb, const double *__restrict__ cams, const double *__restrict__ fxc,
                                                                     const double *__restrict__ pts, const CamCoef *__restrict__ ctab, double *__restrict__ C,
-                                                                    double *__restrict__ gp) { ba_point_blocks_body<true>(pb, cams, fxc, pts, ctab, C, gp, blockIdx.x, gridDim.x); }
+                                                                    double *__restrict__ gp, const int32_t *__restrict__ order) { ba_point_blocks_body<true>(pb, cams, fxc, pts, ctab, C, gp, order, blockIdx.x, gridDim.x); }
 
 __device__ __forceinline__ void ba_camera_blocks_body(mm_ba_problem pb, const double *__restrict__ cams,
                                                                const double *__restrict__ pts, double *__restrict__ B,
@@ -204,15 +223,19 @@
 
 __global__ __launch_bounds__(256) void ba_normal_eq_kernel(mm_ba_problem pb, const double *__restrict__ cams, const double *__restrict__ pts,
                                                            const CamCoef *__restrict__ ctab, double *__restrict__ B, double *__restrict__ gc,
-                                                           double *__restrict__ C, double *__restrict__ gp) {
+                                                           double *__restrict__ C, double *__restrict__ gp, const int32_t *__restrict__ order,
+                                                           const int32_t *__restrict__ go) {
+    if (go && go[0] == 0) return;
     if ((int)blockIdx.x < pb.F) ba_camera_blocks_body(pb, cams, pts, B, gc, blockIdx.x, (unsigned)pb.F);
-    else ba_point_blocks_body<false>(pb, cams, nullptr, pts, ctab, C, gp, blockIdx.x - (unsigned)pb.F, gridDim.x - (unsigned)pb.F);
+    else ba_point_blocks_body<false>(pb, cams, nullptr, pts, ctab, C, gp, order, blockIdx.x - (unsigned)pb.F, gridDim.x - (unsigned)pb.F);
 }
 __global__ __launch_bounds__(256) void ba_normal_eq_fixed_kernel(mm_ba_problem pb, const double *__restrict__ cams, const double *__restrict__ fxc,
                                                                  const double *__restrict__ pts, const CamCoef *__restrict__ ctab, double *__restrict__ B,
-                                                                 double *__restrict__ gc, double *__restrict__ C, double *__restrict__ gp) {
+                                                                 double *__restrict__ gc, double *__restrict__ C, double *__restrict__ gp,
+                                                                 const int32_t *__restrict__ order, const int32_t *__restrict__ go) {
+    if (go && go[0] == 0) return;
     if ((int)blockIdx.x < pb.F) ba_camera_blocks_body(pb, cams, pts, B, gc, blockIdx.x, (unsigned)pb.F);
-    else ba_point_blocks_body<true>(pb, cams, fxc, pts, ctab, C, gp, blockIdx.x - (unsigned)pb.F, gridDim.x - (unsigned)pb.F);
+    else ba_point_blocks_body<true>(pb, cams, fxc, pts, ctab, C, gp, order, blockIdx.x - (unsigned)pb.F, gridDim.x - (unsigned)pb.F);
 }
 
 __global__ __launch_bounds__(256) void ba_jvp_kernel(mm_ba_problem pb, const double *__restrict__ cams,
@@ -373,10 +396,12 @@
 
 __device__ __forceinline__ void ba_backsub_points_body(mm_ba_problem pb, const double *__restrict__ T,
                                                                 const double *__restrict__ Cinv, const double *__restrict__ gp,
-                                                                double *__restrict__ dp, const unsigned bx, const unsigned gx) {
+                                                                double *__restrict__ dp, const int32_t *__restrict__ order, const unsigned bx,
+                                                                const unsigned gx) {
     const int sub = threadIdx.x & (PB_LANES - 1);
-    const int p = bx * (256 / PB_LANES) + (threadIdx.x / PB_LANES);
-    const bool live = p < pb.P;
+    const int slot = bx * (256 / PB_LANES) + (threadIdx.x / PB_LANES);
+    const bool live = slot < pb.P;
+    const int p = live && order ? order[slot] : slot;
     double t[3] = {0.0, 0.0, 0.0};
     if (live) {
         const int e_end = pb.pt_ptr[p + 1];
@@ -404,7 +429,7 @@
 }
 __global__ __launch_bounds__(256) void ba_backsub_points_kernel(mm_ba_problem pb, const double *__restrict__ T,
                                                                 const double *__restrict__ Cinv, const double *__restrict__ gp,
-                                                                double *__restrict__ dp) { ba_backsub_points_body(pb, T, Cinv, gp, dp, blockIdx.x, gridDim.x); }
+                                                                double *__restrict__ dp, const int32_t *__restrict__ order) { ba_backsub_points_body(pb, T, Cinv, gp, dp, order, blockIdx.x, gridDim.x); }
 
 __device__ __forceinline__ void cam_coef_body(const double *__restrict__ cams, int F, CamCoef *__restrict__ tab, const unsigned bx, const unsigned gx) {
     const int f = bx * 256 + threadIdx.x;
@@ -467,7 +492,7 @@
                                                                          const mm_batch_dyn *__restrict__ dyn) {
     const int pid = list[blockIdx.x];
     const mm_batch_prob &bp = tab[pid];
-    sum_partials_publish_body(bp.res_partial, (int)bp.g_res, bp.board, 14, 16, (MMHostBoard *)bp.mailbox, dyn[pid].seq, 0, 1);
+    sum_partials_publish_body(bp.res_partial, (int)bp.g_res, bp.board, 14, 16, (MMHostBoard *)bp.mailbox, dyn[pid].seq, 0.0, nullptr, nullptr, 0, 1);
 }
 __global__ __launch_bounds__(64) void publish_r0_batch_kernel(const mm_batch_prob *__restrict__ tab, const int32_t *__restrict__ list,
                                                               const mm_batch_dyn *__restrict__ dyn) {
@@ -506,14 +531,14 @@
 }
 __global__ __launch_bounds__(256) void ba_backsub_points_batch_kernel(const mm_batch_prob *__restrict__ tab, const int32_t *__restrict__ list) {
     MM_BATCH_PROB(g_pts);
-    ba_backsub_points_body(bp.pb, bp.backsub_T, bp.Cinv, bp.g + bp.nc, bp.dp, blockIdx.x, bp.g_pts);
+    ba_backsub_points_body(bp.pb, bp.backsub_T, bp.Cinv, bp.g + bp.nc, bp.dp, nullptr, blockIdx.x, bp.g_pts);
 }
 __global__ __launch_bounds__(256) void ba_normal_eq_batch_kernel(const mm_batch_prob *__restrict__ tab, const int32_t *__restrict__ list) {
     const mm_batch_prob &bp = tab[list[blockIdx.y]];
     const unsigned F = (unsigned)bp.pb.F;
     if (blockIdx.x < F) ba_camera_blocks_body(bp.pb, bp.x, bp.x + bp.nc, bp.B, bp.g, blockIdx.x, F);
     else if (blockIdx.x - F < bp.g_pblk)
-        ba_point_blocks_body<false>(bp.pb, bp.x, nullptr, bp.x + bp.nc, (const CamCoef *)bp.ctab_x, bp.C, bp.g + bp.nc, blockIdx.x - F, bp.g_pblk);
+        ba_point_blocks_body<false>(bp.pb, bp.x, nullptr, bp.x + bp.nc, (const CamCoef *)bp.ctab_x, bp.C, bp.g + bp.nc, nullptr, blockIdx.x - F, bp.g_pblk);
 }
 
 }
@@ -566,8 +591,6 @@
 }
 void mm_cam_table_invalidate(mm_ctx *ctx) { ctx->cam_tab_for = nullptr; }
 
-int mm_ba_residual_publish(mm_ctx *ctx, const mm_ba_problem *pb, const double *cams, const double *pts, void *ws,
-                           size_t ws_bytes, double *board, int cost_slot, int count, void *host_board, unsigned long long seq);
 
 #define MM_CAM_TABLE(ctx, pb, cams)                                               \
     const CamCoef *ctab = nullptr;                                                \
@@ -609,34 +632,37 @@
     return MM_OK;
 }
 
-int mm_ba_normal_eq(mm_ctx *ctx, const mm_ba_problem *pb, const double *cams, const double *pts, double *B, double *gc,
-                    double *C, double *gp) {
+static int normal_eq_run(mm_ctx *ctx, const mm_ba_problem *pb, const double *cams, const double *pts, double *B, double *gc,
+                         double *C, double *gp, const int32_t *go) {
     int rc = check_pb(ctx, pb, "mm_ba_normal_eq");
     if (rc) return rc;
     if (!cams || !pts) return mm_fail(ctx, MM_ERR_ARG, "mm_ba_normal_eq: null pointer");
     if ((B == nullptr) != (gc == nullptr) || (C == nullptr) != (gp == nullptr))
         return mm_fail(ctx, MM_ERR_ARG, "mm_ba_normal_eq: B/gc and C/gp come in pairs");
+    const int32_t *order = mm_pt_order_of(ctx, pb);
     if (B && C && pb->P > 0 && pb->F > 0) {
         if (!pb->pt_ptr || !pb->pt_obs || !pb->cam_ptr || !pb->cam_obs) return mm_fail(ctx, MM_ERR_ARG, "mm_ba_normal_eq: CSR missing");
         MM_CAM_TABLE(ctx, pb, cams);
         const unsigned g_pblk = (unsigned)((pb->P + 256 / PB_LANES - 1) / (256 / PB_LANES));
         if (ctx->fx_F > 0)
             MM_LAUNCH(ctx, "ba_normal_eq_fixed_kernel", ba_normal_eq_fixed_kernel, dim3((unsigned)pb->F + g_pblk), dim3(256), 0, *pb, cams,
-                      ctx->fx_cams, pts, ctab, B, gc, C, gp);
+                      ctx->fx_cams, pts, ctab, B, gc, C, gp, order, go);
         else
-            MM_LAUNCH(ctx, "ba_normal_eq_kernel", ba_normal_eq_kernel, dim3((unsigned)pb->F + g_pblk), dim3(256), 0, *pb, cams, pts, ctab, B, gc, C, gp);
+            MM_LAUNCH(ctx, "ba_normal_eq_kernel", ba_normal_eq_kernel, dim3((unsigned)pb->F + g_pblk), dim3(256), 0, *pb, cams, pts, ctab, B, gc,
+                      C, gp, order, go);
         return MM_OK;
     }
+    if (go) return mm_fail(ctx, MM_ERR_ARG, "mm_ba_normal_eq_gated: needs B, gc, C, gp and F, P > 0 (the merged launch)");
     if (C) {
         if (!pb->pt_ptr || !pb->pt_obs) return mm_fail(ctx, MM_ERR_ARG, "mm_ba_normal_eq: point CSR missing");
         if (pb->P > 0) {
             MM_CAM_TABLE(ctx, pb, cams);
             if (ctx->fx_F > 0)
                 MM_LAUNCH(ctx, "ba_point_blocks_fixed_kernel", ba_point_blocks_fixed_kernel, dim3((pb->P + 256 / PB_LANES - 1) / (256 / PB_LANES)),
-                          dim3(256), 0, *pb, cams, ctx->fx_cams, pts, ctab, C, gp);
+                          dim3(256), 0, *pb, cams, ctx->fx_cams, pts, ctab, C, gp, order);
             else
                 MM_LAUNCH(ctx, "ba_point_blocks_kernel", ba_point_blocks_kernel, dim3((pb->P + 256 / PB_LANES - 1) / (256 / PB_LANES)), dim3(256), 0,
-                          *pb, cams, pts, ctab, C, gp);
+                          *pb, cams, pts, ctab, C, gp, order);
         }
     }
     if (B) {
@@ -646,6 +672,21 @@
         }
     }
     return MM_OK;
+}
+
+int mm_ba_normal_eq(mm_ctx *ctx, const mm_ba_problem *pb, const double *cams, const double *pts, double *B, double *gc,
+                    double *C, double *gp) {
+    return normal_eq_run(ctx, pb, cams, pts, B, gc, C, gp, nullptr);
+}
+
+int mm_ba_normal_eq_gated(mm_ctx *ctx, const mm_ba_problem *pb, const mm_ba_fixed *fx, const double *cams, const double *pts,
+                          double *B, double *gc, double *C, double *gp, const int32_t *go) {
+    if (!ctx) return MM_ERR_ARG;
+    if (!go) return mm_fail(ctx, MM_ERR_ARG, "mm_ba_normal_eq_gated: null flag");
+    if (!fx || fx->F_fixed == 0) return normal_eq_run(ctx, pb, cams, pts, B, gc, C, gp, go);
+    if (fx->F_fixed < 0 || !fx->cams) return mm_fail(ctx, MM_ERR_ARG, "mm_ba_normal_eq_gated: bad fixed-camera descriptor");
+    mm_fixed_scope scope(ctx, fx);
+    return normal_eq_run(ctx, pb, cams, pts, B, gc, C, gp, go);
 }
 
 int mm_ba_jvp(mm_ctx *ctx, const mm_ba_problem *pb, const double *cams, const double *pts, const double *wc,
@@ -717,7 +758,7 @@
             MM_LAUNCH(ctx, "ba_backsub_kernel", ba_backsub_obs_kernel, dim3((unsigned)((pb->O + 255) / 256)), dim3(256), 0, *pb, cams, pts,
                       ctab, dc, (double *)ws);
         MM_LAUNCH(ctx, "ba_backsub_points_kernel", ba_backsub_points_kernel, dim3((pb->P + 256 / PB_LANES - 1) / (256 / PB_LANES)), dim3(256), 0,
-                  *pb, (const double *)ws, Cinv, gp, dp);
+                  *pb, (const double *)ws, Cinv, gp, dp, mm_pt_order_of(ctx, pb));
         return MM_OK;
     }
     MM_LAUNCH(ctx, "ba_backsub_kernel", ba_backsub_kernel, dim3((pb->P + 255) / 256), dim3(256), 0, *pb, cams, pts, ctab, Cinv, gp, dc, dp);
@@ -749,6 +790,16 @@
     return mm_ba_normal_eq(ctx, pb, cams, pts, B, gc, C, gp);
 }
 
+int mm_ba_backsub_fixed(mm_ctx *ctx, const mm_ba_problem *pb, const mm_ba_fixed *fx, const double *cams, const double *pts,
+                        const double *Cinv, const double *gp, const double *dc, double *dp, void *ws, size_t ws_bytes) {
+    if (!ctx) return MM_ERR_ARG;
+    if (!fx || fx->F_fixed == 0) return mm_ba_backsub(ctx, pb, cams, pts, Cinv, gp, dc, dp, ws, ws_bytes);
+    int rc = mm_ba_fixed_check(ctx, fx, "mm_ba_backsub_fixed");
+    if (rc) return rc;
+    mm_fixed_scope scope(ctx, fx);
+    return mm_ba_backsub(ctx, pb, cams, pts, Cinv, gp, dc, dp, ws, ws_bytes);
+}
+
 int mm_trf_damping(mm_ctx *ctx, const double *gh2, const double *d11, double Delta, double min_damping, double *out) {
     if (!ctx) return MM_ERR_ARG;
     if (!gh2 || !d11 || !out || !(Delta > 0.0)) return mm_fail(ctx, MM_ERR_ARG, "mm_trf_damping: bad argument");
@@ -758,8 +809,19 @@
 
 }
 
+int mm_sum_partials_publish(mm_ctx *ctx, const double *partial, int n, double *board, int cost_slot, int count, void *host_board,
+                            unsigned long long seq, const mm_trial_flag *flag) {
+    if (!partial || n < 0 || !board || !host_board || count > 16 || cost_slot >= count || (flag && (!flag->info || !flag->go || count <= GO_SLOT)))
+        return mm_fail(ctx, MM_ERR_ARG, "mm_sum_partials_publish: bad argument");
+    MM_LAUNCH(ctx, "sum_partials_kernel", sum_partials_publish_kernel, dim3(1), dim3(256), 0, partial, n, board, cost_slot, count,
+              (MMHostBoard *)host_board, seq, flag ? flag->cost : 0.0, flag ? flag->info : (const int32_t *)nullptr,
+              flag ? flag->go : (int32_t *)nullptr);
+    return MM_OK;
+}
+
 int mm_ba_residual_publish(mm_ctx *ctx, const mm_ba_problem *pb, const double *cams, const double *pts, void *ws,
-                           size_t ws_bytes, double *board, int cost_slot, int count, void *host_board, unsigned long long seq) {
+                           size_t ws_bytes, double *board, int cost_slot, int count, void *host_board, unsigned long long seq,
+                           const mm_trial_flag *flag) {
     int rc = check_pb(ctx, pb, "mm_ba_residual");
     if (rc) return rc;
     if (!cams || !pts || !board || !host_board || count > 16 || cost_slot >= count) return mm_fail(ctx, MM_ERR_ARG, "mm_ba_residual_publish: bad argument");
@@ -772,9 +834,7 @@
                   (double *)nullptr, (double *)ws);
     else
         MM_LAUNCH(ctx, "ba_residual_kernel", ba_residual_kernel, dim3(blocks), dim3(256), 0, *pb, cams, pts, ctab, (double *)nullptr, (double *)ws);
-    MM_LAUNCH(ctx, "sum_partials_kernel", sum_partials_publish_kernel, dim3(1), dim3(256), 0, (const double *)ws, blocks, board,
-              cost_slot, count, (MMHostBoard *)host_board, seq);
-    return MM_OK;
+    return mm_sum_partials_publish(ctx, (const double *)ws, blocks, board, cost_slot, count, host_board, seq, flag);
 }
 
 
diff --git a/meatmodeler_amd/csrc/ba_index.hip b/meatmodeler_amd/csrc/ba_index.hip
--- a/meatmodeler_amd/csrc/ba_index.hip
+++ b/meatmodeler_amd/csrc/ba_index.hip
@@ -196,6 +196,35 @@
     return hipSuccess;
 }
 
+__global__ __launch_bounds__(256) void pt_order_key_kernel(const int32_t *__restrict__ pt_ptr, int P, int lanes, uint32_t max_trips,
+                                                           uint32_t *__restrict__ key, int32_t *__restrict__ identity) {
+    const int p = blockIdx.x * 256 + threadIdx.x;
+    if (p >= P) return;
+    const int len = pt_ptr[p + 1] - pt_ptr[p];
+    const uint32_t trips = len > 0 ? (uint32_t)((len + lanes - 1) / lanes) : 0u;
+    key[p] = max_trips - (trips < max_trips ? trips : max_trips);
+    identity[p] = p;
+}
+constexpr int PT_ORDER_LANES = 4;
+uint32_t pt_order_max_trips(int64_t O) { return (uint32_t)((O + PT_ORDER_LANES - 1) / PT_ORDER_LANES); }
+struct WsOrder {
+    size_t key, key_s, identity, tmp, tmp_bytes, total;
+};
+hipError_t ws_order_layout(int P, int64_t O, hipStream_t st, WsOrder &w) {
+    size_t t_sort = 0;
+    hipError_t e = rocprim::radix_sort_pairs(nullptr, t_sort, (const uint32_t *)nullptr, (uint32_t *)nullptr, (const int32_t *)nullptr,
+                                             (int32_t *)nullptr, (size_t)P, 0u, (unsigned)bits_for((int64_t)pt_order_max_trips(O) + 1), st);
+    if (e != hipSuccess) return e;
+    Carve c;
+    w.key = c.take((size_t)P * 4);
+    w.key_s = c.take((size_t)P * 4);
+    w.identity = c.take((size_t)P * 4);
+    w.tmp_bytes = t_sort;
+    w.tmp = c.take(w.tmp_bytes);
+    w.total = c.at;
+    return hipSuccess;
+}
+
 bool index_args_ok(const mm_ba_index *ix) {
     return ix && ix->F > 0 && ix->P > 0 && ix->O > 0 && ix->O < 0x7fffffffLL && ix->fi && ix->pi && ix->head;
 }
@@ -206,7 +235,46 @@
 
 }
 
+size_t mm_pt_order_scratch_bytes(int P, int64_t O, hipStream_t st) {
+    if (P <= 0) return 0;
+    WsOrder w;
+    return ws_order_layout(P, O, st, w) == hipSuccess ? w.total : 0;
+}
+
 extern "C" {
+
+size_t mm_ba_point_order_workspace_bytes(mm_ctx *ctx, const mm_ba_problem *pb) {
+    if (!ctx || !pb || pb->P <= 0 || pb->O < 0) return 0;
+    return mm_pt_order_scratch_bytes(pb->P, pb->O, ctx->stream);
+}
+
+int mm_ba_point_order(mm_ctx *ctx, const mm_ba_problem *pb, int32_t *order, void *ws, size_t ws_bytes) {
+    if (!ctx) return MM_ERR_ARG;
+    if (!pb || pb->P < 0 || pb->O < 0 || (pb->P > 0 && (!pb->pt_ptr || !order)))
+        return mm_fail(ctx, MM_ERR_ARG, "mm_ba_point_order: bad argument");
+    if (pb->P == 0) return MM_OK;
+    WsOrder w;
+    MM_HIP(ctx, ws_order_layout(pb->P, pb->O, ctx->stream, w));
+    if (!ws || ws_bytes < w.total || ((uintptr_t)ws & 15)) return mm_fail(ctx, MM_ERR_WORKSPACE, "mm_ba_point_order: workspace too small or misaligned");
+    uint8_t *b = (uint8_t *)ws;
+    uint32_t *key = (uint32_t *)(b + w.key), *key_s = (uint32_t *)(b + w.key_s);
+    int32_t *identity = (int32_t *)(b + w.identity);
+    const uint32_t max_trips = pt_order_max_trips(pb->O);
+    MM_LAUNCH(ctx, "pt_order_key_kernel", pt_order_key_kernel, dim3((unsigned)((pb->P + 255) / 256)), dim3(256), 0, pb->pt_ptr, pb->P,
+              PT_ORDER_LANES, max_trips, key, identity);
+    size_t tb = w.tmp_bytes;
+    MM_HIP(ctx, rocprim::radix_sort_pairs((void *)(b + w.tmp), tb, (const uint32_t *)key, key_s, (const int32_t *)identity, order,
+                                          (size_t)pb->P, 0u, (unsigned)bits_for((int64_t)max_trips + 1), ctx->stream));
+    return MM_OK;
+}
+
+int mm_ba_point_order_set(mm_ctx *ctx, const int32_t *order, int P) {
+    if (!ctx) return MM_ERR_ARG;
+    if (P < 0 || (order && P == 0)) return mm_fail(ctx, MM_ERR_ARG, "mm_ba_point_order_set: bad argument");
+    ctx->pt_order = order;
+    ctx->pt_order_P = order ? P : 0;
+    return MM_OK;
+}
 
 int mm_ba_index_bounds(int F, int cam_span, int64_t n_pairs, int chunk, int64_t *seg_cap, int64_t *chunk_cap) {
     if (F <= 0 || cam_span < 0 || n_pairs < 0 || chunk <= 0 || !seg_cap || !chunk_cap) return MM_ERR_ARG;
diff --git a/meatmodeler_amd/csrc/mm_common.h b/meatmodeler_amd/csrc/mm_common.h
--- a/meatmodeler_amd/csrc/mm_common.h
+++ b/meatmodeler_amd/csrc/mm_common.h
@@ -46,7 +46,28 @@
     const void *chol_init_done = nullptr;
     int chol_init_sides = 0;
     int batch_last = -1;
-};
+    const int32_t *pt_order = nullptr;
+    int pt_order_P = 0;
+};
+
+struct mm_pt_order_scope {
+    mm_ctx *c;
+    const int32_t *saved;
+    int saved_P;
+    explicit mm_pt_order_scope(mm_ctx *ctx) : c(ctx), saved(ctx->pt_order), saved_P(ctx->pt_order_P) {}
+    void set(const int32_t *order, int P) {
+        c->pt_order = order;
+        c->pt_order_P = P;
+    }
+    ~mm_pt_order_scope() {
+        c->pt_order = saved;
+        c->pt_order_P = saved_P;
+    }
+};
+static inline const int32_t *mm_pt_order_of(const mm_ctx *ctx, const mm_ba_problem *pb) {
+    return ctx->pt_order && ctx->pt_order_P == pb->P ? ctx->pt_order : nullptr;
+}
+size_t mm_pt_order_scratch_bytes(int P, int64_t O, hipStream_t st);
 
 struct mm_stream_swap {
     mm_ctx *c;
@@ -73,8 +94,16 @@
 void mm_cam_table_hold(mm_ctx *ctx, bool on);
 void mm_cam_table_invalidate(mm_ctx *ctx);
 
+struct mm_trial_flag {
+    double cost;
+    const int32_t *info;
+    int32_t *go;
+};
 int mm_ba_residual_publish(mm_ctx *ctx, const mm_ba_problem *pb, const double *cams, const double *pts, void *ws,
-                           size_t ws_bytes, double *board, int cost_slot, int count, void *host_board, unsigned long long seq);
+                           size_t ws_bytes, double *board, int cost_slot, int count, void *host_board, unsigned long long seq,
+                           const mm_trial_flag *flag);
+int mm_sum_partials_publish(mm_ctx *ctx, const double *partial, int n, double *board, int cost_slot, int count, void *host_board,
+                            unsigned long long seq, const mm_trial_flag *flag);
 
 int mm_trf_fused0_scaled(mm_ctx *ctx, const double *g, double *si, const double *B, const double *C, double *gh, double *ghs, int64_t n,
                          int64_t split, double *out, void *ws, size_t ws_bytes);
diff --git a/meatmodeler_amd/csrc/trf.hip b/meatmodeler_amd/csrc/trf.hip
--- a/meatmodeler_amd/csrc/trf.hip
+++ b/meatmodeler_amd/csrc/trf.hip
@@ -126,7 +126,10 @@
     double *x, *x_new, *g, *si, *gh, *ghs, *gn, *q1, *w, *q2, *s1, *s2;
     double *B, *Bd, *C, *Cd, *Cinv, *u1, *Jq2, *dp, *v, *S;
     double *r0, *r1, *r2, *r3, *d11, *bs, *damp, *board, *cost2, *rowsx;
-    int32_t *info;
+    int32_t *info, *go;
+    int32_t *pt_order;
+    void *ws_order;
+    size_t ws_order_b;
     void *ws_res, *ws_md, *ws_jvp, *ws_schur, *ws_chol, *ws_back;
     size_t ws_res_b, ws_md_b, ws_jvp_b, ws_schur_b, ws_chol_b, ws_back_b;
     double *exs, *ex;
@@ -134,7 +137,7 @@
     size_t total;
 };
 
-TrfWs carve_trf(const mm_ba_problem *pb, void *base, int64_t ex_half_bw = -1) {
+TrfWs carve_trf(const mm_ba_problem *pb, void *base, int64_t ex_half_bw = -1, size_t order_scratch = 0) {
     TrfWs t;
     Carve c(base);
     const size_t F = pb->F, P = pb->P, O = (size_t)pb->O, n = 6 * F + 3 * P, nc = 6 * F;
@@ -161,6 +164,7 @@
     t.cost2 = c.take<double>(1);
     t.rowsx = c.take<double>(3);
     t.info = c.take<int32_t>(1);
+    t.go = c.take<int32_t>(1);
     t.ws_res_b = 2048 * 8;
     t.ws_res = c.take<char>(t.ws_res_b);
     t.ws_md_b = mm_multi_dot_workspace_bytes();
@@ -184,6 +188,13 @@
         t.exs = c.take<double>(EX_SCALARS);
         t.ex = c.take<double>(t.ex_count + 2);
     }
+    t.pt_order = nullptr;
+    t.ws_order = nullptr;
+    t.ws_order_b = order_scratch;
+    if (order_scratch) {
+        t.pt_order = c.take<int32_t>(P);
+        t.ws_order = c.take<char>(order_scratch);
+    }
     t.total = c.used;
     return t;
 }
@@ -205,11 +216,27 @@
 
 using namespace mm_trf;
 
+bool env_on(const char *name) {
+    const char *e = getenv(name);
+    return !e || atoi(e) != 0;
+}
+bool speculate_on() {
+    static const bool on = env_on("MM_TRF_SPECULATE");
+    return on;
+}
+bool pt_order_on() {
+    static const bool on = env_on("MM_PT_ORDER");
+    return on;
+}
+size_t order_scratch_of(const mm_ba_problem *pb, hipStream_t st) {
+    return pt_order_on() && pb->P > 0 && pb->O > 0 && pb->pt_ptr ? mm_pt_order_scratch_bytes(pb->P, pb->O, st) : 0;
+}
+
 }
 
 extern "C" size_t mm_ba_trf_workspace_bytes(const mm_ba_problem *pb) {
     if (!pb || pb->F < 0 || pb->P < 0 || pb->O < 0) return 0;
-    return carve_trf(pb, nullptr).total;
+    return carve_trf(pb, nullptr, -1, order_scratch_of(pb, nullptr)).total;
 }
 
 #define TRF_CALL(expr)        \
@@ -221,6 +248,25 @@
 extern "C" size_t mm_ba_trf_dist_workspace_bytes(const mm_ba_problem *pb, int half_bandwidth) {
     if (!pb || pb->F < 0 || pb->P < 0 || pb->O < 0 || half_bandwidth < 0) return 0;
     return carve_trf(pb, nullptr, half_bandwidth).total;
+}
+
+static int ensure_host_board(mm_ctx *ctx) {
+    if (!ctx->host_board) {
+        MM_HIP(ctx, hipHostMalloc(&ctx->host_board, sizeof(HostBoard), hipHostMallocDefault));
+        memset(ctx->host_board, 0, sizeof(HostBoard));
+        ctx->host_board_seq = 0;
+    }
+    return MM_OK;
+}
+
+extern "C" int mm_trf_trial_flag(mm_ctx *ctx, const double *partial, int n, double cost, const int32_t *info, double *board, int32_t *go) {
+    if (!ctx) return MM_ERR_ARG;
+    if (!partial || n < 0 || !info || !board || !go) return mm_fail(ctx, MM_ERR_ARG, "mm_trf_trial_flag: bad argument");
+    TRF_CALL(ensure_host_board(ctx));
+    const unsigned long long seq = ++ctx->host_board_seq;
+    const mm_trial_flag flag = {cost, info, go};
+    TRF_CALL(mm_sum_partials_publish(ctx, partial, n, board, 14, 16, ctx->host_board, seq, &flag));
+    return wait_seq(ctx, &((HostBoard *)ctx->host_board)->seq, seq, "mm_trf_trial_flag: the board");
 }
 
 static int trf_run(mm_ctx *ctx, const mm_ba_problem *pb, double *cams, double *pts, const mm_trf_params *prm, mm_trf_report *rep,
@@ -232,10 +278,12 @@
     if (dist && (dist->world < 1 || dist->world > EX_MAX_WORLD || dist->rank < 0 || dist->rank >= dist->world || !dist->allreduce ||
                  dist->half_bandwidth < 0))
         return mm_fail(ctx, MM_ERR_ARG, "mm_ba_trf_dist: bad communicator description (1 <= world <= %d)", EX_MAX_WORLD);
-    const size_t need = dist ? mm_ba_trf_dist_workspace_bytes(pb, dist->half_bandwidth) : mm_ba_trf_workspace_bytes(pb);
+    size_t order_scratch = dist ? 0 : order_scratch_of(pb, ctx->stream);
+    if (order_scratch && ws_bytes < carve_trf(pb, nullptr, -1, order_scratch).total) order_scratch = 0;
+    const size_t need = carve_trf(pb, nullptr, dist ? dist->half_bandwidth : -1, order_scratch).total;
     if (!ws || ws_bytes < need || ((uintptr_t)ws & 255))
         return mm_fail(ctx, MM_ERR_WORKSPACE, "mm_ba_trf: workspace too small or misaligned");
-    const TrfWs t = carve_trf(pb, ws, dist ? dist->half_bandwidth : -1);
+    const TrfWs t = carve_trf(pb, ws, dist ? dist->half_bandwidth : -1, order_scratch);
     struct TableHold {
         mm_ctx *c;
         explicit TableHold(mm_ctx *ctx) : c(ctx) { mm_cam_table_hold(c, true); }
@@ -266,6 +314,13 @@
     double *x = t.x, *x_new = t.x_new;
     MM_HIP(ctx, hipMemcpyAsync(x, cams, (size_t)nc * sizeof(double), hipMemcpyDeviceToDevice, st));
     if (P) MM_HIP(ctx, hipMemcpyAsync(x + nc, pts, (size_t)3 * P * sizeof(double), hipMemcpyDeviceToDevice, st));
+    mm_pt_order_scope order_scope(ctx);
+    order_scope.set(nullptr, 0);
+    if (t.pt_order) {
+        TRF_CALL(mm_ba_point_order(ctx, pb, t.pt_order, t.ws_order, t.ws_order_b));
+        order_scope.set(t.pt_order, P);
+    }
+    const bool speculate = !dist && speculate_on() && F > 0 && P > 0;
     double host[16];
     rep->chol_fallbacks = 0;
     rep->collectives = 0;
@@ -301,11 +356,7 @@
         MM_HIP(ctx, hipMemcpyAsync(t.g, t.ex + (size_t)F * 36, (size_t)nc * sizeof(double), hipMemcpyDeviceToDevice, st));
         return MM_OK;
     };
-    if (!ctx->host_board) {
-        MM_HIP(ctx, hipHostMalloc(&ctx->host_board, sizeof(HostBoard), hipHostMallocDefault));
-        memset(ctx->host_board, 0, sizeof(HostBoard));
-        ctx->host_board_seq = 0;
-    }
+    TRF_CALL(ensure_host_board(ctx));
     HostBoard *hb = (HostBoard *)ctx->host_board;
     auto take_board = [&](unsigned long long seq, int count) -> int {
         TRF_CALL(wait_seq(ctx, &hb->seq, seq, "mm_ba_trf: the trial-step scalars"));
@@ -374,6 +425,7 @@
         }
         double *reg_eff = t.damp + 1;
         bool rows_pending = false;
+        bool swept = false;
         auto trial = [&](double Delta_) -> int {
             if (rows_pending) {
                 rows_pending = false;
@@ -395,9 +447,14 @@
             }
             if (!dist) {
                 const unsigned long long seq = ++ctx->host_board_seq;
+                const mm_trial_flag flag = {d.cost, t.info, t.go};
                 TRF_CALL(mm_ba_residual_publish(ctx, pb, x_new, pts_of(x_new), t.ws_res, t.ws_res_b, t.board, 14, 16,
-                                                ctx->host_board, seq));
-                return take_board(seq, 16);
+                                                ctx->host_board, seq, speculate ? &flag : nullptr));
+                if (speculate)
+                    TRF_CALL(mm_ba_normal_eq_gated(ctx, pb, nullptr, x_new, pts_of(x_new), t.B, t.g, t.C, pts_of(t.g), t.go));
+                TRF_CALL(take_board(seq, 16));
+                swept = speculate && host[15] != 0;
+                return MM_OK;
             }
             TRF_CALL(mm_ba_residual(ctx, pb, x_new, pts_of(x_new), nullptr, t.board + 14, t.ws_res, t.ws_res_b));
             TRF_CALL(exchange({{t.board + 14, 3}, {t.board + 15, 4}}));
@@ -476,6 +533,7 @@
             TRF_CALL(exchange({{t.r3, 0}, {t.r3 + 3, 0}, {t.r3 + 6, 0}, {t.r3 + 9, 0}, {t.r3 + 12, 0}, {t.bs, 1}, {t.bs + 3, 1}}));
             TRF_CALL(trial(d.Delta));
             solve = d.on_solve(dist && host[15] > 0 ? -1 : (int)host[6], host[13], host[10], host[9]);
+            if ((solve == ABANDONED || solve == RETRY) && swept) TRF_CALL(normal_eq(x));
             if (solve == ABANDONED) {
                 if (ctx->chol_avoid_fused) return mm_fail(ctx, MM_ERR_HIP, "mm_ba_trf: the banded factorisation reported info = -1");
                 ctx->chol_avoid_fused = true;
@@ -488,10 +546,14 @@
         if (solve == INDEFINITE)
             return mm_fail(ctx, MM_ERR_NUMERIC, "mm_ba_trf: reduced camera system is not positive definite (pivot %d)", (int)host[6]);
         if (solve == DONE) break;
-        while ((next = d.on_trial(host[2], host[3], host[4], host[14])) == TRIAL) TRF_CALL(trial(d.Delta));
+        while ((next = d.on_trial(host[2], host[3], host[4], host[14])) == TRIAL) {
+            if (swept) TRF_CALL(normal_eq(x));
+            TRF_CALL(trial(d.Delta));
+        }
+        if (!d.accepted && swept) TRF_CALL(normal_eq(x));
         if (d.accepted) {
             std::swap(x, x_new);
-            TRF_CALL(normal_eq(x));
+            if (!swept) TRF_CALL(normal_eq(x));
             if (dist) TRF_CALL(mm_ba_scale_update(ctx, F, P, t.B, t.C, t.si, 0));
         }
     }
@@ -536,7 +598,7 @@
 
 extern "C" size_t mm_ba_trf_batched_workspace_bytes(const mm_ba_problem *pb) {
     if (!pb || pb->F < 0 || pb->P < 0 || pb->O < 0) return 0;
-    return carve_trf(pb, nullptr).total + batch_tables_bytes(pb);
+    return std::max(carve_trf(pb, nullptr).total + batch_tables_bytes(pb), mm_ba_trf_workspace_bytes(pb));
 }
 
 extern "C" int mm_ba_trf_batched(mm_ctx *ctx, int n_prob, const mm_ba_problem *const *pbs, double *const *cams, double *const *pts,
```

After: 8999 billion descriptor pairs/s (match stage). No clear change (-0.6%).
